# microsoft/ConfigNet

Measured on AMD Instinct MI355X. Metric: train-step images/sec at 256x256 (G+D fwd+bwd), higher is better.
Workload: dtype f32; 1 GPU; ConfigNet second-stage iteration (D + synth-D + latent-D + G + EMA), 256x256, batch 16 per GPU, fp32, Keras-Adam; global_batch=16, resolution=256, latent_dim=145, parallelism=dp1, losses_finite=True

## Files before the change

### confignet_amd/_lib.py

```python
import ctypes
import os

_HERE = os.path.dirname(os.path.abspath(__file__))
LIB_PATH = os.environ.get("CN_LIB") or os.path.join(_HERE, "libconfignet_hip.so")


class CnSumJob(ctypes.Structure):
    _fields_ = [("src", ctypes.c_void_p), ("dst", ctypes.c_void_p), ("count", ctypes.c_longlong), ("parts", ctypes.c_int),
                ("accumulate", ctypes.c_int)]


class CnDepthJob(ctypes.Structure):
    _fields_ = [("a", ctypes.c_void_p), ("b", ctypes.c_void_p), ("c", ctypes.c_void_p), ("m", ctypes.c_int), ("n", ctypes.c_int),
                ("k", ctypes.c_int), ("lda", ctypes.c_int), ("ldb", ctypes.c_int), ("ldc", ctypes.c_int)]


class CnRowsJob(ctypes.Structure):
    _fields_ = [("a", ctypes.c_void_p), ("b", ctypes.c_void_p), ("c", ctypes.c_void_p), ("bias", ctypes.c_void_p), ("mask", ctypes.c_void_p)] + \
               [(n_, ctypes.c_int) for n_ in ("m", "n", "k", "lda", "ldb", "ldc", "tb", "act", "accumulate")] + [("slope", ctypes.c_float)]


class CnGanJob(ctypes.Structure):
    _fields_ = [("s", ctypes.c_void_p), ("out", ctypes.c_void_p), ("gout", ctypes.c_void_p), ("n", ctypes.c_int), ("label", ctypes.c_float)]


class CnConvGeom(ctypes.Structure):
    _fields_ = [(n, ctypes.c_int) for n in (
        "nd", "n", "in_d", "in_h", "in_w", "cin", "out_d", "out_h", "out_w", "cout",
        "k_d", "k_h", "k_w", "s_d", "s_h", "s_w", "dl_d", "dl_h", "dl_w", "p_d", "p_h", "p_w", "up")]


CN_F32, CN_BF16 = 0, 1
CN_U8 = 2
CN_EUNSUPPORTED = -3


class ConfigNetHipError(RuntimeError):
    pass


if not os.path.exists(LIB_PATH):
    raise ImportError(
        "confignet_amd: %s is missing -- build it with `python confignet_amd/build.py` "
        "(or __graft_entry__.build()).  There is no CPU/PyTorch fallback." % LIB_PATH)

lib = ctypes.CDLL(LIB_PATH)

_p = ctypes.c_void_p
_i = ctypes.c_int
_f = ctypes.c_float
_z = ctypes.c_size_t
_G = ctypes.POINTER(CnConvGeom)

SIGNATURES = {
    "cn_version": [],
    "cn_conv_fwd": [_G, _p, _p, _p, _p, _i, _f, _p],
    "cn_conv_fwd_res": [_G, _p, _p, _p, _p, _p, _i, _f, _p],
    "cn_conv_fwd_stats": [_G, _p, _p, _p, _p, _i, _f, _p, _i, _f, _p],
    "cn_scale_columns_segments": [_p, _p, _p, _p, _i, _z, _p],
    "cn_conv_weight_tflip": [_p, _p, _i, _i, _i, _p],
    "cn_conv_dgrad": [_G, _p, _p, _p, _p],
    "cn_conv_dgrad_w": [_G, _p, _p, _p, _p],
    "cn_conv_dgrad_w_res": [_G, _p, _p, _p, _p, _p],
    "cn_bn_fold_bwd": [_p, _i, _i, _p, _p, _p, _p, _p, _p, _p, _p],
    "cn_conv_wgrad_thin_partials": [],
    "cn_conv_wgrad_thin": [_G, _p, _p, _p, _p, _i, _p],
    "cn_conv_wgrad": [_G, _p, _p, _p, _i, _p],
    "cn_conv_wgrad_workspace_bytes": [_G],
    "cn_conv_wgrad_ws": [_G, _p, _p, _p, _i, _p, _z, _p],
    "cn_conv_wgrad_ws_slabs": [_G, _p, _p, _p, _i, _p, _z, ctypes.POINTER(_i), _p],
    "cn_conv_wgrad_dt_workspace_bytes": [_G, _i, _i, ctypes.POINTER(_z)],
    "cn_conv_wgrad_dt": [_G, _p, _i, _p, _i, _p, _i, _p, _z, ctypes.POINTER(_i), _p],
    "cn_conv_wgrad_plan": [_G, _i, _i, _i, ctypes.c_uint, _i, ctypes.POINTER(ctypes.c_longlong)],
    "cn_sum_parts_grouped": [_p, _i, _p],
    "cn_gemm_depth_grouped": [_p, _i, _p],
    "cn_gan_loss_grouped": [_p, _i, _i, _p],
    "cn_gemm_rows_grouped": [_p, _i, _p],
    "cn_gemm_rows_grouped_k": [_p, _i, _p],
    "cn_gemm_rows_grouped_plan": [_p, _i, ctypes.POINTER(_i), _i, ctypes.POINTER(_i)],
    "cn_conv_tune": [_i, _i, ctypes.c_long],
    "cn_conv_fwd_plan": [_G, _i, _i, _i, _i, _i, _i, _i, ctypes.POINTER(ctypes.c_int * 8)],
    "cn_conv_loop_select": [_i, _i, _i, _i],
    "cn_fwd2_col_block": [_i, _i, _i, _i, _i, _i],
    "cn_conv_fwd_dt": [_p, _p, _i, _p, _p, _p, _i, _i, _f, _p],
    "cn_conv_dgrad_dt": [_p, _p, _i, _p, _p, _i, _p],
    "cn_conv_wgrad_c3_partials": [],
    "cn_conv_wgrad_c3": [_p, _p, _p, _i, _p, _p, _i, _p],
    "cn_conv_wino_filter": [_p, _p, _i, _i, _i, _p],
    "cn_conv_fwd_wino": [_i, _i, _i, _i, _i, _p, _p, _p, _p, _i, _f, _p],
    "cn_conv_fwd_wino4": [_i, _i, _i, _i, _i, _p, _p, _p, _p, _i, _f, _p],
    "cn_conv_fwd_wino4_ep": [_i, _i, _i, _i, _i, _p, _p, _p, _p, _i, _f, _i, _p, _p, _p, _p, _i, _f, _p],
    "cn_conv_wino4_filter": [_p, _p, _i, _i, _i, _p],
    "cn_sumpool2": [_p, _p, _i, _i, _i, _i, _i, _i, _i, _p],
    "cn_gemm": [_i, _i, _i, _i, _i, _p, _i, _p, _i, _p, _i, _p, _i, _f, _p],
    "cn_gemm_plan": [_i] * 10 + [ctypes.POINTER(ctypes.c_int * 9)],
    "cn_nc_reduce4": [_p, _p, _i, _i, _i, _f, _i, _i, _p],
    "cn_nc_reduce": [_p, _p, _p, _p, _i, _i, _i, _i, _f, _i, _p],
    "cn_nc_reduce_plan": [_i, _i, _i, _i, _i, _i, ctypes.POINTER(ctypes.c_int * 8)],
    "cn_nc_lin2": [_p, _p, _p, _p, _p, _p, _p, _p, _i, _i, _i, _i, _i, _f, _i, _p],
    "cn_nc_rows_plan": [ctypes.c_longlong, _i, _i, ctypes.POINTER(ctypes.c_int * 2)],
    "cn_norm_coef_fwd": [_i, _p, _p, _p, _p, _p, _p, _p, _p, _i, _i, _i, _f, _p, _i, _p],
    "cn_norm_coef_bwd": [_i, _p, _p, _p, _p, _p, _p, _p, _p, _p, _p, _i, _i, _i, _f, _p],
    "cn_dual_tail_coef_fwd": [_p] * 13 + [_i, _i, _i, _f, _i, _i, _p],
    "cn_dual_tail_coef_bwd": [_p] * 13 + [ctypes.POINTER(ctypes.c_void_p), _i, _i, _i, _f, _i, _i, _p],
    "cn_dual_tail_gx": [_p] * 12 + [_i, _i, _i, _f, _i, _i, _p],
    "cn_dual_tail_gx_tx": [_p] * 18 + [_i, _i, _i, _f, _i, _i, _i, _p],
    "cn_norm_apply": [_i, _i] + [_p] * 13 + [_i, _i, _i, _f, _i, _f, _i, _p],
    "cn_nc_reduce_hxt": [_p, _p, _p, _p, _i, _i, _i, _f, _i, _i, _i, _p],
    "cn_zero": [_p, ctypes.c_size_t, _p],
    "cn_set_deterministic": [_i],
    "cn_get_deterministic": [],
    "cn_det_release_stream": [_p],
    "cn_gemm_acc": [_i, _i, _i, _i, _i, _p, _i, _p, _i, _p, _i, _p],
    "cn_sum_rows_into": [_p, _p, _i, _i, _i, _p],
    "cn_bn_act_bwd": [_p, _p, _p, _p, _p, _p, _p, _p, _i, _i, _i, _i, _i, _i, _p],
    "cn_nc_reduce_dact": [_p, _p, _p, _p, _p, _i, _i, _i, _i, _f, _i, _i, _p],
    "cn_act_fwd": [_p, _p, _z, _i, _f, _i, _p],
    "cn_act_bwd": [_p, _p, _p, _z, _i, _f, _i, _p],
    "cn_act_bwd_bias": [_p, _p, _p, _p, _i, _i, _i, _i, _f, _i, _i, _p],
    "cn_axpby": [_p, _p, _p, _z, _f, _f, _i, _p],
    "cn_mul": [_p, _p, _p, _z, _i, _p],
    "cn_sqdiff_sum": [_p, _p, _p, _z, _f, _i, _p],
    "cn_row_sumsq": [_p, _p, _i, _z, _p],
    "cn_row_scale": [_p, _p, _p, _i, _z, _f, _i, _p],
    "cn_row_scale_diff": [_p, _p, _p, _p, _i, ctypes.c_size_t, _f, _i, _p],
    "cn_tap_bwd": [_p, _p, _p, _p, _p, _i, ctypes.c_size_t, _f, _i, _f, _i, _p],
    "cn_maxpool2_bwd_act": [_p, _p, _p, _p, _f, _p, _i, _i, _i, _i, _i, _i, _p],
    "cn_stream_plan": [_i, _i, ctypes.c_longlong, _z, _i, _i, _i, _i, _i, _i, ctypes.c_uint, _i, ctypes.POINTER(ctypes.c_longlong * 4)],
    "cn_stream_plan_ptrs": [_i, _i, _i, ctypes.c_longlong, _z, _i, _i, _i, _i, _i, _i, ctypes.POINTER(ctypes.c_void_p * 4), _i, ctypes.POINTER(ctypes.c_longlong * 4)],
    "cn_stream_last_plan": [ctypes.POINTER(ctypes.c_longlong * 5)],
    "cn_masked_diff": [_p, _p, _p, _p, _z, _i, _p],
    "cn_maxpool_fwd": [_p, _p, _i, _i, _i, _i, _i, _i, _i, _i, _p],
    "cn_maxpool_bwd": [_p, _p, _p, _i, _i, _i, _i, _i, _i, _i, _i, _p],
    "cn_avgpool3_same": [_p, _p, _i, _i, _i, _i, _i, _p],
    "cn_dwconv3x3_fwd": [_p, _p, _p, _p, _i, _i, _i, _i, _i, _i, _f, _p],
    "cn_image_preprocess": [_p, _i, _p, _i, _i, _i, _i, _i, _i, _f, _f, _p],
    "cn_dwconv3x3_dgrad": [_p, _p, _p, _i, _i, _i, _i, _i, _p],
    "cn_dwconv3x3_wgrad_slices": [_i, _i, _i, _i, _i],
    "cn_dwconv3x3_wgrad": [_p, _p, _p, _i, _i, _i, _i, _i, _i, _p],
    "cn_bn_train_coef": [_p] * 12 + [ctypes.c_longlong, _i, _f, ctypes.c_double, _i, _p],
    "cn_bn_train_apply": [_p, _p, _p, _p, ctypes.c_longlong, _i, _i, _p],
    "cn_bn_train_bwd_slices": [ctypes.c_longlong, _i],
    "cn_chan_slices_plan": [ctypes.c_longlong, _i, _i, ctypes.POINTER(ctypes.c_int * 5)],
    "cn_bn_train_bwd_reduce": [_p] * 6 + [_i, ctypes.c_longlong, _i, _i, _p],
    "cn_bn_train_bwd_apply": [_p] * 8 + [ctypes.c_longlong, _i, _i, _p],
    "cn_chan_affine3_fwd": [_p, _p, _z, ctypes.POINTER(_i), _f, ctypes.POINTER(_f), _p],
    "cn_chan_affine3_bwd": [_p, _p, _z, ctypes.POINTER(_i), _f, _p],
    "cn_gan_loss_fwd": [_p, _p, _i, _f, _p],
    "cn_gan_loss_bwd": [_p, _p, _p, _i, _f, _p],
    "cn_euler_matrix": [_p, _p, _i, _p],
    "cn_euler_matrix_bwd": [_p, _p, _p, _i, _p],
    "cn_rotate3d_fwd": [_p, _p, _p, _i, _i, _i, _p],
    "cn_rotate3d_bwd": [_p, _p, _p, _p, _p, _i, _i, _i, _p],
    "cn_rotate3d_bwd_plan": [_i, _i, _i, _i, ctypes.POINTER(ctypes.c_int * 4)],
    "cn_adam_step": [_p, _p, _p, _p, _p, _z, _p, _f, _f, _f, _f, _p],
    "cn_ema_step": [_p, _p, _z, _f, _p],
    "cn_gather_images_u8": [_p, _p, _p, _p, _i, _i, _i, _i, _p],
    "cn_to_uint8": [_p, _p, _z, _p],
    "cn_hdri_rows_v": [_p, _p, _p, _p, _i, _i, _i, _i, _i, _p],
    "cn_hdri_rows_h": [_p, _p, _p, _p, _p, _p, _p, _i, _i, _i, _i, _i, _i, _p],
    "cn_exp2m1": [_p, _p, _z, _p],
    "cn_warp_affine_u8": [_p] * 6 + [_i] * 6 + [_p],
    "cn_warp_nearest_f32": [_p] * 6 + [_i] * 6 + [_p],
    "cn_eye_mask": [_p, _p, _z, _i] + [_f] * 6 + [_p],
    "cn_spin": [ctypes.c_ulonglong, _p],
    "cn_conv_weight_prep_bf16": [_p, _p, _p, _i, _i, _i, _p],
    "cn_conv_fwd_bf16": [_G, _p, _p, _p, _p, _i, _f, _p],
    "cn_conv_dgrad_bf16": [_G, _p, _p, _p, _p],
    "cn_conv_wgrad_bf16": [_G, _p, _p, _p, _i, _p],
    "cn_cast": [_p, _i, _p, _i, _z, _p],
    "cn_upfold_weights": [_p, _p, _p, _i, ctypes.POINTER(_i), ctypes.POINTER(_i), _i, _i, ctypes.POINTER(_i), ctypes.POINTER(_i), _p],
    "cn_upfold_wgrad": [_p, _p, _i, ctypes.POINTER(_i), ctypes.POINTER(_i), _i, _i, _i, _p],
    "cn_prof_enable": [_i],
    "cn_prof_reset": [],
    "cn_prof_collect": [ctypes.POINTER(_i), ctypes.POINTER(ctypes.c_double), ctypes.POINTER(ctypes.c_double)],
    "cn_prof_collect_by_family": [ctypes.POINTER(_i), ctypes.POINTER(ctypes.c_double), ctypes.POINTER(ctypes.c_double), ctypes.POINTER(ctypes.c_double)],
}

for _name, _args in SIGNATURES.items():
    _fn = getattr(lib, _name)
    _fn.argtypes = _args
    _fn.restype = ctypes.c_int
lib.cn_conv_wgrad_workspace_bytes.restype = ctypes.c_size_t
lib.cn_last_error_string.argtypes = []
lib.cn_last_error_string.restype = ctypes.c_char_p


def check(code, what):
    if code != 0:
        raise ConfigNetHipError("%s failed (%d): %s" % (what, code, lib.cn_last_error_string().decode()))
```

### confignet_amd/csrc/common.h

```cpp
#pragma once
#include <hip/hip_runtime.h>
#include <stdint.h>
#include <stdio.h>
#include "../../include/confignet_hip.h"

void cn_set_error(const char* fmt, ...);

#define CN_CHECK_ARG(cond, ...)            \
    do {                                   \
        if (!(cond)) {                     \
            cn_set_error(__VA_ARGS__);     \
            return CN_EINVAL;              \
        }                                  \
    } while (0)

#define CN_HIP(expr)                                                              \
    do {                                                                          \
        hipError_t e__ = (expr);                                                  \
        if (e__ != hipSuccess) {                                                  \
            cn_set_error("%s failed: %s (%s:%d)", #expr, hipGetErrorString(e__), __FILE__, __LINE__); \
            return CN_EHIP;                                                       \
        }                                                                         \
    } while (0)

#define CN_LAUNCH_CHECK()                                                         \
    do {                                                                          \
        hipError_t e__ = hipGetLastError();                                       \
        if (e__ != hipSuccess) {                                                  \
            cn_set_error("kernel launch failed: %s (%s:%d)", hipGetErrorString(e__), __FILE__, __LINE__); \
            return CN_EHIP;                                                       \
        }                                                                         \
    } while (0)

int cn_zero_async(void* p, size_t bytes, hipStream_t s);

int cn_det();
float* cn_det_ws(hipStream_t s, size_t need_floats);
constexpr size_t CN_DET_WS_FLOATS = (size_t)16 << 20;
int cn_sum_parts(const float* src, float* dst, int parts, long count, int accumulate, float scale, hipStream_t s);

int cn_fwd2(const CnConvGeom* gp, int cfg, int bt, const float* A, const float* B, const float* bias, float* C, long M, int N, int K,
            int act, float slope, int splits, long part_stride, int par, hipStream_t s, const float* res, double x_elems, double w_elems,
            float* stats = nullptr, int stats_mode = 0, float stats_slope = 0.f, int srows = 1, int sper = 1);
void cn_fwd2_tune(int kb, int ns, int np);
void cn_fwd2_grid(int cfg, long M, int N, int par, int splits, int grid[3]);
int cn_igemm_fwd(int cfg, const CnConvGeom& g, bool vec, int par, int splits, const float* x, const float* w, const float* bias, float* y,
                 int act, float slope, hipStream_t s, int bt, long part_stride, const float* res);
void cn_igemm_fwd_grid(int cfg, const CnConvGeom& g, bool vec, int par, int splits, int grid[3]);
int cn_igemm_fwd_thin(const CnConvGeom& g, const float* x, const float* w, const float* bias, float* y, int act, float slope, hipStream_t s);
enum ConvRoute { CN_ROUTE_UP2K4_RGB = 0, CN_ROUTE_S2_IMAGE_DGRAD, CN_ROUTE_S1_IMAGE_DGRAD, CN_ROUTE_THIN_PAR_IGEMM, CN_ROUTE_THIN_COOP,
                 CN_ROUTE_THIN, CN_ROUTE_C3, CN_ROUTE_C7S2, CN_ROUTE_FWD2, CN_ROUTE_IGEMM, CN_ROUTE_UNSUPPORTED };
constexpr int CN_THIN_COOP_PX = 4;
void cn_small_conv(int route, unsigned grid_x, const CnConvGeom& g, bool vec, int par, const void* x, int x_dt, const float* w,
                   const float* bias, void* y, int y_dt, int act, float slope, hipStream_t s);
int cn_fwd2_bf16(const CnConvGeom& g, int cfg, int flip, const void* x, const void* wb, const float* bias, void* y, int act, float slope,
                 int par, hipStream_t s);

enum WgradRoute { CN_WG_C3 = 0, CN_WG_THIN, CN_WG_TINY, CN_WG_WGRAD2, CN_WG_IGEMM, CN_WG_BF16, CN_WG_NONE };
constexpr int CN_C3_WGRAD_TILE = 64, CN_C3_WGRAD_PARTS = 512;
constexpr int CN_THIN_WGRAD_TH = 8, CN_THIN_WGRAD_TW = 32, CN_THIN_WGRAD_PARTS = 512;
struct Wg2Plan {
    int cfg;
    long tiles_x, tiles_y, splits, rows;
};
bool cn_wgrad2_ok(const CnConvGeom& g);
Wg2Plan cn_wgrad2_plan(const CnConvGeom& g, int forced_cfg, long wg_target);
void cn_wgrad2(int cfg, int ns, const CnConvGeom& g, const float* x, const float* gy, float* out, long slab_stride, int rows, int tiles_x,
               int tiles_y, int splits, int accumulate, unsigned grid, hipStream_t s);
void cn_igemm_wgrad(int cfg, const CnConvGeom& g, const float* x, const float* gy, float* gw, int rows, float* parts, int tx, int ty,
                    int splits, dim3 grid, hipStream_t s);
int cn_tiny_wgrad(const CnConvGeom& g, const float* x, const float* gy, float* gw, int blocks, float* parts, hipStream_t s);
void cn_bf16_wgrad(int cfg, const CnConvGeom& g, const void* x, const void* gy, float* gw, int rows, int tx, int ty, int splits, dim3 grid,
                   hipStream_t s);
int cn_c3_wgrad(const CnConvGeom& g, const float* x, const void* gy, int gy_dt, float* scratch, int tiles_x, int ntiles, int nparts,
                size_t lds, hipStream_t s);
void cn_c3_wgrad_reduce(const float* scratch, float* gw, int nparts, int count, int accumulate, hipStream_t s);
void cn_thin_wgrad(const CnConvGeom& g, const float* x, const float* gy, float* scratch, int nwg, size_t lds, int tiles_y, int tiles_x,
                   int ntiles, hipStream_t s);

enum { CN_FAM_FWD_128x128 = 0, CN_FAM_FWD_128x64, CN_FAM_FWD_64x64, CN_FAM_FWD_128x32, CN_FAM_FWD_128x96, CN_FAM_WGRAD_128x128,
       CN_FAM_WGRAD_128x96, CN_FAM_WGRAD_64x64, CN_FAM_WGRAD_128x32, CN_FAM_WINO, CN_FAM_C3_FWD, CN_FAM_S2_IMAGE_DGRAD,
       CN_FAM_THIN, CN_FAM_C3_WGRAD, CN_FAM_BF16_FWD, CN_FAM_BF16_WGRAD, CN_FAM_WGRAD_256x64, CN_FAM_WGRAD_SLAB_SUM };
void cn_prof_begin(hipStream_t s, double flops, double bytes = 0.0, int family = 31);
void cn_prof_end(hipStream_t s);

__device__ __forceinline__ void divmod_pos(int m, int d, int& q, int& r) {
    if ((d & (d - 1)) == 0) {
        q = m >> (__builtin_ctz(d));
        r = m & (d - 1);
    } else {
        q = m / d;
        r = m - q * d;
    }
}

__device__ __forceinline__ float cn_apply_act(float v, int act, float slope) {
    switch (act) {
        case CN_ACT_LRELU: return v > 0.f ? v : v * slope;
        case CN_ACT_RELU: return v > 0.f ? v : 0.f;
        case CN_ACT_TANH: return tanhf(v);
        default: break;
    }
    if (act == CN_ACT_RELU6) return fminf(fmaxf(v, 0.f), 6.f);
    if (act == CN_ACT_SIGMOID) return __fdividef(1.f, 1.f + __expf(-v));
    return v;
}

__device__ __forceinline__ float act_deriv(float o, int act, float slope) {
    if (act == CN_ACT_LRELU) return o > 0.f ? 1.f : slope;
    if (act == CN_ACT_RELU) return o > 0.f ? 1.f : 0.f;
    if (act == CN_ACT_TANH) return 1.f - o * o;
    return 1.f;
}

static inline int cn_cdiv(long a, long b) { return (int)((a + b - 1) / b); }

int cn_cu_count();
```

### confignet_amd/csrc/conv_dispatch.hip

```cpp
#include "common.h"

#include <algorithm>

#include "mma_tile.h"
#include "conv_geom.h"

namespace {

int g_tune_cfg = -1;
int g_tune_splits = 0;
long g_tune_wg_blocks = 0;
int g_tune_wg2_ns = 0;
int g_fwd2_sel = -1;
constexpr int g_fwd2_min_nks = 1;
constexpr int g_fwd2_min_c = 48;

struct ConvReq {
    int bt, has_bias, act, has_res, stats_mode, x_dt, y_dt;
};

struct ConvPlan {
    int route = CN_ROUTE_UNSUPPORTED;
    int ret = CN_EUNSUPPORTED;
    int cfg = -1;
    int splits = 1, par = 0;
    bool vec = false;
    bool plain = false;
    int family = -1;
    int srows = 1, sper = 1;
    int grid[3] = {0, 0, 0};
};

int image_route(const CnConvGeom& g, const ConvReq& q) {
    const bool x32 = q.x_dt == CN_F32, y32 = q.y_dt == CN_F32, x16 = q.x_dt == CN_BF16, y16 = q.y_dt == CN_BF16;
    if (x32 && (y32 || y16) && !q.bt && g.nd == 2 && g.cin == 3 && g.dl_h == 1 && g.dl_w == 1 && !g.up && g.cout > 4 && g.cout <= 64) {
        if (g.k_h == 3 && g.k_w == 3 && g.s_h == g.s_w && (g.s_h == 1 || g.s_h == 2)) return CN_ROUTE_C3;
        if (g.k_h == 7 && g.k_w == 7 && g.s_h == 2 && g.s_w == 2 && !q.has_res) return CN_ROUTE_C7S2;
    }
    if (y32 && g.nd == 2 && g.k_h == 3 && g.k_w == 3 && g.s_h == 1 && g.s_w == 1 && !g.up && g.cout == 3 && !q.has_bias &&
        q.act == CN_ACT_NONE && g.p_h >= 0 && g.p_h <= 2 && g.p_w >= 0 && g.p_w <= 2) {
        if ((x32 || x16) && g.dl_h == 2 && g.dl_w == 2 && g.cin == 48 && g.out_h <= 2 * g.in_h && g.out_w <= 2 * g.in_w) return CN_ROUTE_S2_IMAGE_DGRAD;
        if (x32 && g.dl_h == 1 && g.dl_w == 1 && g.cin == 64) return CN_ROUTE_S1_IMAGE_DGRAD;
    }
    return CN_ROUTE_UNSUPPORTED;
}

ConvPlan plan_conv_fwd(const CnConvGeom& g, const ConvReq& q) {
    ConvPlan p;
    const long M = (long)g.n * g.out_d * g.out_h * g.out_w;
    const bool res = q.has_res != 0, stats = q.stats_mode != 0;
    const int bt = q.bt;
    auto small = [&p](int route, int family, long grid_x) {
        p.route = route;
        p.ret = CN_OK;
        p.family = family;
        p.grid[0] = (int)grid_x; p.grid[1] = p.grid[2] = 1;
        return p;
    };
    auto refuse = [&p](int code) {
        p.ret = code;
        return p;
    };
    const int img = image_route(g, q);
    const long img_grid = img == CN_ROUTE_S2_IMAGE_DGRAD ? (long)g.n * cn_cdiv(g.in_h, 8) * cn_cdiv(g.in_w, 32)
                                                         : (long)g.n * cn_cdiv(g.out_h, 8) * cn_cdiv(g.out_w, 32);
    const int img_family = img == CN_ROUTE_C3 || img == CN_ROUTE_C7S2 ? CN_FAM_C3_FWD : CN_FAM_S2_IMAGE_DGRAD;
    if (q.x_dt != CN_F32 || q.y_dt != CN_F32)
        return img != CN_ROUTE_UNSUPPORTED ? small(img, img_family, img_grid) : p;
    if ((res || stats) && (g.cout <= 4 || g.cin == 3 || g.cout % 4 != 0)) return p;
    if (stats && (bt || cn_det() || g.cin % BK != 0)) return p;
    if (bt && (g.cout <= 4 || g.cin % BK != 0 || g.cout % 4 != 0)) return p;
    if (g.cout <= 4) {
        p.vec = g.cin % 4 == 0;
        p.par = parity_ordered(g);
        const size_t lds = sizeof(float) * 4 * (size_t)g.k_d * g.k_h * g.k_w * g.cin;
        if (lds > 64 * 1024) {
            cn_set_error("thin conv: filter of %zu bytes does not fit the LDS stage", lds);
            return refuse(CN_EINVAL);
        }
        const int T = g.k_d * g.k_h * g.k_w, CL = g.cin / 4;
        const bool dl1 = g.dl_d * g.dl_h * g.dl_w == 1;
        if (g.nd == 2 && g.up == 1 && g.k_h == 4 && g.k_w == 4 && g.s_h == 1 && g.s_w == 1 && g.dl_h == 1 && g.dl_w == 1 &&
            g.cout == 3 && g.cin == 32 && g.p_h == 1 && g.p_w == 1 && g.out_h <= 2 * g.in_h && g.out_w <= 2 * g.in_w)
            return small(CN_ROUTE_UP2K4_RGB, CN_FAM_THIN, (long)g.n * cn_cdiv(g.in_h, 8) * cn_cdiv(g.in_w, 16));
        if (img != CN_ROUTE_UNSUPPORTED) return small(img, img_family, img_grid);
        if (p.par && g.cin % BK == 0 && q.act == CN_ACT_NONE) return small(CN_ROUTE_THIN_PAR_IGEMM, CN_FAM_FWD_128x32, cn_cdiv(M, 128));
        if (p.vec && g.cout == 3 && CL >= 5 && CL <= 16 && T <= 32 && (p.par || dl1) && g.dl_d * g.dl_h * g.dl_w <= 8)
            return small(CN_ROUTE_THIN_COOP, -1, cn_cdiv(M, (256 / (CL <= 8 ? 8 : 16)) * CN_THIN_COOP_PX));
        return small(CN_ROUTE_THIN, -1, cn_cdiv(M, 256));
    }
    if (img != CN_ROUTE_UNSUPPORTED) return small(img, img_family, img_grid);
    if (g.cout % 4 != 0) {
        cn_set_error("cout=%d: implicit-GEMM path needs cout %% 4 == 0", g.cout);
        return refuse(CN_EINVAL);
    }
    const bool vec = g.cin % BK == 0;
    const int par = parity_ordered(g) && vec;
    const long t128 = (long)cn_cdiv(M, 128) * cn_cdiv(g.cout, 128);
    const long t128x64 = (long)cn_cdiv(M, 128) * cn_cdiv(g.cout, 64);
    int cfg;
    long tiles;
    if (g.cout <= 32) { cfg = 3; tiles = (long)cn_cdiv(M, 128) * cn_cdiv(g.cout, 32); }
    else if (g.cout > 64 && t128 >= 512) { cfg = 0; tiles = t128; }
    else if (t128x64 >= 512) { cfg = 1; tiles = t128x64; }
    else { cfg = 2; tiles = (long)cn_cdiv(M, 64) * cn_cdiv(g.cout, 64); }
    if (g.cout % 96 == 0 && g.cout % 128 != 0 &&
        (long)cn_cdiv(M, 128) * (g.cout / 96) >= (g.cout == 96 ? 256 : 384)) {
        cfg = 4;
        tiles = (long)cn_cdiv(M, 128) * (g.cout / 96);
    }
    int splits = 1;
    const bool par_small = par && cfg == 2;
    const long nks_total = vec ? (long)g.k_d * g.k_h * g.k_w * (g.cin / BK) : 0;
    if (cfg == 0 && vec && !par && nks_total <= 8) { cfg = 1; tiles = t128x64; }
    const bool short_full = !par && tiles >= 256 && nks_total < 64;
    if (vec && tiles < (par_small ? 1024 : 512) && !short_full) {
        long nks = nks_total;
        if (par) nks /= (long)g.dl_d * g.dl_h * g.dl_w;
        long want = ((par_small ? 3072 : 1024) + tiles - 1) / tiles;
        if (want > 16) want = 16;
        const long min_steps = par_small ? 8 : 16;
        if (want > nks / min_steps) want = nks / min_steps;
        if (want > 1) splits = (int)want;
    }
    const bool n32 = g.cout == 32 && g.cin >= 32;
    const bool fwd2_takes = g_fwd2_sel != 0 && vec && nks_total > g_fwd2_min_nks && ((g.cin >= g_fwd2_min_c && g.cout >= g_fwd2_min_c) || n32) &&
                            g.dl_d <= 2 && g.dl_h <= 2 && g.dl_w <= 2 && (double)g.n * g.in_d * g.in_h * g.in_w * g.cin < 5.3e8 &&
                            (double)g.k_d * g.k_h * g.k_w * g.cin * g.cout < 5.3e8;
    if (fwd2_takes) {
        const int T = g.k_d * g.k_h * g.k_w;
        const long Me = (par && T == 1) ? M / ((long)g.dl_d * g.dl_h * g.dl_w) : M;
        long nks = nks_total;
        if (par) nks /= (long)g.dl_d * g.dl_h * g.dl_w;
        splits = 1;
        const bool par_balanced = par && g.k_d % g.dl_d == 0 && g.k_h % g.dl_h == 0 && g.k_w % g.dl_w == 0;
        if (n32) {
            cfg = 3;
            tiles = cn_cdiv(M, 128);
        } else if (par && T > 1 && !par_balanced) {
            cfg = 2;
            tiles = (long)cn_cdiv(M, 64) * cn_cdiv(g.cout, 64);
            if (g.cout % 96 == 0 && g.cout % 64 != 0 && (long)cn_cdiv(M, 128) * (g.cout / 96) >= 512) {
                cfg = 4;
                tiles = (long)cn_cdiv(M, 128) * (g.cout / 96);
            }
            if (cfg == 2 && tiles < 1024) {
                long want = (1536 + tiles / 2) / tiles;
                if (want > 16) want = 16;
                if (want > nks / 8) want = nks / 8;
                if (want > 1) splits = (int)want;
            }
        } else {
            struct Cand { int cfg, bm, bn; double step_us; };
            const Cand cands[2] = {{2, 64, 64, 0.265}, {4, 128, 96, 0.68}};
            double best = 0.0;
            bool have = false;
            for (const Cand& c : cands) {
                if (c.cfg == 4 && (g.cout % 96 != 0 || g.cout % 64 == 0 || (long)cn_cdiv(Me, 128) * (g.cout / 96) < 256)) continue;
                const long tl = (long)cn_cdiv(Me, c.bm) * cn_cdiv(g.cout, c.bn);
                const long smax = nks / 8 > 1 ? (nks / 8 > 16 ? 16 : nks / 8) : 1;
                for (long s_ = 1; s_ <= smax; ++s_) {
                    const double waves = (double)cn_cdiv(tl * s_, cn_cu_count());
                    double t = 10.0 + waves * (double)cn_cdiv(nks, s_) * c.step_us * (waves == 1.0 ? 1.06 : 1.0);
                    if (s_ > 1) t += 9.0 + (double)s_ * (double)M * g.cout * 4.0 / 6.0e6;
                    if (s_ > 1 && (res || stats)) t += 5.0 + 2.0 * (double)M * g.cout * 4.0 / 3.0e6;
                    if (!have || t < best) { have = true; best = t; cfg = c.cfg; tiles = tl; splits = (int)s_; }
                }
            }
        }
    }
    if (g_tune_cfg >= 0) cfg = g_tune_cfg;
    if (g_tune_splits > 0) splits = g_tune_splits;
    if (res && splits > 1) return p;
    if (stats) {
        const int qd = par ? g.out_d / g.dl_d : g.out_d, qh = par ? g.out_h / g.dl_h : g.out_h, qw = par ? g.out_w / g.dl_w : g.out_w;
        p.srows = qd * qh * qw;
        p.sper = par ? g.n * p.srows : (int)M;
        if (!fwd2_takes || splits > 1 || cfg == 3 || p.srows % (cfg == 2 ? 64 : 128) != 0) return p;
    }
    if (cn_det() && splits > 1) {
        const long cap = (long)(CN_DET_WS_FLOATS / ((size_t)M * g.cout));
        if (splits > cap) splits = (int)cap;
        if (splits <= 1 || !vec) splits = 1;
    }
    p.route = fwd2_takes && (cfg != 3 || n32) && cfg >= 0 && cfg <= 4 ? CN_ROUTE_FWD2 : CN_ROUTE_IGEMM;
    if (stats && p.route != CN_ROUTE_FWD2) return refuse(CN_EINVAL);
    p.ret = CN_OK;
    p.cfg = cfg;
    p.splits = splits;
    p.par = par;
    p.vec = vec;
    p.family = cfg == 0 ? CN_FAM_FWD_128x128 : cfg == 1 ? CN_FAM_FWD_128x64 : cfg == 3 ? CN_FAM_FWD_128x32 : cfg == 4 ? CN_FAM_FWD_128x96 : CN_FAM_FWD_64x64;
    if (p.route == CN_ROUTE_FWD2) {
        p.plain = !par && g.k_d * g.k_h * g.k_w == 1 && g.s_d == 1 && g.s_h == 1 && g.s_w == 1 && g.dl_d == 1 && g.dl_h == 1 &&
                  g.dl_w == 1 && !g.up && g.p_d == 0 && g.p_h == 0 && g.p_w == 0 && g.out_d == g.in_d && g.out_h == g.in_h &&
                  g.out_w == g.in_w;
        cn_fwd2_grid(cfg, M, g.cout, par, splits, p.grid);
    } else {
        cn_igemm_fwd_grid(cfg, g, vec, par, splits, p.grid);
    }
    return p;
}

int run_conv_fwd(const ConvPlan& p, const CnConvGeom& g, const ConvReq& q, const void* x, const float* w, const float* bias,
                 const float* res, void* y, float slope, float* stats, float stats_slope, hipStream_t s) {
    if (p.route == CN_ROUTE_UNSUPPORTED) return p.ret;
    const long M = (long)g.n * g.out_d * g.out_h * g.out_w;
    const int splits = p.splits;
    float* parts = nullptr;
    if (cn_det() && splits > 1) {
        parts = cn_det_ws(s, (size_t)splits * M * g.cout);
        if (!parts) return CN_EINVAL;
    }
    const int kact = splits > 1 ? CN_ACT_NONE : q.act;
    if (splits > 1 && !parts) {
        if (int ez__ = cn_zero_async(y, sizeof(float) * M * g.cout, s)) return ez__;
    }
    const long part_stride = parts ? (long)M * g.cout : 0;
    float* const out = parts ? parts : (float*)y;
    if (p.family >= 0) cn_prof_begin(s, conv_flops(g), conv_bytes(g, q.x_dt == CN_BF16 ? 2.0 : 4.0, q.y_dt == CN_BF16 ? 2.0 : 4.0), p.family);
    int e = CN_OK;
    switch (p.route) {
        case CN_ROUTE_FWD2: {
            const double xe = (double)g.n * g.in_d * g.in_h * g.in_w * g.cin, we = (double)g.k_d * g.k_h * g.k_w * g.cin * g.cout;
            e = cn_fwd2(p.plain ? nullptr : &g, p.cfg, q.bt, (const float*)x, w, bias, out, M, g.cout, g.cin, kact, slope, splits, part_stride,
                        p.plain ? 0 : p.par, s, res, xe, we, stats, q.stats_mode, stats_slope, p.srows, p.sper);
            break;
        }
        case CN_ROUTE_IGEMM:
            e = cn_igemm_fwd(p.cfg, g, p.vec, p.par, splits, (const float*)x, w, bias, out, kact, slope, s, q.bt, part_stride, res);
            break;
        case CN_ROUTE_THIN_PAR_IGEMM:
            e = cn_igemm_fwd_thin(g, (const float*)x, w, bias, out, kact, slope, s);
            break;
        default:
            cn_small_conv(p.route, (unsigned)p.grid[0], g, p.vec, p.par, x, q.x_dt, w, bias, y, q.y_dt, kact, slope, s);
            break;
    }
    if (p.family >= 0) cn_prof_end(s);
    CN_CHECK_ARG(e != CN_EUNSUPPORTED, "convolution plan (route %d, tile %d) refused by its kernel", p.route, p.cfg);
    if (e != CN_OK) return e;
    CN_LAUNCH_CHECK();
    if (parts) e = cn_sum_parts(parts, (float*)y, splits, (long)M * g.cout, 0, 1.f, s);
    if (e == CN_OK && splits > 1 && q.act != CN_ACT_NONE) e = cn_act_fwd(y, y, (size_t)M * g.cout, q.act, slope, CN_F32, s);
    return e;
}

int conv_fwd(const CnConvGeom* gp, const ConvReq& q, const void* x, const float* w, const float* bias, const float* res, void* y,
             float slope, float* stats, float stats_slope, void* stream) {
    if (int e = check_geom(gp)) return e;
    CN_CHECK_ARG(x && w && y, "NULL tensor");
    return run_conv_fwd(plan_conv_fwd(*gp, q), *gp, q, x, w, bias, res, y, slope, stats, stats_slope, (hipStream_t)stream);
}

}

extern "C" int cn_conv_fwd(const CnConvGeom* gp, const float* x, const float* w, const float* bias, float* y, int act,
                           float slope, void* stream) {
    return conv_fwd(gp, ConvReq{0, bias != nullptr, act, 0, 0, CN_F32, CN_F32}, x, w, bias, nullptr, y, slope, nullptr, 0.f, stream);
}

extern "C" int cn_conv_fwd_stats(const CnConvGeom* gp, const float* x, const float* w, const float* bias, float* y, int act,
                                 float slope, float* stats, int stats_mode, float stats_slope, void* stream) {
    CN_CHECK_ARG(stats && (stats_mode == 1 || stats_mode == 2), "cn_conv_fwd_stats: stats buffer and mode 1 / 2");
    CN_CHECK_ARG(stats_mode == 1 || act == CN_ACT_NONE, "cn_conv_fwd_stats: mode 2 takes the statistics of the pre-activation output");
    return conv_fwd(gp, ConvReq{0, bias != nullptr, act, 0, stats_mode, CN_F32, CN_F32}, x, w, bias, nullptr, y, slope, stats, stats_slope, stream);
}

extern "C" int cn_conv_fwd_res(const CnConvGeom* gp, const float* x, const float* w, const float* bias, const float* res, float* y,
                               int act, float slope, void* stream) {
    CN_CHECK_ARG(res, "cn_conv_fwd_res: res is NULL");
    return conv_fwd(gp, ConvReq{0, bias != nullptr, act, 1, 0, CN_F32, CN_F32}, x, w, bias, res, y, slope, nullptr, 0.f, stream);
}

extern "C" int cn_conv_fwd_dt(const CnConvGeom* gp, const void* x, int x_dt, const float* w, const float* bias, void* y, int y_dt,
                              int act, float slope, void* stream) {
    if (int e = check_geom(gp)) return e;
    CN_CHECK_ARG(x && w && y, "NULL tensor");
    if (x_dt == CN_F32 && y_dt == CN_F32) return CN_EUNSUPPORTED;
    const ConvReq q{0, bias != nullptr, act, 0, 0, x_dt, y_dt};
    return run_conv_fwd(plan_conv_fwd(*gp, q), *gp, q, x, w, bias, nullptr, y, slope, nullptr, 0.f, (hipStream_t)stream);
}

extern "C" int cn_conv_dgrad(const CnConvGeom* gp, const float* gy, const float* w_tflip, float* gu, void* stream) {
    if (int e = check_geom(gp)) return e;
    CN_CHECK_ARG(gp->dl_d == 1 && gp->dl_h == 1 && gp->dl_w == 1, "dgrad of a dilated-input geometry is not defined here");
    const CnConvGeom d = dgrad_geom(*gp);
    return cn_conv_fwd(&d, gy, w_tflip, nullptr, gu, CN_ACT_NONE, 0.f, stream);
}

extern "C" int cn_conv_dgrad_dt(const CnConvGeom* gp, const void* gy, int gy_dt, const float* w_tflip, void* gu, int gu_dt,
                                void* stream) {
    if (int e = check_geom(gp)) return e;
    if (gp->dl_d != 1 || gp->dl_h != 1 || gp->dl_w != 1) return CN_EUNSUPPORTED;
    const CnConvGeom d = dgrad_geom(*gp);
    return cn_conv_fwd_dt(&d, gy, gy_dt, w_tflip, nullptr, gu, gu_dt, CN_ACT_NONE, 0.f, stream);
}

extern "C" int cn_conv_dgrad_w(const CnConvGeom* gp, const float* gy, const float* w, float* gu, void* stream) {
    if (int e = check_geom(gp)) return e;
    if (gp->dl_d != 1 || gp->dl_h != 1 || gp->dl_w != 1) return CN_EUNSUPPORTED;
    const CnConvGeom d = dgrad_geom(*gp);
    return conv_fwd(&d, ConvReq{1, 0, CN_ACT_NONE, 0, 0, CN_F32, CN_F32}, gy, w, nullptr, nullptr, gu, 0.f, nullptr, 0.f, stream);
}

// ... 40 lines not shown
    int grid[3] = {0, 0, 0};
    size_t lds = 0;
    size_t ws_floats = 0;
    size_t det_floats = 0;
    bool zero = false;
    int sum = WG_SUM_NONE;
};

struct WgTile { int bm, bn; };
WgTile wgrad_tile(int cfg) { return cfg == 3 ? WgTile{128, 32} : cfg == 4 ? WgTile{128, 96} : cfg == 0 ? WgTile{128, 128} : cfg == 5 ? WgTile{256, 64} : WgTile{64, 64}; }
int wgrad_family(int cfg) {
    return cfg == 3 ? CN_FAM_WGRAD_128x32 : cfg == 4 ? CN_FAM_WGRAD_128x96 : cfg == 0 ? CN_FAM_WGRAD_128x128 : cfg == 5 ? CN_FAM_WGRAD_256x64 : CN_FAM_WGRAD_64x64;
}

void sliced_grid(const CnConvGeom& g, WgTile t, WgradPlan& p) {
    const long Ktot = (long)g.k_d * g.k_h * g.k_w * g.cin;
    const int gx = cn_cdiv(Ktot, t.bm), gy = cn_cdiv(g.cout, t.bn);
    p.grid[0] = gx; p.grid[1] = gy; p.grid[2] = (int)p.splits;
    if ((long)gx * gy > 1 && p.splits >= 16) {
        p.tx = gx; p.ty = gy;
        p.grid[0] = cn_cdiv(p.splits, 8) * 8 * gx * gy; p.grid[1] = p.grid[2] = 1;
    }
}

bool igemm_wgrad_slices(const CnConvGeom& g, WgTile t, long wg_target, bool det, WgradPlan& p) {
    const long M = (long)g.n * g.out_d * g.out_h * g.out_w;
    const long Ktot = (long)g.k_d * g.k_h * g.k_w * g.cin;
    const long tiles = (long)cn_cdiv(Ktot, t.bm) * cn_cdiv(g.cout, t.bn);
    const long wg_blocks = wg_target > 0 ? wg_target : 2048;
    long splits = (wg_blocks + tiles - 1) / tiles;
    if (det) {
        const long cap = (long)(CN_DET_WS_FLOATS / ((size_t)Ktot * g.cout));
        if (cap < 1) {
            cn_set_error("deterministic filter gradient: %ld x %d filter does not fit the workspace", Ktot, g.cout);
            return false;
        }
        if (splits > cap) splits = cap;
    }
    long rows = (M + splits - 1) / splits;
    if (rows < 256) rows = 256;
    rows = (rows + BK - 1) / BK * BK;
    p.rows = rows;
    p.splits = (M + rows - 1) / rows;
    return true;
}

void bf16_wgrad_slices(const CnConvGeom& g, WgTile t, WgradPlan& p) {
    constexpr long KS = 32, min_rows = 512;
    const long M = (long)g.n * g.out_d * g.out_h * g.out_w;
    const long Ktot = (long)g.k_d * g.k_h * g.k_w * g.cin;
    const long tiles = (long)cn_cdiv(Ktot, t.bm) * cn_cdiv(g.cout, t.bn);
    const long per_cu = t.bm * t.bn >= 128 * 128 ? 3 : t.bm * t.bn >= 128 * 96 ? 4 : 5;
    const long target = 256 * per_cu * (t.bn >= 96 ? 1 : 2);
    long splits = target / tiles;
    if (splits > M / min_rows) splits = M / min_rows;
    const long fill = std::min<long>(M / 256, (256 + tiles - 1) / tiles);
    if (splits < fill) splits = fill;
    if (splits >= 16) splits &= ~7L;
    if (splits < 1) splits = 1;
    long rows = (M + splits - 1) / splits;
    if (rows < 256) rows = std::min<long>(256, (M + KS - 1) / KS * KS);
    rows = (rows + KS - 1) / KS * KS;
    p.rows = rows;
    p.splits = (M + rows - 1) / rows;
}

WgradPlan plan_conv_wgrad(const CnConvGeom& g, const WgradReq& q) {
    WgradPlan p;
    const long M = (long)g.n * g.out_d * g.out_h * g.out_w;
    const long Ktot = (long)g.k_d * g.k_h * g.k_w * g.cin;
    const size_t count = (size_t)Ktot * g.cout;
    const bool x32 = q.x_dt == CN_F32, y32 = q.gy_dt == CN_F32, x16 = q.x_dt == CN_BF16, y16 = q.gy_dt == CN_BF16;
    auto may = [&q](int route) { return (q.routes & wg_bit(route)) != 0; };
    auto take = [&p](int route, int family) {
        p.route = route;
        p.ret = CN_OK;
        p.family = family;
    };
    if (may(CN_WG_C3) && x32 && (y32 || y16) && g.nd == 2 && g.cin == 3 && g.k_h == 3 && g.k_w == 3 && g.k_d == 1 && g.s_h == g.s_w &&
        (g.s_h == 1 || g.s_h == 2) && g.dl_h == 1 && g.dl_w == 1 && g.up == 0 && g.cout <= 64 && g.cout >= 4 && g.cout % 4 == 0) {
        take(CN_WG_C3, CN_FAM_C3_WGRAD);
        p.tx = cn_cdiv(g.out_w, CN_C3_WGRAD_TILE);
        p.grid[0] = CN_C3_WGRAD_PARTS; p.grid[1] = p.grid[2] = 1;
        const int pw = CN_C3_WGRAD_TILE * g.s_h + 2, gpitch = (g.cout + 3) & ~3;
        p.lds = sizeof(float) * 4 * (size_t)(3 * pw * 3 + CN_C3_WGRAD_TILE * gpitch);
        if (p.lds < sizeof(float) * 4 * 2 * 16 * 64) p.lds = sizeof(float) * 4 * 2 * 16 * 64;
        p.ws_floats = CN_C3_WGRAD_PARTS * count;
        p.sum = WG_SUM_C3;
        return p;
    }
    const int T = g.k_h * g.k_w;
    if (may(CN_WG_THIN) && x32 && y32 && g.nd == 2 && g.cout <= 4 && g.cin % 4 == 0 && g.cin >= 8 && g.cin <= 64 && g.s_h == 1 && g.s_w == 1 &&
        g.dl_h == 1 && g.dl_w == 1 && T <= 16 && T * (g.cin / 4) <= 256) {
        const int PH0 = ((CN_THIN_WGRAD_TH + g.k_h - 1) >> g.up) + 2, PW0 = ((CN_THIN_WGRAD_TW + g.k_w - 1) >> g.up) + 2;
        size_t lds = sizeof(float) * ((size_t)PH0 * PW0 * g.cin + CN_THIN_WGRAD_TH * CN_THIN_WGRAD_TW * 4);
        const size_t red = sizeof(float) * 256 * 4 * g.cout;
        if (lds < red) lds = red;
        if (lds <= 64 * 1024) {
            take(CN_WG_THIN, -1);
            p.ty = cn_cdiv(g.out_h, CN_THIN_WGRAD_TH); p.tx = cn_cdiv(g.out_w, CN_THIN_WGRAD_TW);
            const int ntiles = g.n * p.ty * p.tx;
            p.grid[0] = ntiles < CN_THIN_WGRAD_PARTS ? ntiles : CN_THIN_WGRAD_PARTS; p.grid[1] = p.grid[2] = 1;
            p.lds = lds;
            p.ws_floats = CN_THIN_WGRAD_PARTS * count;
            p.sum = WG_SUM_PARTS;
            return p;
        }
    }
    if (x16 && y16) {
        if (!may(CN_WG_BF16) || g.cin % 8 || g.cout % 8) return p;
        take(CN_WG_BF16, CN_FAM_BF16_WGRAD);
        p.cfg = wgrad_tile_cfg(g);
        bf16_wgrad_slices(g, wgrad_tile(p.cfg), p);
        sliced_grid(g, wgrad_tile(p.cfg), p);
        p.zero = true;
        return p;
    }
    if (!x32 || !y32) return p;
    if (may(CN_WG_WGRAD2) && cn_wgrad2_ok(g) && Ktot >= 64) {
        const int t = g_tune_cfg;
        const Wg2Plan w = cn_wgrad2_plan(g, t == 0 || t == 2 || t == 3 || t == 4 || t == 5 ? t : -1, g_tune_wg_blocks);
        take(CN_WG_WGRAD2, wgrad_family(w.cfg));
        p.cfg = w.cfg;
        p.stages = w.cfg == 3 || g_tune_wg2_ns == 3 ? 3 : 4;
        p.splits = w.splits; p.rows = w.rows;
        p.tx = (int)w.tiles_x; p.ty = (int)w.tiles_y;
        p.grid[0] = (int)((w.splits >= 8 ? cn_cdiv(w.splits, 8) * 8 : w.splits) * w.tiles_x * w.tiles_y); p.grid[1] = p.grid[2] = 1;
        if (w.splits > 1) {
            p.ws_floats = (size_t)w.splits * count;
            p.sum = q.caller_slabs ? WG_SUM_CALLER : WG_SUM_PARTS;
        }
        return p;
    }
    if (may(CN_WG_TINY) && Ktot <= 4 && g.cout <= 4 && g.k_d * g.k_h * g.k_w == 1 && g.s_h == 1 && g.s_w == 1 && g.s_d == 1 && !g.up &&
        g.p_h == 0 && g.p_w == 0 && g.p_d == 0) {
        take(CN_WG_TINY, -1);
        p.grid[0] = cn_cdiv(M, 256) > 1024 ? 1024 : cn_cdiv(M, 256); p.grid[1] = p.grid[2] = 1;
        p.zero = true;
        if (q.det) {
            p.det_floats = (size_t)p.grid[0] * 16;
            p.sum = WG_SUM_PARTS;
        }
        return p;
    }
    if (!may(CN_WG_IGEMM)) return p;
    const int cfg = wgrad_tile_cfg(g);
    if (!igemm_wgrad_slices(g, wgrad_tile(cfg), g_tune_wg_blocks, q.det, p)) {
        p.ret = CN_EINVAL;
        return p;
    }
    take(CN_WG_IGEMM, wgrad_family(cfg));
    p.cfg = cfg;
    sliced_grid(g, wgrad_tile(cfg), p);
    p.zero = true;
    if (q.det) {
        p.det_floats = (size_t)p.splits * count;
        p.sum = WG_SUM_PARTS;
    }
    return p;
}

int sum_conv_wgrad(const WgradPlan& p, int nparts, long count, int mode, float* gw, const float* ws, const float* det, int* parts_out,
                   hipStream_t s) {
    CN_LAUNCH_CHECK();
    const int add = mode != CN_WGRAD_WRITE;
    if (p.sum == WG_SUM_PARTS) return cn_sum_parts(det ? det : ws, gw, nparts, count, det ? 1 : add, 1.f, s);
    if (p.sum == WG_SUM_C3) {
        cn_c3_wgrad_reduce(ws, gw, nparts, (int)count, mode == CN_WGRAD_ADD, s);
        CN_LAUNCH_CHECK();
    }
    if (p.sum == WG_SUM_CALLER) *parts_out = nparts;
    return CN_OK;
}

int run_conv_wgrad(const WgradPlan& p, const CnConvGeom& g, const WgradReq& q, const void* x, const void* gy, float* gw, int mode,
                   float* ws, size_t ws_bytes, int* parts_out, hipStream_t s) {
    if (parts_out) *parts_out = 0;
    if (p.route == CN_WG_NONE) return p.ret;
    CN_CHECK_ARG(mode == CN_WGRAD_WRITE || mode == CN_WGRAD_ADD || mode == CN_WGRAD_ZEROED, "filter gradient: mode %d", mode);
    CN_CHECK_ARG(p.ws_floats == 0 || (ws && ws_bytes >= sizeof(float) * p.ws_floats), "filter gradient: workspace of %zu bytes, %zu needed",
                 ws ? ws_bytes : (size_t)0, sizeof(float) * p.ws_floats);
    CN_CHECK_ARG(p.sum != WG_SUM_CALLER || parts_out, "filter gradient: slabs left to a caller that takes none");
    CN_CHECK_ARG(p.route != CN_WG_BF16 || (((uintptr_t)x | (uintptr_t)gy) & 15) == 0, "bf16 convolution needs 16-byte aligned tensors");
    const long count = (long)g.k_d * g.k_h * g.k_w * g.cin * g.cout;
    const int add = mode != CN_WGRAD_WRITE;
    float* det = nullptr;
    if (p.det_floats) {
        det = cn_det_ws(s, p.det_floats);
        if (!det) return CN_EINVAL;
    }
    if (p.zero && !add) {
        if (int ez__ = cn_zero_async(gw, sizeof(float) * count, s)) return ez__;
    }
    if (p.family >= 0)
        cn_prof_begin(s, p.route == CN_WG_C3 ? 2.0 * 27.0 * g.cout * (double)g.n * g.out_h * g.out_w : conv_flops(g),
                      conv_bytes(g, q.x_dt == CN_BF16 ? 2.0 : 4.0, q.gy_dt == CN_BF16 ? 2.0 : 4.0, 4.0), p.family);
    const dim3 grid(p.grid[0], p.grid[1], p.grid[2]);
    int nparts = (int)p.splits, e = CN_OK;
    switch (p.route) {
        case CN_WG_C3:
            e = cn_c3_wgrad(g, (const float*)x, gy, q.gy_dt, ws, p.tx, g.n * g.out_h * p.tx, nparts = p.grid[0], p.lds, s);
            break;
        case CN_WG_THIN:
            cn_thin_wgrad(g, (const float*)x, (const float*)gy, ws, nparts = p.grid[0], p.lds, p.ty, p.tx, g.n * p.ty * p.tx, s);
            break;
        case CN_WG_TINY:
            nparts = cn_tiny_wgrad(g, (const float*)x, (const float*)gy, gw, p.grid[0], det, s);
            break;
        case CN_WG_WGRAD2:
            cn_wgrad2(p.cfg, p.stages, g, (const float*)x, (const float*)gy, p.splits > 1 ? ws : gw, p.splits > 1 ? count : 0, (int)p.rows,
                      p.tx, p.ty, (int)p.splits, add, grid.x, s);
            break;
        case CN_WG_IGEMM:
            cn_igemm_wgrad(p.cfg, g, (const float*)x, (const float*)gy, gw, (int)p.rows, det, p.tx, p.ty, (int)p.splits, grid, s);
            break;
        default:
            cn_bf16_wgrad(p.cfg, g, x, gy, gw, (int)p.rows, p.tx, p.ty, (int)p.splits, grid, s);
            break;
    }
    const bool sum_in_bracket = p.route != CN_WG_C3;
    if (p.family >= 0 && !sum_in_bracket) cn_prof_end(s);
    if (e == CN_OK) e = sum_conv_wgrad(p, nparts, count, mode, gw, ws, det, parts_out, s);
    if (p.family >= 0 && sum_in_bracket) cn_prof_end(s);
    return e;
}

int conv_wgrad(const CnConvGeom* gp, const WgradReq& q, const void* x, const void* gy, float* gw, int mode, void* ws, size_t ws_bytes,
               int* parts, void* stream) {
    if (int e = check_geom(gp)) return e;
    CN_CHECK_ARG(x && gy && gw, "NULL tensor");
    return run_conv_wgrad(plan_conv_wgrad(*gp, q), *gp, q, x, gy, gw, mode, (float*)ws, ws_bytes, parts, (hipStream_t)stream);
}

}

extern "C" int cn_conv_wgrad(const CnConvGeom* gp, const float* x, const float* gy, float* gw, int accumulate, void* stream) {
    return conv_wgrad(gp, WgradReq{CN_F32, CN_F32, false, WG_ATOMIC}, x, gy, gw, accumulate ? CN_WGRAD_ADD : CN_WGRAD_WRITE, nullptr, 0, nullptr, stream);
}

extern "C" size_t cn_conv_wgrad_workspace_bytes(const CnConvGeom* gp) {
    if (!gp || check_geom(gp) != CN_OK) return 0;
    return sizeof(float) * plan_conv_wgrad(*gp, WgradReq{CN_F32, CN_F32, false, WG_FP32_GEMM}).ws_floats;
}

extern "C" int cn_conv_wgrad_ws(const CnConvGeom* gp, const float* x, const float* gy, float* gw, int accumulate, void* workspace,
                                size_t workspace_bytes, void* stream) {
    return conv_wgrad(gp, WgradReq{CN_F32, CN_F32, false, WG_FP32_GEMM}, x, gy, gw, accumulate ? CN_WGRAD_ADD : CN_WGRAD_WRITE, workspace,
                      workspace_bytes, nullptr, stream);
}

extern "C" int cn_conv_wgrad_ws_slabs(const CnConvGeom* gp, const float* x, const float* gy, float* gw, int accumulate, void* workspace,
                                      size_t workspace_bytes, int* parts, void* stream) {
    CN_CHECK_ARG(parts, "cn_conv_wgrad_ws_slabs: parts is NULL");
    return conv_wgrad(gp, WgradReq{CN_F32, CN_F32, true, WG_FP32_GEMM}, x, gy, gw, accumulate ? CN_WGRAD_ADD : CN_WGRAD_WRITE, workspace,
                      workspace_bytes, parts, stream);
}

extern "C" int cn_conv_wgrad_bf16(const CnConvGeom* gp, const uint16_t* x, const uint16_t* gy, float* gw, int accumulate,
                                  void* stream) {
    return conv_wgrad(gp, WgradReq{CN_BF16, CN_BF16, false, wg_bit(CN_WG_BF16)}, x, gy, gw, accumulate ? CN_WGRAD_ADD : CN_WGRAD_WRITE, nullptr, 0,
                      nullptr, stream);
}

extern "C" int cn_conv_wgrad_c3_partials(void) { return CN_C3_WGRAD_PARTS; }

extern "C" int cn_conv_wgrad_c3(const CnConvGeom* gp, const float* x, const void* gy, int gy_dt, float* scratch, float* gw,
                                int accumulate, void* stream) {
    CN_CHECK_ARG(gp && x && gy && scratch && gw && (gy_dt == CN_F32 || gy_dt == CN_BF16), "conv_wgrad_c3: bad args");
    return conv_wgrad(gp, WgradReq{CN_F32, gy_dt, false, wg_bit(CN_WG_C3)}, x, gy, gw, accumulate ? CN_WGRAD_ADD : CN_WGRAD_WRITE, scratch, SIZE_MAX,
                      nullptr, stream);
}

extern "C" int cn_conv_wgrad_thin_partials(void) { return CN_THIN_WGRAD_PARTS; }

extern "C" int cn_conv_wgrad_thin(const CnConvGeom* gp, const float* x, const float* gy, float* scratch, float* gw, int accumulate,
                                  void* stream) {
    CN_CHECK_ARG(scratch, "conv_wgrad_thin: NULL");
    return conv_wgrad(gp, WgradReq{CN_F32, CN_F32, false, wg_bit(CN_WG_THIN)}, x, gy, gw, accumulate ? CN_WGRAD_ADD : CN_WGRAD_WRITE, scratch, SIZE_MAX,
                      nullptr, stream);
}

extern "C" int cn_conv_wgrad_dt_workspace_bytes(const CnConvGeom* gp, int x_dt, int gy_dt, size_t* bytes) {
    if (int e = check_geom(gp)) return e;
    CN_CHECK_ARG(bytes, "cn_conv_wgrad_dt_workspace_bytes: bytes is NULL");
    const WgradPlan p = plan_conv_wgrad(*gp, WgradReq{x_dt, gy_dt, false, WG_ALL});
    *bytes = sizeof(float) * p.ws_floats;
    return p.ret;
}

extern "C" int cn_conv_wgrad_dt(const CnConvGeom* gp, const void* x, int x_dt, const void* gy, int gy_dt, float* gw, int mode, void* workspace,
                                size_t workspace_bytes, int* parts, void* stream) {
    return conv_wgrad(gp, WgradReq{x_dt, gy_dt, parts != nullptr, WG_ALL}, x, gy, gw, mode, workspace, workspace_bytes, parts, stream);
}

extern "C" int cn_conv_wgrad_plan(const CnConvGeom* gp, int x_dt, int gy_dt, int caller_slabs, unsigned routes, int det, long long out[12]) {
    if (int e = check_geom(gp)) return e;
    CN_CHECK_ARG(out, "cn_conv_wgrad_plan: out is NULL");
    const WgradPlan p = plan_conv_wgrad(*gp, WgradReq{x_dt, gy_dt, caller_slabs != 0, routes, det < 0 ? cn_det() != 0 : det != 0});
    const long long v[12] = {p.route, p.cfg, p.splits, p.rows, p.family, p.grid[0], p.grid[1], p.grid[2], (long long)p.ws_floats, p.zero, p.sum, p.stages};
    for (int i = 0; i < 12; ++i) out[i] = v[i];
    return p.ret;
}

extern "C" int cn_conv_loop_select(int loop, int kb, int ns, int np) {
    CN_CHECK_ARG(loop >= -1 && loop <= 1 && (kb == 0 || kb == 16 || kb == 32) && (ns == 0 || ns == 3 || ns == 4) && np >= -1 && np <= 2,
                 "cn_conv_loop_select: bad argument");
    g_fwd2_sel = loop;
    cn_fwd2_tune(kb, ns, np);
    g_tune_wg2_ns = ns;
    return CN_OK;
}

extern "C" int cn_conv_tune(int cfg, int splits, long wg_blocks) {
    g_tune_cfg = cfg;
    g_tune_splits = splits;
    g_tune_wg_blocks = wg_blocks;
    return CN_OK;
}
```

### confignet_amd/csrc/elementwise.hip

```cpp
#include "common.h"
#include "typed.h"
#include <stdlib.h>

namespace {

__device__ __forceinline__ float lrelu(float v, float s) { return v > 0.f ? v : v * s; }


template <int V> struct RowV { float v[V]; };

template <int V, typename T>
__device__ __forceinline__ RowV<V> ld_row(const T* p) {
    RowV<V> r;
    if constexpr (V == 4) {
        const float4 t = ld4<T>(p);
        r.v[0] = t.x; r.v[1] = t.y; r.v[2] = t.z; r.v[3] = t.w;
    } else {
        r.v[0] = ldf<T>(p);
    }
    return r;
}
template <int V, typename T>
__device__ __forceinline__ void st_row(T* p, const RowV<V>& r) {
    if constexpr (V == 4) st4<T>(p, make_float4(r.v[0], r.v[1], r.v[2], r.v[3]));
// ... 1312 lines not shown
    CN_CHECK_ARG(a && b && out && (dt == CN_F32 || dt == CN_BF16), "sqdiff_sum: bad args");
    if (!numel) return CN_OK;
    StreamPlan sp;
    if (int e = stream_entry_plan(stream_req(SP_SQDIFF_SUM, dt, 1, numel), dt, StreamPtrs{{a, b}}, &sp)) return e;
    const int vec = sp.path == SP_VEC, blocks = sp.gx;
    float* parts = nullptr;
    if (sp.parts) {
        parts = cn_det_ws((hipStream_t)stream, (size_t)sp.parts);
        if (!parts) return CN_EINVAL;
    }
    CN_DISPATCH_DT(dt, hipLaunchKernelGGL((sqdiff_sum_kernel<T>), dim3(blocks), dim3(256), 0, (hipStream_t)stream, (const T*)a, (const T*)b, out, numel, scale, vec, parts));
    CN_LAUNCH_CHECK();
    if (parts) return cn_sum_parts(parts, out, blocks, 1, 1, scale, (hipStream_t)stream);
    return CN_OK;
}
extern "C" int cn_row_sumsq(const float* x, float* out, int n, size_t row, void* stream) {
    CN_CHECK_ARG(x && out && n > 0 && row > 0, "row_sumsq: bad args");
    StreamPlan sp;
    if (int e = stream_entry_plan(stream_req(SP_ROW_SUMSQ, CN_F32, n, row), CN_F32, StreamPtrs{{x}}, &sp)) return e;
    const int vec = sp.path == SP_VEC, bpr = sp.gx;
    if (sp.parts) {
        float* parts = cn_det_ws((hipStream_t)stream, (size_t)sp.parts);
        if (!parts) return CN_EINVAL;
        hipLaunchKernelGGL(row_sumsq_kernel, dim3(bpr, n), dim3(256), 0, (hipStream_t)stream, x, out, row, vec, parts);
        CN_LAUNCH_CHECK();
        return cn_sum_parts(parts, out, bpr, n, 0, 1.f, (hipStream_t)stream);
    }
    if (int ez__ = cn_zero_async(out, sizeof(float) * n, (hipStream_t)stream)) return ez__;
    hipLaunchKernelGGL(row_sumsq_kernel, dim3(bpr, n), dim3(256), 0, (hipStream_t)stream, x, out, row, vec, (float*)nullptr);
    CN_LAUNCH_CHECK();
    return CN_OK;
}
extern "C" int cn_row_scale(const void* x, const float* s, void* out, int n, size_t row, float k, int dt, void* stream) {
    CN_CHECK_ARG(x && s && out && n > 0 && row > 0 && (dt == CN_F32 || dt == CN_BF16), "row_scale: bad args");
    StreamPlan sp;
    if (int e = stream_entry_plan(stream_req(SP_ROW_SCALE, dt, n, row), dt, StreamPtrs{{x, out}}, &sp)) return e;
    const int vec = sp.path == SP_VEC;
    CN_DISPATCH_DT(dt, hipLaunchKernelGGL((row_scale_kernel<T>), dim3(sp.gx, sp.gy), dim3(256), 0, (hipStream_t)stream, (const T*)x, s, (T*)out, row, k, vec));
    CN_LAUNCH_CHECK();
    return CN_OK;
}
extern "C" int cn_row_scale_diff(const void* x, const void* x2, const float* s, void* out, int n, size_t row, float k, int dt, void* stream) {
    CN_CHECK_ARG(x && x2 && s && out && n > 0 && row > 0 && (dt == CN_F32 || dt == CN_BF16), "row_scale_diff: bad args");
    StreamPlan sp;
    if (int e = stream_entry_plan(stream_req(SP_ROW_SCALE_DIFF, dt, n, row), dt, StreamPtrs{{x, x2, out}}, &sp)) return e;
    const int vec = sp.path == SP_VEC;
    CN_DISPATCH_DT(dt, hipLaunchKernelGGL((row_scale_kernel<T>), dim3(sp.gx, sp.gy), dim3(256), 0, (hipStream_t)stream, (const T*)x, s, (T*)out, row, k, vec, (const T*)x2));
    CN_LAUNCH_CHECK();
    return CN_OK;
}
extern "C" int cn_tap_bwd(const void* y, const void* target, const void* g, const float* s, void* out, int n, size_t row, float k,
                          int act, float slope, int dt, void* stream) {
    CN_CHECK_ARG(y && target && s && out && n > 0 && row > 0 && (dt == CN_F32 || dt == CN_BF16), "tap_bwd: bad args");
    StreamPlan sp;
    if (int e = stream_entry_plan(stream_req(SP_TAP_BWD, dt, n, row), dt, StreamPtrs{{y, target, g, out}}, &sp)) return e;
    const int vec = sp.path == SP_VEC;
    CN_DISPATCH_DT(dt, hipLaunchKernelGGL((tap_bwd_kernel<T>), dim3(sp.gx, sp.gy), dim3(256), 0, (hipStream_t)stream, (const T*)y, (const T*)target,
                                          (const T*)g, s, (T*)out, row, k, vec, act, slope));
    CN_LAUNCH_CHECK();
    return CN_OK;
}
extern "C" int cn_masked_diff(const float* a, const float* b, const uint8_t* mask, float* out, size_t pixels, int c, void* stream) {
    CN_CHECK_ARG(a && mask && out && c > 0, "masked_diff: bad args");
    if (!pixels) return CN_OK;
    EW_LAUNCH(masked_diff_kernel, pixels, a, b, mask, out, pixels, c)
}
extern "C" int cn_maxpool_fwd(const void* x, void* y, int n, int h, int w, int c, int k, int s, int pad, int dt, void* stream) {
    CN_CHECK_ARG(x && y && n > 0 && h > 0 && w > 0 && c > 0 && k > 0 && s > 0 && pad >= 0 && (dt == CN_F32 || dt == CN_BF16), "maxpool: bad args");
    StreamPlan sp;
    if (int e = stream_entry_plan(pool_req(SP_MAXPOOL_FWD, dt, n, h, w, c, k, s, pad), dt, StreamPtrs{{x, y}}, &sp)) return e;
    const int oh = sp.oh, ow = sp.ow;
    if (sp.path == SP_VEC) {
        CN_DISPATCH_DT(dt, hipLaunchKernelGGL((maxpool_fwd4_kernel<T>), dim3(sp.gx), dim3(256), 0, (hipStream_t)stream,
                                              (const T*)x, (T*)y, n, h, w, c / 4, oh, ow, k, s, pad));
        CN_LAUNCH_CHECK();
        return CN_OK;
    }
    CN_DISPATCH_DT(dt, hipLaunchKernelGGL((maxpool_fwd_kernel<T>), dim3(sp.gx), dim3(256), 0, (hipStream_t)stream, (const T*)x, (T*)y, n, h, w, c, oh, ow, k, s, pad));
    CN_LAUNCH_CHECK();
    return CN_OK;
}
extern "C" int cn_avgpool3_same(const void* x, void* y, int n, int h, int w, int c, int dt, void* stream) {
    CN_CHECK_ARG(x && y && n > 0 && h > 0 && w > 0 && c > 0 && (dt == CN_F32 || dt == CN_BF16), "avgpool3_same: bad args");
    StreamPlan sp;
    if (int e = stream_entry_plan(pool_req(SP_AVGPOOL3_SAME, dt, n, h, w, c, 3, 1, 1), dt, StreamPtrs{{x, y}}, &sp)) return e;
    CN_DISPATCH_DT(dt, {
        if (sp.path == SP_VEC) hipLaunchKernelGGL((avgpool3_same_kernel<4, T>), dim3(sp.gx), dim3(256), 0, (hipStream_t)stream, (const T*)x, (T*)y, n, h, w, c);
        else hipLaunchKernelGGL((avgpool3_same_kernel<1, T>), dim3(sp.gx), dim3(256), 0, (hipStream_t)stream, (const T*)x, (T*)y, n, h, w, c);
    });
    CN_LAUNCH_CHECK();
    return CN_OK;
}
extern "C" int cn_maxpool_bwd(const void* x, const void* gy, void* gx, int n, int h, int w, int c, int k, int s, int pad, int dt, void* stream) {
    CN_CHECK_ARG(x && gy && gx && n > 0 && h > 0 && w > 0 && c > 0 && k > 0 && s > 0 && pad >= 0 && (dt == CN_F32 || dt == CN_BF16), "maxpool_bwd: bad args");
    StreamPlan sp;
    if (int e = stream_entry_plan(pool_req(SP_MAXPOOL_BWD, dt, n, h, w, c, k, s, pad), dt, StreamPtrs{{x, gy, gx}}, &sp)) return e;
    const int oh = sp.oh, ow = sp.ow;
    if (sp.path == SP_POOL2) {
        const long windows4 = (long)n * oh * ow * (c / 4);
        CN_DISPATCH_DT(dt, hipLaunchKernelGGL((maxpool2_bwd_kernel<T>), dim3(sp.gx), dim3(256), 0, (hipStream_t)stream,
                                              (const T*)x, (const T*)gy, (T*)gx, windows4, oh, ow, c / 4));
        CN_LAUNCH_CHECK();
        return CN_OK;
    }
    if (sp.path == SP_VEC) {
        CN_DISPATCH_DT(dt, hipLaunchKernelGGL((maxpool_bwd4_kernel<T>), dim3(sp.gx), dim3(256), 0, (hipStream_t)stream,
                                              (const T*)x, (const T*)gy, (T*)gx, n, h, w, c / 4, oh, ow, k, s, pad));
        CN_LAUNCH_CHECK();
        return CN_OK;
    }
    CN_DISPATCH_DT(dt, hipLaunchKernelGGL((maxpool_bwd_kernel<T>), dim3(sp.gx), dim3(256), 0, (hipStream_t)stream, (const T*)x, (const T*)gy, (T*)gx, n, h, w, c, oh, ow, k, s, pad));
    CN_LAUNCH_CHECK();
    return CN_OK;
}
extern "C" int cn_maxpool2_bwd_act(const void* x, const void* gy, const void* target, const float* s, float k, void* gx, int n, int h,
                                   int w, int c, int s_rows, int dt, void* stream) {
    CN_CHECK_ARG(x && gy && gx && n > 0 && h > 0 && w > 0 && c > 0 && (dt == CN_F32 || dt == CN_BF16) && (!target || (s && (s_rows == 1 || s_rows == n))),
                 "maxpool2_bwd_act: bad args");
    StreamPlan sp;
    if (int e = stream_entry_plan(pool_req(SP_MAXPOOL2_BWD_ACT, dt, n, h, w, c, 2, 2, 0), dt, StreamPtrs{{x, gy, target, gx}}, &sp)) return e;
    const int oh = sp.oh, ow = sp.ow;
    const long windows4 = (long)n * oh * ow * (c / 4);
    CN_DISPATCH_DT(dt, hipLaunchKernelGGL((maxpool2_bwd_kernel<T>), dim3(sp.gx), dim3(256), 0, (hipStream_t)stream,
                                          (const T*)x, (const T*)gy, (T*)gx, windows4, oh, ow, c / 4, 1, (const T*)target, s, s_rows, k));
    CN_LAUNCH_CHECK();
    return CN_OK;
}
extern "C" int cn_stream_plan(int op, int dt, long long rows, size_t row, int c, int h, int w, int k, int s, int pad, unsigned aligned, int det,
                              long long out[4]) {
    CN_CHECK_ARG(out && op >= 0 && op < SP_OPS && (dt == CN_F32 || dt == CN_BF16) && rows > 0 && rows <= 2147483647LL, "stream_plan: bad args");
    const bool pool = op >= SP_MAXPOOL_FWD;
    CN_CHECK_ARG(pool || row > 0, "stream_plan: no elements");
    CN_CHECK_ARG(!pool || (c > 0 && h > 0 && w > 0 && k > 0 && s > 0 && pad >= 0), "stream_plan: bad pool geometry");
    CN_CHECK_ARG(op != SP_ROW_SUMSQ || dt == CN_F32, "stream_plan: row_sumsq is fp32");
    StreamPlan sp;
    const StreamReq r{op, dt, (long)rows, row, c, h, w, k, s, pad, aligned, det ? 1 : 0};
    if (int e = plan_stream(r, &sp)) return e;
    out[0] = sp.path; out[1] = sp.gx; out[2] = sp.gy; out[3] = sp.parts;
    return CN_OK;
}
extern "C" int cn_stream_plan_ptrs(int op, int dt, int dst_dt, long long rows, size_t row, int c, int h, int w, int k, int s, int pad,
                                   const void* const ptrs[4], int det, long long out[4]) {
    CN_CHECK_ARG(ptrs && op >= 0 && op < SP_OPS && (dst_dt == CN_F32 || dst_dt == CN_BF16) && (dt == CN_F32 || dt == CN_BF16), "stream_plan_ptrs: bad args");
    return cn_stream_plan(op, dt, rows, row, c, h, w, k, s, pad, stream_mask(op, dt, dst_dt, StreamPtrs{{ptrs[0], ptrs[1], ptrs[2], ptrs[3]}}), det, out);
}
extern "C" int cn_stream_last_plan(long long out[5]) {
    CN_CHECK_ARG(out, "stream_last_plan: NULL");
    for (int i = 0; i < 5; ++i) out[i] = g_stream_last[i];
    return CN_OK;
}
extern "C" int cn_chan_affine3_fwd(const float* x, float* y, size_t pixels, const int* perm, float scale, const float* off, void* stream) {
    CN_CHECK_ARG(x && y && perm && off, "chan_affine3: NULL");
    for (int i = 0; i < 3; ++i) CN_CHECK_ARG(perm[i] >= 0 && perm[i] < 3, "chan_affine3: bad perm");
    EW_LAUNCH(chan_affine3_fwd_kernel, pixels, x, y, pixels, perm[0], perm[1], perm[2], scale, off[0], off[1], off[2])
}
extern "C" int cn_chan_affine3_bwd(const float* gy, float* gx, size_t pixels, const int* perm, float scale, void* stream) {
    CN_CHECK_ARG(gy && gx && perm, "chan_affine3_bwd: NULL");
    for (int i = 0; i < 3; ++i) CN_CHECK_ARG(perm[i] >= 0 && perm[i] < 3, "chan_affine3: bad perm");
    EW_LAUNCH(chan_affine3_bwd_kernel, pixels, gy, gx, pixels, perm[0], perm[1], perm[2], scale)
}
extern "C" int cn_gan_loss_fwd(const float* s, float* out, int n, float label, void* stream) {
    CN_CHECK_ARG(s && out && n > 0, "gan_loss: bad args");
    hipLaunchKernelGGL(gan_loss_fwd_kernel, dim3(1), dim3(256), 0, (hipStream_t)stream, s, out, n, label);
    CN_LAUNCH_CHECK();
    return CN_OK;
}
extern "C" int cn_gan_loss_bwd(const float* s, const float* gout, float* gs, int n, float label, void* stream) {
    CN_CHECK_ARG(s && gout && gs && n > 0, "gan_loss_bwd: bad args");
    hipLaunchKernelGGL(gan_loss_bwd_kernel, dim3(cn_cdiv(n, 256)), dim3(256), 0, (hipStream_t)stream, s, gout, gs, n, label);
    CN_LAUNCH_CHECK();
    return CN_OK;
}
namespace {
constexpr int CN_GAN_GROUP = 16;
struct GanJobs {
    const float* s[CN_GAN_GROUP];
    float* out[CN_GAN_GROUP];
    const float* gout[CN_GAN_GROUP];
    int n[CN_GAN_GROUP];
    float label[CN_GAN_GROUP];
};
__global__ __launch_bounds__(256) void gan_loss_grouped_fwd_kernel(GanJobs J) {
    const int j = blockIdx.x;
    const float* __restrict__ s = J.s[j];
    const int n = J.n[j];
    const float label = J.label[j];
    float acc = 0.f;
    for (int i = threadIdx.x; i < n; i += 256) acc += label * softplus_f(-s[i]) + (1.f - label) * softplus_f(s[i]);
    const float t = block_sum(acc);
    if (threadIdx.x == 0) J.out[j][0] = t / (float)n;
}
__global__ __launch_bounds__(256) void gan_loss_grouped_bwd_kernel(GanJobs J) {
    const int j = blockIdx.x;
    const float* __restrict__ s = J.s[j];
    float* __restrict__ gs = J.out[j];
    const int n = J.n[j];
    const float label = J.label[j];
    const float g = J.gout[j] ? J.gout[j][0] : 0.f;
    for (int i = threadIdx.x; i < n; i += 256) gs[i] = g * (-label * sigmoid_f(-s[i]) + (1.f - label) * sigmoid_f(s[i])) / (float)n;
}
}
extern "C" int cn_gan_loss_grouped(const CnGanJob* jobs, int njobs, int backward, void* stream) {
    CN_CHECK_ARG(njobs >= 0 && (njobs == 0 || jobs), "cn_gan_loss_grouped: bad arguments");
    for (int first = 0; first < njobs; first += CN_GAN_GROUP) {
        GanJobs J{};
        const int cnt = njobs - first < CN_GAN_GROUP ? njobs - first : CN_GAN_GROUP;
        for (int q = 0; q < cnt; ++q) {
            const CnGanJob& d = jobs[first + q];
            CN_CHECK_ARG(d.s && d.out && d.n > 0, "cn_gan_loss_grouped: job %d: NULL tensor or n = %d", first + q, d.n);
            J.s[q] = d.s; J.out[q] = d.out; J.gout[q] = d.gout; J.n[q] = d.n; J.label[q] = d.label;
        }
        if (backward) hipLaunchKernelGGL(gan_loss_grouped_bwd_kernel, dim3(cnt), dim3(256), 0, (hipStream_t)stream, J);
        else hipLaunchKernelGGL(gan_loss_grouped_fwd_kernel, dim3(cnt), dim3(256), 0, (hipStream_t)stream, J);
        CN_LAUNCH_CHECK();
    }
    return CN_OK;
}
extern "C" int cn_adam_step(float* theta, const float* grad, float* m, float* v, float* ema, size_t numel,
                            const float* lr_t, float beta1, float beta2, float eps, float ema_alpha, void* stream) {
    CN_CHECK_ARG(theta && grad && m && v && lr_t, "adam: NULL");
    if (!numel) return CN_OK;
    EW_LAUNCH(adam_kernel, numel, theta, grad, m, v, ema, numel, lr_t, beta1, beta2, eps, ema_alpha)
}
extern "C" int cn_ema_step(float* ema, const float* theta, size_t numel, float alpha, void* stream) {
    CN_CHECK_ARG(ema && theta, "ema: NULL");
    if (!numel) return CN_OK;
    EW_LAUNCH(ema_kernel, numel, ema, theta, numel, alpha)
}
extern "C" int cn_gather_images_u8(const uint8_t* pool, const int64_t* idx, const uint8_t* flip, float* out, int n, int h,
                                   int w, int c, void* stream) {
    CN_CHECK_ARG(pool && idx && out && n > 0, "gather_images: bad args");
    const size_t total = (size_t)n * h * w * c;
    EW_LAUNCH(gather_u8_kernel, total, pool, idx, flip, out, n, h, w, c)
}
namespace {
__global__ void scale_columns_segments_kernel(const float* __restrict__ src, float* __restrict__ dst, const int* __restrict__ seg,
                                              const float* __restrict__ a, int nseg, long total4) {
    for (long e4 = (long)blockIdx.x * blockDim.x + threadIdx.x; e4 < total4; e4 += (long)gridDim.x * blockDim.x) {
        const int e = (int)(e4 * 4);
        int lo = 0, hi = nseg - 1;
        while (lo < hi) {
            const int mid = (lo + hi + 1) >> 1;
            if (seg[5 * mid + 1] <= e) lo = mid; else hi = mid - 1;
        }
        const int* sg = seg + 5 * lo;
        const int local = e - sg[1];
        if (local >= sg[2]) continue;
        const int col = local % sg[3];
        const float4 v = *reinterpret_cast<const float4*>(src + sg[0] + local);
        const float4 c = *reinterpret_cast<const float4*>(a + sg[4] + col);
        *reinterpret_cast<float4*>(dst + e) = make_float4(v.x * c.x, v.y * c.y, v.z * c.z, v.w * c.w);
    }
}

__global__ __launch_bounds__(256) void bn_fold_bwd_kernel(const int* __restrict__ seg, int nseg, const float* __restrict__ gwf,
                                                          const float* __restrict__ gshift, const float* __restrict__ arena,
                                                          const float* __restrict__ a, const float* __restrict__ rs,
                                                          const float* __restrict__ bm, float* __restrict__ gout) {
    const int b = blockIdx.x;
    int lo = 0, hi = nseg - 1;
    while (lo < hi) {
        const int mid = (lo + hi + 1) >> 1;
        if (seg[9 * mid + 8] <= b) lo = mid; else hi = mid - 1;
    }
    const int* sg = seg + 9 * lo;
    const int cout = sg[3], K = sg[2] / cout;
    const int c4 = threadIdx.x & 15, rl = threadIdx.x >> 4;
    const int col = (b - sg[8]) * 64 + c4 * 4;
    const float4 av = *reinterpret_cast<const float4*>(a + sg[4] + col);
    float4 dot = make_float4(0.f, 0.f, 0.f, 0.f);
    for (int r = rl; r < K; r += 16) {
        const long off = (long)r * cout + col;
        const float4 g = *reinterpret_cast<const float4*>(gwf + sg[1] + off);
        const float4 w = *reinterpret_cast<const float4*>(arena + sg[0] + off);
        float4* d = reinterpret_cast<float4*>(gout + sg[0] + off);
        float4 o = *d;
        o.x += g.x * av.x; o.y += g.y * av.y; o.z += g.z * av.z; o.w += g.w * av.w;
        *d = o;
        dot.x += g.x * w.x; dot.y += g.y * w.y; dot.z += g.z * w.z; dot.w += g.w * w.w;
    }
    __shared__ float4 red[16][16];
    red[rl][c4] = dot;
    __syncthreads();
    if (rl == 0) {
        float4 t = red[0][c4];
        for (int q = 1; q < 16; ++q) { const float4 u = red[q][c4]; t.x += u.x; t.y += u.y; t.z += u.z; t.w += u.w; }
        const float4 gs = *reinterpret_cast<const float4*>(gshift + sg[4] + col);
        const float4 m = *reinterpret_cast<const float4*>(bm + sg[4] + col);
        const float4 rv = *reinterpret_cast<const float4*>(rs + sg[4] + col);
        float4* gg = reinterpret_cast<float4*>(gout + sg[6] + col);
        float4* gbeta = reinterpret_cast<float4*>(gout + sg[7] + col);
        float4* gbias = reinterpret_cast<float4*>(gout + sg[5] + col);
        float4 o = *gg;
        o.x += rv.x * (t.x + gs.x * m.x); o.y += rv.y * (t.y + gs.y * m.y); o.z += rv.z * (t.z + gs.z * m.z); o.w += rv.w * (t.w + gs.w * m.w);
        *gg = o;
        o = *gbeta;
        o.x += gs.x; o.y += gs.y; o.z += gs.z; o.w += gs.w;
        *gbeta = o;
        o = *gbias;
        o.x += av.x * gs.x; o.y += av.y * gs.y; o.z += av.z * gs.z; o.w += av.w * gs.w;
        *gbias = o;
    }
}
}

extern "C" int cn_bn_fold_bwd(const int* seg, int nseg, int blocks, const float* gwf, const float* gshift, const float* arena,
                              const float* a, const float* rs, const float* bm, float* gout, void* stream) {
    CN_CHECK_ARG(seg && gwf && gshift && arena && a && rs && bm && gout && nseg > 0 && blocks > 0, "bn_fold_bwd: bad args");
    hipLaunchKernelGGL(bn_fold_bwd_kernel, dim3((unsigned)blocks), dim3(256), 0, (hipStream_t)stream, seg, nseg, gwf, gshift, arena, a, rs,
                       bm, gout);
    CN_LAUNCH_CHECK();
    return CN_OK;
}

extern "C" int cn_scale_columns_segments(const float* src, float* dst, const int* seg, const float* a, int nseg, size_t total,
                                         void* stream) {
    CN_CHECK_ARG(src && dst && seg && a && nseg > 0 && total % 4 == 0, "scale_columns_segments: bad args");
    if (!total) return CN_OK;
    const long total4 = (long)(total / 4);
    hipLaunchKernelGGL(scale_columns_segments_kernel, dim3(ew_blocks((size_t)total4)), dim3(256), 0, (hipStream_t)stream, src, dst, seg, a,
                       nseg, total4);
    CN_LAUNCH_CHECK();
    return CN_OK;
}

extern "C" int cn_to_uint8(const float* x, uint8_t* out, size_t numel, void* stream) {
    CN_CHECK_ARG(x && out, "to_uint8: NULL");
    if (!numel) return CN_OK;
    EW_LAUNCH(to_uint8_kernel, numel, x, out, numel)
}
```

### confignet_amd/csrc/wgrad2.hip

```cpp
#include "common.h"

#include "mma_tile.h"
#include "conv_geom.h"
#include "slots.h"

namespace {

typedef __attribute__((address_space(3))) float lds_float;
typedef float v2f __attribute__((ext_vector_type(2)));

constexpr int w2_task_slot(int q, int nslot, int ntask) { return q * nslot / ntask; }
constexpr int w2_dma_before(int ja, int jb, int nslot, int ntask, int limit) {
    int n = 0;
    for (int j = 0; j < ja; ++j) n += w2_task_slot(4 * j + 3, nslot, ntask) < limit ? 1 : 0;
    for (int j = 0; j < jb; ++j) n += w2_task_slot(4 * ja + 2 * j + 1, nslot, ntask) < limit ? 1 : 0;
    return n;
}

template <int WM, int WN, int TM, int TN, int KB, int NS>
__device__ __forceinline__ void wgrad2_body(const CnConvGeom& g, const float* __restrict__ X, const float* __restrict__ GY,
                                            float* __restrict__ out, long slab_stride, int rows_per_split, int tiles_x, int tiles_y,
                                            int nsplits, int accumulate) {
    static_assert(WM * WN == 4, "4 waves per workgroup");
    constexpr int BI = 32 * WM * TM, BN = 32 * WN * TN;
    constexpr int QA = KB * BI / 256, QB = KB * BN / 256;
    static_assert(QA % 4 == 0, "A pieces divide over the 4 waves");
    constexpr int JA = QA / 4, JB = (QB + 3) / 4, LPW = JA + JB;
    constexpr int SA = KB * BI, SB = JB * 4 * 256;
    constexpr int NMT = TM * TN;
    constexpr int GK = NMT >= 3 ? 1 : 4 / NMT;
    constexpr int NM = GK * NMT, G = KB / (2 * GK);
    constexpr int RDA = TM == 2 ? 1 : TM, RDB = TN == 2 ? 1 : TN, RD1 = RDA + RDB, RD = GK * RD1;
    constexpr int NSL = NM > 1 ? NM / 2 : 1;
    constexpr int AHEAD = 2, NSET = 4;
    constexpr int NTASK = 4 * JA + 2 * JB, NSLOT = G * NM;
    static_assert(G >= 4 && G % NSET == 0, "operand sets rotate per group and return to set 0 at the step boundary");
    static_assert((NS - 1) * LPW < 64, "vmcnt range");
    constexpr int VMW = (NS - 3) * LPW + w2_dma_before(JA, JB, NSLOT, NTASK, (G - AHEAD) * NM);
    static_assert(NS >= 3, "stages");
    __shared__ __attribute__((aligned(1024))) float SM[NS * (SA + SB)];

    const int ntile = tiles_x * tiles_y, id = blockIdx.x;
    int bz, tt;
    if (nsplits >= 8) {
        const int grp = id / (8 * ntile), rr = id - grp * 8 * ntile;
        bz = grp * 8 + (rr & 7);
        if (bz >= nsplits) return;
        tt = rr >> 3;
    } else {
        tt = id / nsplits;
        bz = id - tt * nsplits;
    }
    const int by = tt / tiles_x, bx = tt - by * tiles_x;

    const int tid = threadIdx.x, lane = tid & 63;
    const int wave = __builtin_amdgcn_readfirstlane(tid >> 6);
    const int wm = wave / WN, wn = wave % WN, half = lane >> 5, l31 = lane & 31;
    const int M = g.n * g.out_d * g.out_h * g.out_w;
    const int Ktot = g.k_d * g.k_h * g.k_w * g.cin;
    const int i0 = bx * BI, n0 = by * BN;
    const int mbeg = bz * rows_per_split;
    const int mend = min(M, mbeg + rows_per_split);
    const int nks = (mend - mbeg + KB - 1) / KB;

    const __amdgpu_buffer_rsrc_t xres = __builtin_amdgcn_make_buffer_rsrc(
        const_cast<float*>(X), 0, (int)((long)g.n * g.in_d * g.in_h * g.in_w * g.cin * 4), 0x00020000);
    const __amdgpu_buffer_rsrc_t yres = __builtin_amdgcn_make_buffer_rsrc(const_cast<float*>(GY), 0, (int)((long)M * g.cout * 4), 0x00020000);
    constexpr unsigned OOB = 0x80000000u;

    constexpr int PA = BI / 4;
    const int a_pc = lane % PA;
    const int a_i = i0 + 4 * a_pc;
    const bool a_ok = a_i < Ktot;
    int a_kd, a_kh, a_kw;
    const int a_tap = a_ok ? a_i / g.cin : 0;
    const int a_ci = a_ok ? a_i - a_tap * g.cin : 0;
    tap_decode(g, a_tap, a_kd, a_kh, a_kw);
    const int up = g.up;
    const int bw = a_kw - g.p_w, bh = a_kh - g.p_h, bd = a_kd - g.p_d;
    const unsigned ext_w = (unsigned)(g.in_w << up), ext_h = (unsigned)(g.in_h << up), ext_d = (unsigned)(g.in_d << up);
    const int Sw = g.cin, Sh = g.in_w * g.cin, Sd = g.in_h * Sh, Sn = g.in_d * Sd;
    int dg_w, dg_t, dg_h, dg_u, dg_d, dg_n;
    divmod_pos(KB, g.out_w, dg_t, dg_w);
    divmod_pos(dg_t, g.out_h, dg_u, dg_h);
    divmod_pos(dg_u, g.out_d, dg_n, dg_d);
    const int st_w = dg_w * g.s_w, st_h = dg_h * g.s_h, st_d = dg_d * g.s_d, st_n = dg_n * Sn;
    const int wr_w = g.out_w * g.s_w, wr_h = g.out_h * g.s_h, wr_d = g.out_d * g.s_d;
    const int lim_w = bw + wr_w, lim_h = bh + wr_h, lim_d = bd + wr_d;
    int p_m[JA], v_w[JA], v_h[JA], v_d[JA], n_off[JA];
#pragma unroll
    for (int j = 0; j < JA; ++j) {
        int m = mbeg + ((wave + 4 * j) * 64 + lane) / PA, pw, ph, pd, pn;
        p_m[j] = m;
        divmod_pos(m, g.out_w, m, pw);
        divmod_pos(m, g.out_h, m, ph);
        divmod_pos(m, g.out_d, pn, pd);
        v_w[j] = pw * g.s_w + bw;
        v_h[j] = ph * g.s_h + bh;
        v_d[j] = pd * g.s_d + bd;
        n_off[j] = pn * Sn + a_ci;
    }
    constexpr int PB = BN / 4;
    int b_m[JB], b_col[JB];
    unsigned b_dead[JB];
#pragma unroll
    for (int j = 0; j < JB; ++j) {
        const int idx = (wave + 4 * j) * 64 + lane;
        const int col = n0 + 4 * (idx % PB);
        const bool live = wave + 4 * j < QB && col < g.cout;
        b_m[j] = mbeg + idx / PB;
        b_col[j] = live ? col : 0;
        b_dead[j] = live ? 0u : OOB;
    }

    unsigned vo[LPW];
    auto task = [&](auto qc, int rs) __attribute__((always_inline)) {
        constexpr int q = decltype(qc)::value;
        (void)vo; (void)p_m; (void)v_w; (void)v_h; (void)v_d; (void)n_off; (void)b_m; (void)b_col; (void)b_dead;
        if constexpr (q < 4 * JA) {
            constexpr int j = q / 4, part = q % 4;
            if constexpr (part == 0) {
                const bool ok = a_ok & (p_m[j] < mend) & ((unsigned)v_w[j] < ext_w) & ((unsigned)v_h[j] < ext_h) & ((unsigned)v_d[j] < ext_d);
                const int off = n_off[j] + __mul24(v_d[j] >> up, Sd) + __mul24(v_h[j] >> up, Sh) + __mul24(v_w[j] >> up, Sw);
                vo[j] = ok ? (unsigned)off * 4u : OOB;
            } else if constexpr (part == 1) {
                p_m[j] += KB;
                v_w[j] += st_w;
                const bool cw = v_w[j] >= lim_w;
                v_w[j] -= cw ? wr_w : 0;
                v_h[j] += st_h + (cw ? g.s_h : 0);
            } else if constexpr (part == 2) {
                const bool ch = v_h[j] >= lim_h;
                v_h[j] -= ch ? wr_h : 0;
                v_d[j] += st_d + (ch ? g.s_d : 0);
                const bool cd = v_d[j] >= lim_d;
                v_d[j] -= cd ? wr_d : 0;
                n_off[j] += st_n + (cd ? Sn : 0);
            } else {
                __builtin_amdgcn_raw_ptr_buffer_load_lds(xres, (lds_float*)(SM + rs * SA + (wave + 4 * j) * 256), 16, vo[j], 0, 0, 0);
            }
        } else {
            constexpr int j = (q - 4 * JA) / 2, part = (q - 4 * JA) % 2;
            if constexpr (part == 0) {
                const int m = min(b_m[j], M - 1);
                b_m[j] += KB;
                vo[JA + j] = ((unsigned)(__mul24(m, g.cout) + b_col[j]) * 4u) | b_dead[j];
            } else {
                __builtin_amdgcn_raw_ptr_buffer_load_lds(yres, (lds_float*)(SM + NS * SA + rs * SB + (wave + 4 * j) * 256), 16, vo[JA + j], 0, 0, 0);
            }
        }
    };

    f32x16 acc[TM][TN];
#pragma unroll
    for (int i = 0; i < TM; ++i)
#pragma unroll
        for (int j = 0; j < TN; ++j)
#pragma unroll
            for (int r = 0; r < 16; ++r) acc[i][j][r] = 0.f;

    const int ac = wm * 32 * TM + (TM == 2 ? 2 * l31 : l31), bc = wn * 32 * TN + (TN == 2 ? 2 * l31 : l31);
    const unsigned lds0 = (unsigned)(unsigned long long)(lds_float*)SM;
    const unsigned a_lane = lds0 + 4u * (unsigned)(half * BI + ac), b_lane = lds0 + 4u * (unsigned)(NS * SA + half * BN + bc);
    v2f a2[NSET][GK], b2[NSET][GK];
    float a1[NSET][GK][TM], b1[NSET][GK][TN];
    auto read_op = [&](auto rc, auto gc, unsigned ab, unsigned bb) __attribute__((always_inline)) {
        constexpr int r = decltype(rc)::value, gq = decltype(gc)::value, set = gq % NSET;
        constexpr int k = r / RD1, q = r % RD1, kk = 2 * (GK * gq + k);
        (void)a2; (void)b2; (void)a1; (void)b1;
        if constexpr (q < RDA) {
            if constexpr (TM == 2) asm volatile("ds_read_b64 %0, %1 offset:%2" : "=v"(a2[set][k]) : "v"(ab), "n"(4 * kk * BI));
            else asm volatile("ds_read_b32 %0, %1 offset:%2" : "=v"(a1[set][k][TM == 2 ? 0 : q]) : "v"(ab), "n"(4 * kk * BI + 128 * q));
        } else {
            constexpr int qb = q - RDA;
            if constexpr (TN == 2) asm volatile("ds_read_b64 %0, %1 offset:%2" : "=v"(b2[set][k]) : "v"(bb), "n"(4 * kk * BN));
            else asm volatile("ds_read_b32 %0, %1 offset:%2" : "=v"(b1[set][k][TN == 2 ? 0 : qb]) : "v"(bb), "n"(4 * kk * BN + 128 * qb));
        }
    };
    auto read_slot = [&](auto mc, auto gc, unsigned ab, unsigned bb) __attribute__((always_inline)) {
        constexpr int m = decltype(mc)::value;
        sl_static_for<RD>([&](auto rc) __attribute__((always_inline)) {
            constexpr int r = decltype(rc)::value;
            if constexpr (m < NSL && r >= (m * RD + NSL - 1) / NSL && r < ((m + 1) * RD + NSL - 1) / NSL) read_op(rc, gc, ab, bb);
        });
    };
    auto mfma_one = [&](auto mc, auto gc) __attribute__((always_inline)) {
        constexpr int m = decltype(mc)::value, set = decltype(gc)::value % NSET;
        constexpr int k = m / NMT, i = (m % NMT) / TN, j = m % TN;
        float av, bv;
        if constexpr (TM == 2) av = a2[set][k][i]; else av = a1[set][k][i];
        if constexpr (TN == 2) bv = b2[set][k][j]; else bv = b1[set][k][j];
        acc[i][j] = __builtin_amdgcn_mfma_f32_32x32x2f32(av, bv, acc[i][j], 0, 0, 0);
    };

    if (nks > 0) {
#pragma unroll 1
        for (int s = 0; s < NS - 1; ++s)
            sl_static_for<NTASK>([&](auto qc) __attribute__((always_inline)) { task(qc, s); });
        sl_wait_vmcnt<(NS - 2) * LPW>();
        __builtin_amdgcn_s_barrier();
        __builtin_amdgcn_sched_barrier(0);
        sl_static_for<RD>([&](auto rc) __attribute__((always_inline)) { read_op(rc, SlInt<0>{}, a_lane, b_lane); });
        sl_static_for<RD>([&](auto rc) __attribute__((always_inline)) { read_op(rc, SlInt<1>{}, a_lane, b_lane); });
        int st = 0;
        for (int t = 0; t < nks; ++t) {
            const int st_next = st + 1 == NS ? 0 : st + 1, rs = st == 0 ? NS - 1 : st - 1;
            const unsigned a_st = a_lane + 4u * (unsigned)(st * SA), b_st = b_lane + 4u * (unsigned)(st * SB);
            const unsigned a_nx = a_lane + 4u * (unsigned)(st_next * SA), b_nx = b_lane + 4u * (unsigned)(st_next * SB);
            sl_static_for<G>([&](auto gc) __attribute__((always_inline)) {
                constexpr int gq = decltype(gc)::value;
                if constexpr (gq == G - AHEAD) {
                    sl_wait_lgkm<0>();
                    sl_wait_vmcnt<VMW>();
                    __builtin_amdgcn_s_barrier();
                    __builtin_amdgcn_sched_barrier(0);
                } else if constexpr (gq < G - AHEAD) {
                    sl_wait_lgkm<(AHEAD - 1) * RD>();
                }
                sl_static_for<NM>([&](auto mc) __attribute__((always_inline)) {
                    constexpr int m = decltype(mc)::value;
                    mfma_one(mc, gc);
                    __builtin_amdgcn_sched_barrier(0);
                    if constexpr (gq + AHEAD < G) read_slot(mc, SlInt<gq + AHEAD>{}, a_st, b_st);
                    else read_slot(mc, SlInt<gq + AHEAD - G>{}, a_nx, b_nx);
                    sl_static_for<NTASK>([&](auto qc) __attribute__((always_inline)) {
                        constexpr int q = decltype(qc)::value;
                        if constexpr (w2_task_slot(q, NSLOT, NTASK) == gq * NM + m) task(qc, rs);
                    });
                    __builtin_amdgcn_sched_barrier(0);
                });
            });
            st = st_next;
        }
        sl_wait_lgkm<0>();
        sl_wait_vmcnt<0>();
    }

    float* dst = out + (slab_stride ? (long)bz * slab_stride : 0);
    const bool direct_add = !slab_stride && accumulate;
#pragma unroll
    for (int i = 0; i < TM; ++i)
#pragma unroll
        for (int r = 0; r < 16; ++r) {
            const int rho = 4 * half + (r & 3) + 8 * (r >> 2);
            const int row = i0 + wm * 32 * TM + (TM == 2 ? 2 * rho + i : 32 * i + rho);
            if (row >= Ktot) continue;
            float* drow = dst + (long)row * g.cout;
            if (TN == 2 && !direct_add) {
                const int col = n0 + wn * 64 + 2 * l31;
                if (col + 1 < g.cout && (g.cout & 1) == 0) {
                    *reinterpret_cast<float2*>(drow + col) = make_float2(acc[i][0][r], acc[i][TN - 1][r]);
                    continue;
                }
            }
#pragma unroll
            for (int j = 0; j < TN; ++j) {
                const int col = n0 + wn * 32 * TN + (TN == 2 ? 2 * l31 + j : 32 * j + l31);
                if (col >= g.cout) continue;
                if (direct_add) unsafeAtomicAdd(drow + col, acc[i][j][r]);
                else drow[col] = acc[i][j][r];
            }
        }
}

template <int WM, int WN, int TM, int TN, int KB, int NS>
__global__ __launch_bounds__(256) void wgrad2_kernel(CnConvGeom g, const float* __restrict__ X, const float* __restrict__ GY,
                                                     float* __restrict__ out, long slab_stride, int rows_per_split, int tiles_x,
                                                     int tiles_y, int nsplits, int accumulate) {
    wgrad2_body<WM, WN, TM, TN, KB, NS>(g, X, GY, out, slab_stride, rows_per_split, tiles_x, tiles_y, nsplits, accumulate);
}

struct Wg2Tile {
    int cfg, bi, bn, kb;
    double e1, e2;
};
const Wg2Tile WG2_TILES[5] = {{0, 128, 128, 16, 0.72, 0.84}, {4, 128, 96, 16, 0.62, 0.72}, {2, 64, 64, 32, 0.50, 0.56},
                              {3, 128, 32, 32, 0.38, 0.42}, {5, 256, 64, 16, 0.55, 0.63}};

double wg2_cost(const Wg2Tile& t, long M, long Ktot, int cout, long s, long& rows_out, long& splits_out) {
    long rows = (M + s - 1) / s;
    rows = (rows + t.kb - 1) / t.kb * t.kb;
    const long splits = (M + rows - 1) / rows;
    rows_out = rows;
    splits_out = splits;
    const long tiles = (long)cn_cdiv(Ktot, t.bi) * cn_cdiv(cout, t.bn);
    const long per_xcd = splits >= 8 ? (long)cn_cdiv(splits, 8) * tiles : (long)cn_cdiv(tiles * splits, 8);
    const double cyc_row = 32.0 * (t.bi / 32) * (t.bn / 32) / 4.0;
    const double life = ((double)rows * cyc_row + 9000.0) / 2400.0;
    const long xcd_cus = cn_cu_count() >= 8 ? cn_cu_count() / 8 : 1;
    const long rounds = cn_cdiv(per_xcd, 2 * xcd_cus), rem = per_xcd - 2 * xcd_cus * (rounds - 1);
    double us = (double)(rounds - 1) * 2.0 * life / t.e2 + (rem <= xcd_cus ? life / t.e1 : 2.0 * life / t.e2);
    if (splits > 1) us += 2.0 * (double)splits * (double)Ktot * cout * 4.0 / 2.5e6 + 5.0;
    return us;
}

}

Wg2Plan cn_wgrad2_plan(const CnConvGeom& g, int forced, long target) {
    const long M = (long)g.n * g.out_d * g.out_h * g.out_w;
    const long Ktot = (long)g.k_d * g.k_h * g.k_w * g.cin;
    Wg2Plan p{};
    double best = -1.0;
    for (const Wg2Tile& t : WG2_TILES) {
        if (forced >= 0 ? t.cfg != forced
                        : ((t.cfg == 3) != (g.cout <= 32) || (t.cfg == 4 && g.cout % 96 != 0) || (t.cfg == 0 && g.cout < 96) ||
                           (t.cfg == 5 && (g.cout % 64 != 0 || Ktot < 256)) || (t.cfg != 2 && t.cfg != 3 && Ktot < 128)))
            continue;
        const long tiles = (long)cn_cdiv(Ktot, t.bi) * cn_cdiv(g.cout, t.bn);
        const long max_splits = cn_cdiv(M, 4 * t.kb);
        auto consider = [&](long s_) {
            if (s_ < 1) s_ = 1;
            if (s_ > max_splits) s_ = max_splits;
            long rows, splits;
            const double us = wg2_cost(t, M, Ktot, g.cout, s_, rows, splits);
            if (best < 0.0 || us < best) {
                best = us;
                p.cfg = t.cfg;
                p.tiles_x = cn_cdiv(Ktot, t.bi); p.tiles_y = cn_cdiv(g.cout, t.bn);
                p.rows = rows; p.splits = splits;
            }
        };
        if (target > 0) {
            consider(tiles >= target ? 1 : (target + tiles / 2) / tiles);
        } else {
            for (long s_ = 1; s_ < 8 && s_ <= max_splits; ++s_) consider(s_);
            for (long s_ = 8; s_ <= max_splits && s_ <= 1024; s_ += 8) consider(s_);
        }
    }
    return p;
}

bool cn_wgrad2_ok(const CnConvGeom& g) {
    const double xb = (double)g.n * g.in_d * g.in_h * g.in_w * g.cin * 4.0;
    const double yb = (double)g.n * g.out_d * g.out_h * g.out_w * g.cout * 4.0;
    const double sd = (double)g.in_h * g.in_w * g.cin, rows = (double)g.n * g.out_d * g.out_h * g.out_w;
    return g.cin % 4 == 0 && g.cout % 4 == 0 && g.cout > 4 && xb < 2147483647.0 && yb < 2147483647.0 &&
           g.dl_d == 1 && g.dl_h == 1 && g.dl_w == 1 && sd < 8388608.0 && rows < 8388608.0 && g.cout < 8388608;
}

void cn_wgrad2(int cfg, int ns, const CnConvGeom& g, const float* x, const float* gy, float* out, long slab_stride, int rows, int tiles_x,
               int tiles_y, int splits, int accumulate, unsigned grid, hipStream_t s) {
#define WG2(WM, WN, TM, TN, KB_, NS_) hipLaunchKernelGGL((wgrad2_kernel<WM, WN, TM, TN, KB_, NS_>), dim3(grid), dim3(256), 0, s, g, x, gy, out, slab_stride, \
                                                          rows, tiles_x, tiles_y, splits, accumulate)
#define WG2N(WM, WN, TM, TN, KB_) do { if (ns == 3) WG2(WM, WN, TM, TN, KB_, 3); else WG2(WM, WN, TM, TN, KB_, 4); } while (0)
    switch (cfg) {
        case 0: WG2N(2, 2, 2, 2, 16); break;
        case 4: WG2N(4, 1, 1, 3, 16); break;
        case 2: WG2N(2, 2, 1, 1, 32); break;
        case 5: WG2N(4, 1, 2, 2, 16); break;
        default: WG2(4, 1, 1, 1, 32, 3); break;
    }
#undef WG2N
#undef WG2
}
```

### confignet_amd/dnn_models/real_encoder.py

```python
import numpy as np
import torch

from .. import functional as F
from ..nn import Net, glorot_uniform, he_normal
from ..ops import ACT_TANH, ConvSpec

RESNET50_STACKS = [(64, 3, 1), (128, 4, 2), (256, 6, 2), (512, 3, 2)]
BN_EPS = 1.001e-5
C7 = ConvSpec((7, 7), stride=2, explicit_pad=3)
C1 = {1: ConvSpec((1, 1)), 2: ConvSpec((1, 1), stride=2)}
C3 = ConvSpec((3, 3))


def resnet50_layers():
    yield "conv1_conv", "conv", 3, 64, 7
    yield "conv1_bn", "bn", 0, 64, 0
    cin = 64
    for si, (f, blocks, _) in enumerate(RESNET50_STACKS):
        for bi in range(blocks):
            n = "conv%d_block%d" % (si + 2, bi + 1)
            yield n + "_1_conv", "conv", cin, f, 1
            yield n + "_1_bn", "bn", 0, f, 0
            yield n + "_2_conv", "conv", f, f, 3
            yield n + "_2_bn", "bn", 0, f, 0
            if bi == 0:
                yield n + "_0_conv", "conv", cin, 4 * f, 1
                yield n + "_3_conv", "conv", f, 4 * f, 1
                yield n + "_0_bn", "bn", 0, 4 * f, 0
                yield n + "_3_bn", "bn", 0, 4 * f, 0
            else:
                yield n + "_3_conv", "conv", f, 4 * f, 1
                yield n + "_3_bn", "bn", 0, 4 * f, 0
            cin = 4 * f


class RealEncoder(Net):
    def __init__(self, latent_dim, input_shape, rotation_ranges, rng=None):
        super().__init__()
        rng = rng or np.random.default_rng()
        where = {}
        for name, kind, cin, cout, k in resnet50_layers():
            where[name] = len(self._entries)
            if kind == "conv":
                self.add_weight(name + "/kernel", he_normal(rng, (k, k, cin, cout)))
                self.add_weight(name + "/bias", np.zeros(cout, np.float32))
            else:
                self.add_weight(name + "/gamma", np.full(cout, 0.25 if name.endswith("_3_bn") else 1.0, np.float32))
                self.add_weight(name + "/beta", np.zeros(cout, np.float32))
                self.add_weight(name + "/moving_mean", np.zeros(cout, np.float32), trainable=False)
                self.add_weight(name + "/moving_variance", np.ones(cout, np.float32), trainable=False)
        self._convs = []

        def conv_bn(prefix, spec):
            self._convs.append((where[prefix + "_conv"], where[prefix + "_bn"], spec))

        conv_bn("conv1", C7)
        for si, (filters, blocks, stride1) in enumerate(RESNET50_STACKS):
            for bi in range(blocks):
                n = "conv%d_block%d" % (si + 2, bi + 1)
                s = stride1 if bi == 0 else 1
                if bi == 0:
                    conv_bn(n + "_0", C1[s])
                conv_bn(n + "_1", C1[s])
                conv_bn(n + "_2", C3)
                conv_bn(n + "_3", C1[1])
        self.resnet_feature_dim = 2048
        self.add_weight("rotation_regressor/kernel", glorot_uniform(rng, (2048, 3)))
        self.add_weight("rotation_regressor/bias", np.zeros(3, np.float32))
        self.add_weight("feature_to_latent_mlp/kernel", glorot_uniform(rng, (2048, latent_dim)))
        self.add_weight("feature_to_latent_mlp/bias", np.zeros(latent_dim, np.float32))
        self.finalize()
        mult = np.pi * np.array([rotation_ranges[0][1], rotation_ranges[1][1], rotation_ranges[2][1]]) / 180.0
        self.rotation_range_multiplier = torch.tensor(mult, dtype=torch.float32, device=self.device)

    def _bn_coefficients(self, cat=False):
        ws = self.weights
        ks = [k for k, _, _ in self._convs]
        bs = [b for _, b, _ in self._convs]
        sizes = [ws[k + 1].shape[0] for k in ks]
        bias = torch.cat([ws[k + 1] for k in ks])
        gamma = torch.cat([ws[b] for b in bs])
        beta = torch.cat([ws[b + 1] for b in bs])
        if getattr(self, "_stat_cache", None) is None:
            self._stat_cache = (torch.cat([ws[b + 2] for b in bs]), torch.cat([ws[b + 3] for b in bs]))
        mean, var = self._stat_cache
        a = gamma * torch.rsqrt(var + BN_EPS)
        shift = beta + a * (bias - mean)
        if cat:
            return a, torch.split(shift, sizes)
        return torch.split(a, sizes), torch.split(shift, sizes)

    def non_trainable_changed(self):
        cache = getattr(self, "_stat_cache", None)
        if cache is not None:
            bs = [b for _, b, _ in self._convs]
            with torch.no_grad():
                cache[0].copy_(torch.cat([self.weights[b + 2] for b in bs]))
                cache[1].copy_(torch.cat([self.weights[b + 3] for b in bs]))

    def _fold_table(self):
        if getattr(self, "_fold_tab", None) is None:
            rows, views, dst, aoff = [], [], 0, 0
            base = self.arena.data_ptr()
            for kidx, _, _ in self._convs:
                w = self.weights[kidx]
                src = (w.data_ptr() - base) // 4
                assert 0 <= src and src % 4 == 0 and w.numel() % 4 == 0 and w.shape[-1] % 4 == 0 and w.is_contiguous()
                rows.append((src, dst, w.numel(), w.shape[-1], aoff))
                views.append((dst, tuple(w.shape)))
                dst += w.numel()
                aoff += w.shape[-1]
            self._fold_tab = (torch.tensor(rows, dtype=torch.int32, device=self.device), dst, views)
        return self._fold_tab

    def _folded_filters(self, a_cat):
        from ..nn import WEIGHTS_EPOCH
        from .. import ops
        stream = torch.cuda.current_stream().cuda_stream
        key = (WEIGHTS_EPOCH[0], self.epoch)
        cache = self.__dict__.setdefault("_fold_cache", {})
        c = cache.get(stream)
        if c is None or c[0] != key:
            for k in [k for k, v in cache.items() if v[0] != key]:
                del cache[k]
            seg, total, views = self._fold_table()
            packed = ops.scale_columns_segments(self.arena, seg, a_cat, total)
            c = cache[stream] = (key, [packed[o:o + int(np.prod(shp))].view(shp) for o, shp in views], packed)
        if ops._keepalive is not None:
            ops._keepalive.append(c[2])
        return c[1]

    def _features_folded(self, img):
        from .. import ops
        from ..ops import ACT_NONE, ACT_RELU
        a, shift = self._bn_coefficients(cat=True)
        wf = self._folded_filters(a)

        def conv(ci, x, res=None, relu=True):
            spec = self._convs[ci][2]
            g = spec.geom(tuple(x.shape), wf[ci].shape[-1])
            if res is None:
                return ops.conv_fwd(x, wf[ci], shift[ci], g, ACT_RELU if relu else ACT_NONE)
            return ops.conv_fwd_res(x, wf[ci], shift[ci], res, g, ACT_RELU)

        x = F.caffe_preprocess(img)
        x = conv(0, x)
        x = F.maxpool(x, 3, 2, 1)
        ci = 1
        for filters, blocks, stride1 in RESNET50_STACKS:
            for bi in range(blocks):
                if bi == 0:
                    sc = conv(ci, x, relu=False)
                    ci += 1
                else:
                    sc = x
                y = conv(ci, x)
                y = conv(ci + 1, y)
                x = conv(ci + 2, y, res=sc)
                ci += 3
        return F.global_avg_pool(x)

    def _fold_table9(self):
        if getattr(self, "_fold_tab9", None) is None:
            seg = self._fold_table()[0].cpu().numpy()
            base = self.arena.data_ptr()
            rows, blk = [], 0
            for (kidx, bidx, _), r in zip(self._convs, seg):
                cout = int(r[3])
                assert cout % 64 == 0
                offs = [(self.weights[i].data_ptr() - base) // 4 for i in (kidx + 1, bidx, bidx + 1)]
                assert all(o >= 0 and o % 4 == 0 for o in offs)
                rows.append(list(map(int, r)) + offs + [blk])
                blk += cout // 64
            self._fold_tab9 = (torch.tensor(rows, dtype=torch.int32, device=self.device), blk)
        return self._fold_tab9

    def _fold_coefficients(self):
        ws = self.weights
        ks = [k for k, _, _ in self._convs]
        bs = [b for _, b, _ in self._convs]
        with torch.no_grad():
            if getattr(self, "_stat_cache", None) is None:
                self._stat_cache = (torch.cat([ws[b + 2] for b in bs]), torch.cat([ws[b + 3] for b in bs]))
            mean, var = self._stat_cache
            rs = torch.rsqrt(var + BN_EPS)
            a = torch.cat([ws[b] for b in bs]) * rs
            bm = torch.cat([ws[k + 1] for k in ks]) - mean
            shift = torch.addcmul(torch.cat([ws[b + 1] for b in bs]), a, bm)
        return a, shift, rs, bm

    def _trunk_params(self):
        return [w for w in self.weights[:-4] if w.requires_grad]

    folded_tape = True

    def _conv_bn(self, ci, x, coef, res=None, relu=True):
        kidx, _, spec = self._convs[ci]
        z = F.conv(x, self.weights[kidx], None, spec)
        return F.channel_affine_act(z, coef[0][ci], coef[1][ci], res, relu)

    fold_inference = True

    def features(self, img):
        if self.fold_inference and not torch.is_grad_enabled() and img.dtype == torch.float32:
            from .. import ops
            if ops.ACT_DTYPE == torch.float32:
                return self._features_folded(img)
        from .. import ops as _ops
        if self.folded_tape and torch.is_grad_enabled() and (_ops.ACT_DTYPE == torch.float32 or self.folded_tape == "always"):
            params = self._trunk_params()
            if len(params) == sum(1 for i in self._trainable_idx if i < len(self.weights) - 4) or (not params and img.requires_grad):
                x = F.caffe_preprocess(img)
                return F.global_avg_pool(ResNetTrunkFn.apply(self, x, *params))
        coef = self._bn_coefficients()
        x = F.caffe_preprocess(img)
        x = self._conv_bn(0, x, coef)
        x = F.maxpool(x, 3, 2, 1)
        ci = 1
        for filters, blocks, stride1 in RESNET50_STACKS:
            for bi in range(blocks):
                if bi == 0:
                    sc = self._conv_bn(ci, x, coef, relu=False)
                    ci += 1
                else:
                    sc = x
                y = self._conv_bn(ci, x, coef)
                y = self._conv_bn(ci + 1, y, coef)
                x = self._conv_bn(ci + 2, y, coef, res=sc, relu=True)
                ci += 3
        return F.global_avg_pool(x)

    def __call__(self, input_img):
        feat = self.features(self.to_device(input_img))
        w = self.weights
        rot = F.linear(feat, w[-4], w[-3], ACT_TANH) * self.rotation_range_multiplier
        return F.linear(feat, w[-2], w[-1]), rot

    def predict(self, imgs, batch_size=32):
        embs, rots = [], []
        with torch.no_grad():
            for s in range(0, len(imgs), batch_size):
                e, r = self(imgs[s:s + batch_size])
                embs.append(e.cpu().numpy())
                rots.append(r.cpu().numpy())
        return np.concatenate(embs), np.concatenate(rots)


class ResNetTrunkFn(torch.autograd.Function):

    @staticmethod
    def forward(ctx, enc, x, *params):
        from .. import ops
        from ..ops import ACT_NONE, ACT_RELU
        a, shift, rs, bm = enc._fold_coefficients()
        wf = enc._folded_filters(a)
        sizes = [wf[ci].shape[-1] for ci in range(len(enc._convs))]
        offs = [0]
        for c in sizes:
            offs.append(offs[-1] + c)
        sh = [shift[offs[i]:offs[i + 1]] for i in range(len(sizes))]
        x = x.contiguous()

        def conv(ci, t, res=None, relu=True):
            g = enc._convs[ci][2].geom(tuple(t.shape), sizes[ci])
            if res is None:
                return ops.conv_fwd(t, wf[ci], sh[ci], g, ACT_RELU if relu else ACT_NONE)
            return ops.conv_fwd_res(t, wf[ci], sh[ci], res, g, ACT_RELU)

        saved = [x]
        y0 = conv(0, x)
        t = ops.maxpool_fwd(y0, 3, 2, 1)
        saved += [y0, t]
        ci = 1
        for filters, blocks, stride1 in RESNET50_STACKS:
            for bi in range(blocks):
                sc = t
                if bi == 0:
                    sc = conv(ci, t, relu=False)
                    ci += 1
                y1 = conv(ci, t)
                y2 = conv(ci + 1, y1)
                t = conv(ci + 2, y2, res=sc)
                saved += [y1, y2, t]
                ci += 3
        ctx.enc, ctx.coef, ctx.wf, ctx.offs = enc, (a, rs, bm), wf, offs
        ctx.save_for_backward(*saved)
        return t

    @staticmethod
    def backward(ctx, gy):
        from .. import ops
        from ..ops import ACT_RELU
        if torch.is_grad_enabled():
            raise RuntimeError("ResNetTrunkFn is first-order only")
        enc, wf, offs = ctx.enc, ctx.wf, ctx.offs
        a, rs, bm = ctx.coef
        saved = list(ctx.saved_tensors)
        seg5, total, views = enc._fold_table()
        seg9, blocks = enc._fold_table9()
        dev = gy.device
        params = enc._trunk_params()
        want_w = any(ctx.needs_input_grad[2:]) and not F._INPUT_GRADS_ONLY
        sunk = want_w and ops.sink_for(params[0]) is not None
        gwf = gsh = None
        if want_w:
            gwf = torch.empty(total, device=dev, dtype=torch.float32)
            gsh = ops.zero_pool_alloc((offs[-1],), dev)
            if gsh is None:
                gsh = torch.zeros(offs[-1], device=dev, dtype=torch.float32)

        def geom(ci, t):
            return enc._convs[ci][2].geom(tuple(t.shape), wf[ci].shape[-1])

        def wgrad(ci, t_in, gu):
            o, shp = views[ci]
            if want_w:
                ops.sink_conv_wgrad_to(t_in, gu, geom(ci, t_in), shp, gwf[o:o + int(np.prod(shp))].view(shp), defer=sunk)

        def relu_bwd(ci, g, y, also=None):
            if not want_w:
                return ops.act_bwd(g, y, ACT_RELU)
            gu, part = ops.act_bwd_partials(g, y, ACT_RELU)
            ops.sum_rows_into(part, gsh[offs[ci]:offs[ci + 1]], defer=sunk)
            if also is not None:
                ops.sum_rows_into(part, gsh[offs[also]:offs[also + 1]], defer=sunk)
            return gu

        g = gy.contiguous()
        layout = []
        ci = 1
        for filters, blocks_, stride1 in RESNET50_STACKS:
            for bi in range(blocks_):
                layout.append((ci, bi == 0))
                ci += 4 if bi == 0 else 3
        pos = len(saved)
        for first, has_sc in reversed(layout):
            y1, y2, t_out = saved[pos - 3], saved[pos - 2], saved[pos - 1]
            pos -= 3
            t_in = saved[pos - 1]
            c1 = first + 1 if has_sc else first
            gu3 = relu_bwd(c1 + 2, g, t_out, also=first if has_sc else None)
            wgrad(c1 + 2, y2, gu3)
            gu2 = relu_bwd(c1 + 1, ops.conv_dgrad(gu3, wf[c1 + 2], geom(c1 + 2, y2)), y2)
            wgrad(c1 + 1, y1, gu2)
            gu1 = relu_bwd(c1, ops.conv_dgrad(gu2, wf[c1 + 1], geom(c1 + 1, y1)), y1)
            wgrad(c1, t_in, gu1)
            if has_sc:
                wgrad(first, t_in, gu3)
                skip = ops.conv_dgrad(gu3, wf[first], geom(first, t_in))
            else:
                skip = gu3
            g = ops.conv_dgrad_res(gu1, wf[c1], geom(c1, t_in), skip)
        x, y0, t = saved[0], saved[1], saved[2]
        g = ops.maxpool_bwd(y0, g, 3, 2, 1)
        gu0 = relu_bwd(0, g, y0)
        wgrad(0, x, gu0)
        gx = ops.conv_dgrad(gu0, wf[0], geom(0, x)) if ctx.needs_input_grad[1] else None
        if not want_w:
            return (None, gx) + (None,) * len(params)
        if sunk:
            gout = enc.grad_arena
            ops.sink_post(lambda: ops.bn_fold_bwd(seg9, blocks, gwf, gsh, enc.arena, a, rs, bm, gout), keep=(gwf, gsh, a, rs, bm))
            return (None, gx) + (None,) * len(params)
        gout = torch.zeros_like(enc.arena)
        ops.bn_fold_bwd(seg9, blocks, gwf, gsh, enc.arena, a, rs, bm, gout)
        base = enc.arena.data_ptr()
        grads = []
        for p_ in params:
            o = (p_.data_ptr() - base) // 4
            grads.append(gout[o:o + p_.numel()].view(p_.shape))
        return (None, gx) + tuple(grads)
```

### confignet_amd/ops.py

```python
import contextlib
import ctypes
import math
import os
import threading

import torch

from ._lib import CN_BF16, CN_EUNSUPPORTED, CN_F32, CN_U8, CnConvGeom, CnDepthJob, CnGanJob, CnRowsJob, CnSumJob, check, lib

ACT_NONE, ACT_LRELU, ACT_RELU, ACT_TANH, ACT_RELU6, ACT_SIGMOID = 0, 1, 2, 3, 4, 5

ACT_DTYPE = torch.float32


def set_activation_dtype(dtype):
    global ACT_DTYPE
    if isinstance(dtype, str):
        dtype = {"f32": torch.float32, "fp32": torch.float32, "float32": torch.float32, "bf16": torch.bfloat16,
                 "bfloat16": torch.bfloat16}[dtype]
    assert dtype in (torch.float32, torch.bfloat16)
    ACT_DTYPE = dtype


def _stream():
# ... 199 lines not shown
        p3 = (ctypes.c_int * 3)(g.p_d, g.p_h, g.p_w)
        k2, p2 = (ctypes.c_int * 3)(), (ctypes.c_int * 3)()
        wd_ = _c(wd_)
        ks = [g.k_d, g.k_h, g.k_w]
        sizes = [1 if (g.nd == 2 and i == 0) else (ks[i] + 1 if ks[i] >= 3 else 3) for i in range(3)]
        t2 = sizes[0] * sizes[1] * sizes[2]
        both = torch.empty((2, t2 * g.cin * g.cout), device=wd_.device, dtype=torch.float32)
        check(lib.cn_upfold_weights(_fptr(wd_), _ptr(both[0]), _ptr(both[1]), g.nd, k3, p3, g.cin, g.cout, k2, p2, _stream()),
              "cn_upfold_weights")
        assert list(k2) == sizes, (list(k2), sizes)
        return both[0], both[1], tuple(k2), tuple(p2)
    wf, wd, (kd, kh, kw), (pd, ph, pw) = _weight_cache(w, "_cn_upfold_%d_%d%d%d_%d%d%d" % (g.nd, g.k_d, g.k_h, g.k_w, g.p_d, g.p_h, g.p_w), make)
    gd = _copy_geom(g, k_d=kd, k_h=kh, k_w=kw, dl_d=(2 if g.nd == 3 else 1), dl_h=2, dl_w=2,
                    p_d=kd - 1 - pd, p_h=kh - 1 - ph, p_w=kw - 1 - pw, up=0)
    g2 = _copy_geom(g, in_d=g.out_d, in_h=g.out_h, in_w=g.out_w, cin=g.cout, out_d=g.in_d, out_h=g.in_h, out_w=g.in_w,
                    cout=g.cin, k_d=kd, k_h=kh, k_w=kw, s_d=(2 if g.nd == 3 else 1), s_h=2, s_w=2, p_d=pd, p_h=ph, p_w=pw, up=0)
    taps = (kd, kh, kw) if g.nd == 3 else (kh, kw)
    return wf.view(taps + (g.cin, g.cout)), wd.view(taps + (g.cout, g.cin)), gd, g2


def upfold_wgrad(gw2, g, w_shape, out=None, single_writer=False):
    gw = out if out is not None else torch.empty(w_shape, device=gw2.device, dtype=torch.float32)
    k3 = (ctypes.c_int * 3)(g.k_d, g.k_h, g.k_w)
    p3 = (ctypes.c_int * 3)(g.p_d, g.p_h, g.p_w)
    mode = 0 if out is None else (2 if single_writer else 1)
    check(lib.cn_upfold_wgrad(_fptr(_c(gw2)), _ptr(gw), g.nd, k3, p3, g.cin, g.cout, mode, _stream()), "cn_upfold_wgrad")
    return gw


WINOGRAD = True
WINO_MIN_WGS = 32
WINO_MIN_FILL = 0.7


def _wino_ok(g, cin, cout):
    if not (WINOGRAD and g.nd == 2 and g.k_h == 3 and g.k_w == 3 and g.s_h == 1 and g.s_w == 1 and g.dl_h == 1 and g.dl_w == 1
            and g.up == 0 and g.p_h == 1 and g.p_w == 1 and g.out_h == g.in_h and g.out_w == g.in_w):
        return False
    if cin % 16 or cout % 64:
        return False
    th, tw = (g.in_h + 1) // 2, (g.in_w + 1) // 2
    bh, bw = (th + 7) // 8, (tw + 7) // 8
    if th * tw < WINO_MIN_FILL * (bh * bw * 64):
        return False
    return g.n * bh * bw * (cout // 64) >= WINO_MIN_WGS


WINO4 = True
WINO4_MIN_WGS = 128


def _wino4_ok(g, cin, cout):
    if not (WINO4 and WINOGRAD and g.nd == 2 and g.k_h == 3 and g.k_w == 3 and g.s_h == 1 and g.s_w == 1 and g.dl_h == 1 and g.dl_w == 1
            and g.up == 0 and g.p_h == 1 and g.p_w == 1 and g.out_h == g.in_h and g.out_w == g.in_w):
        return False
    if g.in_h % 16 or g.in_w % 32 or cin % 16 or cout % 64:
        return False
    return g.n * (g.in_h // 16) * (g.in_w // 32) * (cout // 64) >= WINO4_MIN_WGS


def _wino4_filter(w, dgrad):
    def make(wd_):
        wd_ = _c(wd_)
        cin, cout = wd_.shape[-2], wd_.shape[-1]
        u = torch.empty((36, cout, cin) if dgrad else (36, cin, cout), device=wd_.device, dtype=torch.float32)
        check(lib.cn_conv_wino4_filter(_fptr(wd_), _ptr(u), cin, cout, int(dgrad), _stream()), "cn_conv_wino4_filter")
        return u
    return _weight_cache(w, "_cn_wino4_d" if dgrad else "_cn_wino4_f", make)


def wino4_saved_flops(g):
    tiles = g.n * (g.in_h // 4) * (g.in_w // 4)
    return 2.0 * g.cin * g.cout * (9.0 * g.n * g.in_h * g.in_w - 36.0 * tiles)


def _wino_filter(w, dgrad):
    def make(wd_):
        wd_ = _c(wd_)
        cin, cout = wd_.shape[-2], wd_.shape[-1]
        u = torch.empty((16, cout, cin) if dgrad else (16, cin, cout), device=wd_.device, dtype=torch.float32)
        check(lib.cn_conv_wino_filter(_fptr(wd_), _ptr(u), cin, cout, int(dgrad), _stream()), "cn_conv_wino_filter")
        return u
    return _weight_cache(w, "_cn_wino_d" if dgrad else "_cn_wino_f", make)


class _StatsSlot(threading.local):
    request = None
    ready = None


_stats = _StatsSlot()
STATS_FUSION = True


class request_stats:
    def __init__(self, kind, slope=0.0):
        self.req = (kind, float(slope))

    def __enter__(self):
        self.prev, _stats.request = _stats.request, (self.req if STATS_FUSION and not DETERMINISTIC else None)

    def __exit__(self, *exc):
        _stats.request = self.prev


def take_stats(y, kind):
    ent, _stats.ready = _stats.ready, None
    if ent is not None and ent[0] == y.data_ptr() and ent[1] == tuple(y.shape) and ent[2] == kind:
        return ent[3]
    return None


def conv_fwd(x, w, bias, g, act=ACT_NONE, slope=0.0):
    req, _stats.request = _stats.request, None
    _stats.ready = None
    out_dtype = _act_out_dtype(g.cout)
    if ACT_DTYPE == torch.float32 and x.dtype == torch.float32 and _wino4_ok(g, g.cin, g.cout):
        y = torch.empty(geom_out_shape(g), device=x.device, dtype=torch.float32)
        check(lib.cn_conv_fwd_wino4(g.n, g.in_h, g.in_w, g.cin, g.cout, _ptr(_c(x)), _ptr(_wino4_filter(w, False)), _fptr(bias), _ptr(y),
                                    act, slope, _stream()), "cn_conv_fwd_wino4")
        prof_note_saved(wino4_saved_flops(g))
        return y
    if ACT_DTYPE == torch.float32 and x.dtype == torch.float32 and _wino_ok(g, g.cin, g.cout):
        y = torch.empty(geom_out_shape(g), device=x.device, dtype=torch.float32)
        check(lib.cn_conv_fwd_wino(g.n, g.in_h, g.in_w, g.cin, g.cout, _ptr(x), _ptr(_wino_filter(w, False)), _fptr(bias), _ptr(y),
                                   act, slope, _stream()), "cn_conv_fwd_wino")
        prof_note_saved(wino_saved_flops(g))
        return y
    if _bf16_conv_ok(g):
        x = cast(x, torch.bfloat16)
        y = torch.empty(geom_out_shape(g), device=x.device, dtype=torch.bfloat16)
        wf, _ = weight_prep_bf16(w)
        check(lib.cn_conv_fwd_bf16(ctypes.byref(g), _ptr(x), _ptr(wf), _fptr(bias), _ptr(y), act, slope, _stream()), "cn_conv_fwd_bf16")
        return y
    x = f32(x)
    if out_dtype == torch.bfloat16 and MIXED_FIRST_LAYERS and g.cin == 3:
        y = torch.empty(geom_out_shape(g), device=x.device, dtype=torch.bfloat16)
        rc = lib.cn_conv_fwd_dt(ctypes.byref(g), _ptr(x), CN_F32, _fptr(w), _fptr(bias), _ptr(y), CN_BF16, act, slope, _stream())
        if rc == 0:
            return y
        if rc != CN_EUNSUPPORTED:
            check(rc, "cn_conv_fwd_dt")
    y = torch.empty(geom_out_shape(g), device=x.device, dtype=torch.float32)
    if req is not None and out_dtype == torch.float32 and g.cout % 4 == 0 and (req[0] == "act" or act == ACT_NONE):
        nk = 2 if req[0] == "act" else 4
        mark = _active_pool.cur if _active_pool is not None else None
        st = zero_pool_alloc((nk, g.n, g.cout), x.device)
        if st is not None:
            rc = lib.cn_conv_fwd_stats(ctypes.byref(g), _ptr(_c(x)), _fptr(w), _fptr(bias), _ptr(y), act, slope, _ptr(st), 1 if nk == 2 else 2,
                                       req[1], _stream())
            if rc == 0:
                _stats.ready = (y.data_ptr(), tuple(y.shape), req[0], tuple(st[k] for k in range(nk)))
                return y
            if rc != CN_EUNSUPPORTED:
                check(rc, "cn_conv_fwd_stats")
            _active_pool.cur = mark
    check(lib.cn_conv_fwd(ctypes.byref(g), _ptr(x), _fptr(w), _fptr(bias), _ptr(y), act, slope, _stream()), "cn_conv_fwd")
    return cast(y, out_dtype)


W4_EP_POOL, W4_EP_POOL_ONLY, W4_EP_MASK = 1, 2, 3


def conv_fwd_pool(x, w, bias, g, act=ACT_NONE, slope=0.0, keep_full=True):
    if not (ACT_DTYPE == torch.float32 and x.dtype == torch.float32 and _wino4_ok(g, g.cin, g.cout)):
        return None
    _stats.request = _stats.ready = None
    y = torch.empty(geom_out_shape(g), device=x.device, dtype=torch.float32) if keep_full else None
    pooled = torch.empty((g.n, g.in_h // 2, g.in_w // 2, g.cout), device=x.device, dtype=torch.float32)
    check(lib.cn_conv_fwd_wino4_ep(g.n, g.in_h, g.in_w, g.cin, g.cout, _ptr(_c(x)), _ptr(_wino4_filter(w, False)), _fptr(bias), _ptr(y),
                                   act, slope, W4_EP_POOL if keep_full else W4_EP_POOL_ONLY, _ptr(pooled), None, None, None, 1, 0.0,
                                   _stream()), "cn_conv_fwd_wino4_ep")
    prof_note_saved(wino4_saved_flops(g))
    return y, pooled


def conv_dgrad_masked(gy, w, g, y, target=None, s=None, k=0.0):
    if not (ACT_DTYPE == torch.float32 and gy.dtype == torch.float32 and y.dtype == torch.float32 and _wino4_ok(g, g.cout, g.cin)):
        return None
    if target is not None and (target.dtype != torch.float32 or s is None or s.numel() not in (1, g.n)):
        return None
    _log_mask(y, ACT_RELU)
    gu = torch.empty(geom_in_shape(g, upsampled=True), device=gy.device, dtype=torch.float32)
    check(lib.cn_conv_fwd_wino4_ep(g.n, g.in_h, g.in_w, g.cout, g.cin, _ptr(_c(gy)), _ptr(_wino4_filter(w, True)), None, _ptr(gu),
                                   ACT_NONE, 0.0, W4_EP_MASK, None, _ptr(_c(y)), None if target is None else _ptr(_c(target)),
                                   None if target is None else _fptr(s), 1 if target is None else s.numel(), k, _stream()),
          "cn_conv_fwd_wino4_ep")
    prof_note_saved(wino4_saved_flops(g))
    return gu


def conv_fwd_res(x, w, bias, res, g, act=ACT_NONE, slope=0.0):
    assert act in (ACT_NONE, ACT_RELU)
    if ACT_DTYPE == torch.float32 and x.dtype == torch.float32 and res.dtype == torch.float32 and not _wino_ok(g, g.cin, g.cout):
        x, res = _c(x), _c(res)
        y = torch.empty(geom_out_shape(g), device=x.device, dtype=torch.float32)
        rc = lib.cn_conv_fwd_res(ctypes.byref(g), _ptr(x), _fptr(w), _fptr(bias), _ptr(res), _ptr(y), act, slope, _stream())
        if rc == 0:
            return y
        if rc != CN_EUNSUPPORTED:
            check(rc, "cn_conv_fwd_res")
    y = conv_fwd(x, w, bias, g)
    return nc_lin2(tuple(y.shape), y, None, res, None, None, flags=8 if act == ACT_RELU else 0)


def scale_columns_segments(src, seg, a, total):
    dst = torch.empty(total, device=src.device, dtype=torch.float32)
    check(lib.cn_scale_columns_segments(_fptr(src), _ptr(dst), _ptr(seg), _fptr(_c(a)), seg.shape[0], total, _stream()),
          "cn_scale_columns_segments")
    return dst


def weight_tflip(w):
    w = _c(w)
    taps = int(math.prod(w.shape[:-2]))
    wt = torch.empty(w.shape[:-2] + (w.shape[-1], w.shape[-2]), device=w.device, dtype=torch.float32)
    check(lib.cn_conv_weight_tflip(_fptr(w), _ptr(wt), taps, w.shape[-2], w.shape[-1], _stream()), "cn_conv_weight_tflip")
    return wt


def conv_dgrad(gy, w, g):
    shape = geom_in_shape(g, upsampled=True)
    if _bf16_conv_ok(g):
        gy = cast(gy, torch.bfloat16)
        gu = torch.empty(shape, device=gy.device, dtype=torch.bfloat16)
        _, wd = weight_prep_bf16(w)
        check(lib.cn_conv_dgrad_bf16(ctypes.byref(g), _ptr(gy), _ptr(wd), _ptr(gu), _stream()), "cn_conv_dgrad_bf16")
        return gu
    if gy.dtype == torch.bfloat16 and MIXED_FIRST_LAYERS and g.cin == 3:
        gu = torch.empty(shape, device=gy.device, dtype=torch.float32)
        wt = _weight_cache(w, "_cn_tflip", weight_tflip)
        rc = lib.cn_conv_dgrad_dt(ctypes.byref(g), _ptr(_c(gy)), CN_BF16, _fptr(wt), _ptr(gu), CN_F32, _stream())
        if rc == 0:
            return cast(gu, _act_out_dtype(g.cin))
        if rc != CN_EUNSUPPORTED:
            check(rc, "cn_conv_dgrad_dt")
    gy = f32(gy)
    gu = torch.empty(shape, device=gy.device, dtype=torch.float32)
    if ACT_DTYPE == torch.float32 and _wino4_ok(g, g.cout, g.cin):
        check(lib.cn_conv_fwd_wino4(g.n, g.in_h, g.in_w, g.cout, g.cin, _ptr(_c(gy)), _ptr(_wino4_filter(w, True)), None, _ptr(gu),
                                    ACT_NONE, 0.0, _stream()), "cn_conv_fwd_wino4")
        prof_note_saved(wino4_saved_flops(g))
        return gu
    if ACT_DTYPE == torch.float32 and _wino_ok(g, g.cout, g.cin):
        check(lib.cn_conv_fwd_wino(g.n, g.in_h, g.in_w, g.cout, g.cin, _ptr(gy), _ptr(_wino_filter(w, True)), None, _ptr(gu),
                                   ACT_NONE, 0.0, _stream()), "cn_conv_fwd_wino")
        prof_note_saved(wino_saved_flops(g))
        return gu
    if DGRAD_FROM_W:
        rc = lib.cn_conv_dgrad_w(ctypes.byref(g), _ptr(gy), _fptr(_c(w)), _ptr(gu), _stream())
        if rc == 0:
            return cast(gu, _act_out_dtype(g.cin))
        if rc != CN_EUNSUPPORTED:
            check(rc, "cn_conv_dgrad_w")
    wt = _weight_cache(w, "_cn_tflip", weight_tflip)
    check(lib.cn_conv_dgrad(ctypes.byref(g), _ptr(gy), _fptr(wt), _ptr(gu), _stream()), "cn_conv_dgrad")
    return cast(gu, _act_out_dtype(g.cin))


def conv_dgrad_res(gy, w, g, res):
    if (ACT_DTYPE == torch.float32 and gy.dtype == torch.float32 and res.dtype == torch.float32 and DGRAD_FROM_W and not g.up
            and not _wino4_ok(g, g.cout, g.cin) and not _wino_ok(g, g.cout, g.cin)):
        gu = torch.empty(geom_in_shape(g, upsampled=True), device=gy.device, dtype=torch.float32)
        rc = lib.cn_conv_dgrad_w_res(ctypes.byref(g), _ptr(_c(gy)), _fptr(_c(w)), _ptr(_c(res)), _ptr(gu), _stream())
        if rc == 0:
            return gu
        if rc != CN_EUNSUPPORTED:
            check(rc, "cn_conv_dgrad_w_res")
    gu = conv_dgrad(gy, w, g)
    return nc_lin2(tuple(gu.shape), gu, None, res, None, None)


DGRAD_FROM_W = True
MIXED_FIRST_LAYERS = True
WGRAD_WRITE, WGRAD_ADD, WGRAD_ZEROED = 0, 1, 2


def conv_wgrad(x, gy, g, w_shape, out=None, accumulate=True, defer=True, ws=None):
    gw, mode = out, WGRAD_ADD if accumulate else WGRAD_WRITE
    if out is None:
        gw, mode = zero_pool_alloc(w_shape, x.device), WGRAD_ZEROED
        if gw is None:
            gw, mode = torch.empty(w_shape, device=x.device, dtype=torch.float32), WGRAD_WRITE
    x = _c(cast(x, torch.bfloat16 if _bf16_conv_ok(g) else torch.float32))
    nbytes = ctypes.c_size_t(0)
    rc = lib.cn_conv_wgrad_dt_workspace_bytes(ctypes.byref(g), _dt(x), _dt(gy), ctypes.byref(nbytes))
    if rc == CN_EUNSUPPORTED and gy.dtype != x.dtype:
        gy = cast(gy, x.dtype)
        rc = lib.cn_conv_wgrad_dt_workspace_bytes(ctypes.byref(g), _dt(x), _dt(gy), ctypes.byref(nbytes))
    check(rc, "cn_conv_wgrad_dt_workspace_bytes")
    gy, nbytes = _c(gy), nbytes.value
    if ws is None:
        ws = torch.empty(nbytes // 4, device=x.device, dtype=torch.float32) if nbytes else None
    else:
        assert ws.dtype == torch.float32 and ws.numel() * 4 >= nbytes, "conv_wgrad: workspace of %d bytes, %d needed" % (ws.numel() * 4, nbytes)
    parts = ctypes.c_int(0) if nbytes and out is not None and _SINK is not None and defer else None
    check(lib.cn_conv_wgrad_dt(ctypes.byref(g), _ptr(x), _dt(x), _ptr(gy), _dt(gy), _fptr(gw), mode, _ptr(ws), nbytes,
                               None if parts is None else ctypes.byref(parts), _stream()), "cn_conv_wgrad_dt")
    if parts is not None and parts.value:
        _SINK.slabs.append((ws, gw, parts.value, gw.numel(), int(mode != WGRAD_WRITE)))
    return gw


GRAD_SINK = True
_SINK = None


def sink_rounds(jobs, key):
    rounds, seen = [], {}
    for job in jobs:
        k = key(job)
        r = seen.get(k, 0)
        seen[k] = r + 1
        if r == len(rounds):
            rounds.append([])
        rounds[r].append(job)
    return rounds


class _Sink:

    def __init__(self, params):
        self.slots = {p.data_ptr(): p.grad for p in params if p.grad is not None}
        self.touched = []
        self.slabs = []
        self.depth = []
        self.upfold = {}
        self.post = []
        self.post_keep = []

    def note_stream(self):
        cur = torch.cuda.current_stream()
        if all(cur != s_ for s_ in self.touched):
            self.touched.append(cur)


def _sum_slabs_grouped(slabs):
    for batch in sink_rounds(slabs, lambda job: job[1].data_ptr()):
        jobs = (CnSumJob * len(batch))()
        for q, (ws, dst, parts, count, acc) in zip(jobs, batch):
            q.src, q.dst, q.count, q.parts, q.accumulate = ws.data_ptr(), dst.data_ptr(), count, parts, acc
        check(lib.cn_sum_parts_grouped(jobs, len(batch), _stream()), "cn_sum_parts_grouped")


def _gemm_depth_grouped(depth):
    for batch in sink_rounds(depth, lambda job: job[2].data_ptr()):
        jobs = (CnDepthJob * len(batch))()
        for q, (a, b, slot) in zip(jobs, batch):
            q.a, q.b, q.c = a.data_ptr(), b.data_ptr(), slot.data_ptr()
            q.m, q.n, q.k, q.lda, q.ldb, q.ldc = a.shape[1], b.shape[1], a.shape[0], a.shape[1], b.shape[1], b.shape[1]
        check(lib.cn_gemm_depth_grouped(jobs, len(batch), _stream()), "cn_gemm_depth_grouped")


def _release_operands(cur, others, operands):
    if not torch.cuda.is_current_stream_capturing():
        for t in operands:
            t.record_stream(cur)
    for s_ in others:
        s_.wait_stream(cur)


class grad_sink:
    def __init__(self, params):
        self.params = params

    def __enter__(self):
        global _SINK
        assert _SINK is None, "nested gradient sinks"
        if GRAD_SINK and self.params:
            _SINK = _Sink(self.params)
        return self

    def join(self):
        st = _SINK
        if st is None:
            return
        cur = torch.cuda.current_stream()
        others = [s_ for s_ in st.touched if s_ != cur]
        for s_ in others:
            cur.wait_stream(s_)
        slabs, depth, upfold, post, post_keep = st.slabs, st.depth, st.upfold, st.post, st.post_keep
        st.touched, st.slabs, st.depth, st.upfold, st.post, st.post_keep = [], [], [], {}, [], []
        _sum_slabs_grouped(slabs)
        _gemm_depth_grouped(depth)
        if slabs or depth:
            _release_operands(cur, others, [j[0] for j in slabs] + [t for j in depth for t in j[:2]])
        for gw2, g, w_shape, slot in upfold.values():
            upfold_wgrad(gw2, g, w_shape, out=slot, single_writer=True)
        for fn in post:
            fn()
        if post:
            _release_operands(cur, others, post_keep)
        if st.slabs or st.depth or st.upfold or st.post:
            raise RuntimeError("a sink_post function queued work on the gradient sink after its join")

    def __exit__(self, exc_type, exc, tb):
        global _SINK
        try:
            if exc_type is None:
                self.join()
        finally:
            _SINK = None


def sink_for(w):
    if _SINK is None or w is None:
        return None
    return _SINK.slots.get(w.data_ptr())


def sink_conv_wgrad(x, gy, g, w_shape, slot):
    if _SINK is not None:
        _SINK.note_stream()
    conv_wgrad(x, gy, g, w_shape, out=slot)


def sink_conv_wgrad_to(x, gy, g, w_shape, dst, defer=True):
    if _SINK is not None:
        _SINK.note_stream()
    conv_wgrad(x, gy, g, w_shape, out=dst, accumulate=False, defer=defer)


def sink_post(fn, keep=()):
    st = _SINK
    if st is None:
        fn()
        return
    st.note_stream()
    st.post_keep.extend(t for t in keep if t is not None)
    st.post.append(fn)


def bn_fold_bwd(seg9, blocks, gwf, gshift, arena, a, rs, bm, gout):
    check(lib.cn_bn_fold_bwd(_ptr(seg9), seg9.shape[0], blocks, _fptr(gwf), _fptr(gshift), _fptr(arena), _fptr(a), _fptr(rs), _fptr(bm),
                             _fptr(gout), _stream()), "cn_bn_fold_bwd")


def sink_upfold_wgrad(gy, x, g2, wd_shape, g, w_shape, slot):
    st = _SINK
    ent = st.upfold.get(slot.data_ptr())
    if ent is None:
        gw2 = zero_pool_alloc(wd_shape, x.device)
        if gw2 is None:
            gw2 = torch.zeros(wd_shape, device=x.device, dtype=torch.float32)
        ent = st.upfold[slot.data_ptr()] = (gw2, g, w_shape, slot)
    st.note_stream()
    conv_wgrad(gy, x, g2, wd_shape, out=ent[0])


def sink_gemm(a, b, slot, trans_a=False, trans_b=False):
    st = _SINK
    if st is not None:
        st.note_stream()
        if (trans_a and not trans_b and a.shape[0] <= 32 and a.dtype == torch.float32 and b.dtype == torch.float32
                and a.is_contiguous() and b.is_contiguous() and slot.is_contiguous()):
            st.depth.append((a, b, slot))
            return
    gemm_acc(a, b, slot, trans_a, trans_b)


class _ZeroPool:
    def __init__(self, device, numel):
        self.buf = torch.zeros(numel, device=device, dtype=torch.float32)
        self.cur = 0
        self.dirty = 0


_pools = {}
_active_pool = None
ZERO_POOL_FLOATS = 96 * 1024 * 1024


def zero_pool_begin(name, device):
    global _active_pool
    p = _pools.get((name, device))
    if p is None:
        p = _pools[(name, device)] = _ZeroPool(device, ZERO_POOL_FLOATS)
    if p.dirty:
        p.buf[:p.dirty].zero_()
    p.cur = 0
    _active_pool = p


def zero_pool_end():
    global _active_pool
    if _active_pool is not None:
        _active_pool.dirty = max(_active_pool.dirty, _active_pool.cur)
    _active_pool = None


def zero_pool_alloc(shape, device):
    p = _active_pool
    if p is None or p.buf.device != device:
        return None
    n = int(math.prod(shape))
    n4 = (n + 3) // 4 * 4
    if p.cur + n4 > p.buf.numel():
        return None
    out = p.buf[p.cur:p.cur + n].view(shape)
    p.cur += n4
    return out


def _sums(shape, device):
    t = zero_pool_alloc(shape, device)
    if t is not None:
        return t, 16
    return torch.empty(shape, device=device, dtype=torch.float32), 0


def zero_(t):
    check(lib.cn_zero(_fptr(t), t.numel() * 4, _stream()), "cn_zero")
    return t


def sumpool2(gu):
    nd = gu.dim() - 2
    sp = [s // 2 for s in gu.shape[1:-1]]
    gx = torch.empty((gu.shape[0], *sp, gu.shape[-1]), device=gu.device, dtype=gu.dtype)
    d, h, w = ([1] + sp) if nd == 2 else sp
    check(lib.cn_sumpool2(_ptr(gu), _ptr(gx), nd, gu.shape[0], d, h, w, gu.shape[-1], _dt(gu), _stream()), "cn_sumpool2")
    return gx


def gemm(a, b, trans_a=False, trans_b=False, bias=None, act=ACT_NONE, slope=0.0):
    m = a.shape[1] if trans_a else a.shape[0]
    k = a.shape[0] if trans_a else a.shape[1]
    n = b.shape[0] if trans_b else b.shape[1]
    kb = b.shape[1] if trans_b else b.shape[0]
    assert k == kb, "gemm inner dims %d vs %d" % (k, kb)
    a, b = f32(a), f32(b)
    c = torch.empty((m, n), device=a.device, dtype=torch.float32)
    check(lib.cn_gemm(int(trans_a), int(trans_b), m, n, k, _ptr(a), a.shape[1], _ptr(b), b.shape[1], _ptr(c), n,
                      _ptr(bias), act, slope, _stream()), "cn_gemm")
    return c


def gemm_acc(a, b, out, trans_a=False, trans_b=False):
    m = a.shape[1] if trans_a else a.shape[0]
    k = a.shape[0] if trans_a else a.shape[1]
    n = b.shape[0] if trans_b else b.shape[1]
    a, b = f32(a), f32(b)
    assert tuple(out.shape) == (m, n) and out.is_contiguous()
    check(lib.cn_gemm_acc(int(trans_a), int(trans_b), m, n, k, _ptr(a), a.shape[1], _ptr(b), b.shape[1], _fptr(out), n, _stream()),
          "cn_gemm_acc")
    return out


def _nsc(x):
    n, c = x.shape[0], x.shape[-1]
    return n, x.numel() // (n * c), c


def nc_reduce(x1, x2=None, want_sum=True, want_dot=True, flags=0, slope=0.0, per_channel=False, x2_period=0):
    x1, x2 = _unify(x1, x2)
    n, s, c = _nsc(x1)
    assert not (x2_period and per_channel)
    flags |= x2_period << 8
    rep = 1
    if per_channel:
        rep, s, c = _spread(x1)
        n = rep
    sums, flag = _sums((int(want_sum) + int(want_dot), n, c), x1.device)
    s1, s2 = (sums[0] if want_sum else None), (sums[-1] if want_dot else None)
    check(lib.cn_nc_reduce(_ptr(x1), _ptr(x2), _ptr(s1), _ptr(s2), n, s, c, flags | flag, slope, _dt(x1), _stream()), "cn_nc_reduce")
    sums = _readd(sums, rep, 1)
    return (sums[0] if want_sum else None), (sums[-1] if want_dot else None)


def nc_reduce4(x, slope):
    n, s, c = _nsc(x)
    out, flags = _sums((4, n, c), x.device)
    check(lib.cn_nc_reduce4(_ptr(x), _ptr(out), n, s, c, slope, flags, _dt(x), _stream()), "cn_nc_reduce4")
    return out[0], out[1], out[2], out[3]


def nc_lin2(shape, x1=None, a1=None, x2=None, a2=None, b=None, flags=0, slope=0.0, per_channel=False, a3=None, b3=None,
            x2_period=0, out=None):
    n, c = shape[0], shape[-1]
    s = int(math.prod(shape)) // (n * c)
    x1, x2 = _unify(x1, x2)
    if flags & 4:
        _log_mask(x2)
    ref = x1 if x1 is not None else (x2 if x2 is not None else b)
    dtype = ref.dtype if (x1 is not None or x2 is not None) else _act_out_dtype(c)
    if out is not None:
        assert out.is_contiguous() and out.numel() == int(math.prod(shape))
        if out.dtype != dtype:
            x1, x2 = (None if x1 is None else cast(x1, out.dtype)), (None if x2 is None else cast(x2, out.dtype))
        y = out
    else:
        y = torch.empty(shape, device=ref.device, dtype=dtype)
    flags |= x2_period << 8
    check(lib.cn_nc_lin2(_ptr(x1), _fptr(a1), _ptr(x2), _fptr(a2), _fptr(b), _fptr(a3), _fptr(b3), _ptr(y), n, s, c,
                         0 if per_channel else c, flags, slope, _dt(y), _stream()), "cn_nc_lin2")
    return y


NORM_ADAIN, NORM_INSTANCE, NORM_STYLE = 0, 1, 2


def norm_coef_fwd(mode, s1, s2, p1, p2, spatial, eps, x=None):
    n, c = s1.shape
    A = torch.empty((n, 2 * c) if mode == NORM_STYLE else (n, c), device=s1.device, dtype=torch.float32)
    B = torch.empty((n, c), device=s1.device, dtype=torch.float32) if mode != NORM_STYLE else None
    mean = torch.empty((n, c), device=s1.device, dtype=torch.float32)
    r = torch.empty((n, c), device=s1.device, dtype=torch.float32)
    check(lib.cn_norm_coef_fwd(mode, _ptr(s1), _ptr(s2), _ptr(p1), _ptr(p2), _ptr(A), _ptr(B), _ptr(mean), _ptr(r),
                               n, c, spatial, eps, _ptr(x), CN_F32 if x is None else _dt(x), _stream()), "cn_norm_coef_fwd")
    return A, B, mean, r


def norm_coef_bwd(mode, t1, t2, mean, r, p1, spatial, eps):
    n, c = mean.shape
    dev = mean.device
    c1 = torch.empty((n, c), device=dev, dtype=torch.float32) if mode != NORM_STYLE else None
    c2 = torch.empty((n, c), device=dev, dtype=torch.float32)
    c0 = torch.empty((n, c), device=dev, dtype=torch.float32)
    gp1 = gp2 = None
    if mode == NORM_ADAIN:
        gp1 = torch.empty((n, 2 * c), device=dev, dtype=torch.float32)
    elif mode == NORM_INSTANCE:
        gp1 = torch.empty((c,), device=dev, dtype=torch.float32)
        gp2 = torch.empty((c,), device=dev, dtype=torch.float32)
    check(lib.cn_norm_coef_bwd(mode, _ptr(t1), _ptr(t2), _ptr(mean), _ptr(r), _ptr(p1), _ptr(c1), _ptr(c2), _ptr(c0),
                               _ptr(gp1), _ptr(gp2), n, c, spatial, eps, _stream()), "cn_norm_coef_bwd")
    return c1, c2, c0, gp1, gp2


NORM_APPLY = True


def norm_apply_fwd(mode, x, s1, s2, p1, p2, eps, flags=0, slope=0.0):
    if not NORM_APPLY or x.shape[-1] % 4 or x.dtype != torch.float32:
        return None
    n, s, c = _nsc(x)
    y = torch.empty_like(x)
    mean = torch.empty((n, c), device=x.device, dtype=torch.float32)
    r = torch.empty_like(mean)
    rc = lib.cn_norm_apply(mode, 0, _ptr(x), None, _fptr(s1), _fptr(s2), _fptr(_c(p1)), _fptr(None if p2 is None else _c(p2)), _ptr(mean), _ptr(r),
                           None, None, None, None, _ptr(y), n, s, c, eps, flags, slope, _dt(x), _stream())
    if rc == CN_EUNSUPPORTED:
        return None
    check(rc, "cn_norm_apply")
    return y, mean, r


def norm_apply_bwd(mode, gy, x, t1, t2, mean, r, p1, eps, flags=0, slope=0.0, a3=None, b3=None):
    if not NORM_APPLY or x.shape[-1] % 4 or x.dtype != torch.float32 or gy.dtype != torch.float32:
        return None
    gy, x = _unify(gy, x)
    n, s, c = _nsc(x)
    if flags & 4:
        _log_mask(x)
    gx = torch.empty_like(x)
    if mode == NORM_ADAIN:
        gp1, gp2 = torch.empty((n, 2 * c), device=x.device, dtype=torch.float32), None
    else:
        gp1 = torch.empty((c,), device=x.device, dtype=torch.float32)
        gp2 = torch.empty_like(gp1)
    rc = lib.cn_norm_apply(mode, 1, _ptr(gy), _ptr(x), _fptr(t1), _fptr(t2), _fptr(_c(p1)), None, _ptr(mean), _ptr(r), _ptr(gp1), _ptr(gp2),
                           _fptr(a3), _fptr(b3), _ptr(gx), n, s, c, eps, flags, slope, _dt(x), _stream())
    if rc == CN_EUNSUPPORTED:
        return None
    check(rc, "cn_norm_apply")
    return gx, gp1, gp2


def dual_tail_coef_fwd(T, U, mean, q, sm, ssd, gamma, spatial, eps=1e-3):
    ref = mean if mean is not None else sm
    period, c = ref.shape
    mk = lambda *sh: torch.empty(sh, device=ref.device, dtype=torch.float32)
    C1 = C2 = C0 = ts = None
    n_inst = n_style = 0
    if T is not None:
        n_inst = T[0].shape[0]
        C1, C2, C0 = mk(n_inst, c), mk(n_inst, c), mk(n_inst, c)
    if U is not None:
        n_style = U[0].shape[0]
        ts = mk(n_style, 2 * c)
    T1, T2 = T if T is not None else (None, None)
    U1, U2 = U if U is not None else (None, None)
    check(lib.cn_dual_tail_coef_fwd(_ptr(T1), _ptr(T2), _ptr(U1), _ptr(U2), _ptr(mean), _ptr(q), _ptr(sm), _ptr(ssd),
                                    _ptr(gamma), _ptr(C1), _ptr(C2), _ptr(C0), _ptr(ts), n_inst + n_style, c, spatial, eps,
                                    n_style, period, _stream()),
          "cn_dual_tail_coef_fwd")
    return C1, C2, C0, ts


def dual_tail_coef_bwd(H, E, u, T, U, mean, q, sm, ssd, gamma, spatial, eps=1e-3):
    ref = mean if mean is not None else sm
    period, c = ref.shape
    names = ["K1", "K2", "K0", "D2", "D0", "kh", "kt", "ka", "kc", "et", "ex", "e0", "ggamma", "ggamma_rows"]
    out = {k: None for k in names}
    mk = lambda *sh: torch.empty(sh, device=ref.device, dtype=torch.float32)
    n_inst = n_style = 0
    if H is not None:
        n_inst = H[0].shape[0]
        for k in ("K1", "K2", "K0", "kh", "kt", "ka", "kc", "ggamma_rows"):
            out[k] = mk(n_inst, c)
        out["ggamma"] = mk(c)
    if u is not None:
        n_style = u.shape[0]
        for k in ("D2", "D0", "et", "ex", "e0"):
            out[k] = mk(n_style, c)
    arr = (ctypes.c_void_p * 14)(*[(out[k].data_ptr() if out[k] is not None else None) for k in names])
    H1, H2p = H if H is not None else (None, None)
    T1, T2 = T if T is not None else (None, None)
    U1, U2 = U if U is not None else (None, None)
    check(lib.cn_dual_tail_coef_bwd(_ptr(H1), _ptr(H2p), _ptr(E), _ptr(u), _ptr(T1), _ptr(T2), _ptr(U1), _ptr(U2),
                                    _ptr(mean), _ptr(q), _ptr(sm), _ptr(ssd), _ptr(gamma), arr, n_inst + n_style, c, spatial, eps,
                                    n_style, period, _stream()),
          "cn_dual_tail_coef_bwd")
    return out


def dual_tail_gx(h, ta, tx, x, co, slope):
    h, ta, tx, x = _unify(h, ta, tx, x)
    _log_mask(x)
    n, s, c = _nsc(x)
    nrep = 1 if h is None else h.shape[0] // n
    assert h is None or (h.shape[0] == nrep * n and ta.shape[0] == nrep * n)
    out = torch.empty_like(x)
    check(lib.cn_dual_tail_gx(_ptr(h), _ptr(ta), _ptr(tx), _ptr(x), _ptr(co["kh"]), _ptr(co["kt"]), _ptr(co["ka"]),
                              _ptr(co["kc"]), _ptr(co["et"]), _ptr(co["ex"]), _ptr(co["e0"]), _ptr(out), n, s, c, slope,
                              nrep, _dt(x), _stream()), "cn_dual_tail_gx")
    return out


def dual_tail_gx_tx(h, ta, tx, x, co, slope, ta_is_tx=False):
    h, ta, tx, x = _unify(h, ta, tx, x)
    _log_mask(x)
    n, s, c = _nsc(x)
    nrep = h.shape[0] // n
    assert h.shape[0] == nrep * n and ta.shape[0] == nrep * n and tx.shape[0] == (nrep + 1) * n
    out = torch.empty_like(x)
    out_tx = torch.empty_like(tx)
    check(lib.cn_dual_tail_gx_tx(_ptr(h), _ptr(ta), _ptr(tx), _ptr(x), _ptr(co["kh"]), _ptr(co["kt"]), _ptr(co["ka"]), _ptr(co["kc"]),
# ... 567 lines not shown
```

### include/confignet_hip.h

```cpp
#ifndef CONFIGNET_HIP_H
#define CONFIGNET_HIP_H
#include <stddef.h>
#include <stdint.h>

#ifdef __cplusplus
extern "C" {
#endif

#define CN_OK 0
#define CN_EINVAL (-1)
#define CN_EHIP (-2)
#define CN_EUNSUPPORTED (-3)

#define CN_F32 0
#define CN_BF16 1
#define CN_U8 2

#define CN_ACT_NONE 0
#define CN_ACT_LRELU 1
#define CN_ACT_RELU 2
#define CN_ACT_TANH 3
#define CN_ACT_RELU6 4
#define CN_ACT_SIGMOID 5

typedef struct CnConvGeom {
    int nd, n;
    int in_d, in_h, in_w, cin;
    int out_d, out_h, out_w, cout;
    int k_d, k_h, k_w;
    int s_d, s_h, s_w;
    int dl_d, dl_h, dl_w;
    int p_d, p_h, p_w;
    int up;
} CnConvGeom;

const char* cn_last_error_string(void);
int cn_version(void);

int cn_conv_fwd(const CnConvGeom* g, const float* x, const float* w, const float* bias,
                float* y, int act, float slope, void* stream);
int cn_conv_fwd_stats(const CnConvGeom* g, const float* x, const float* w, const float* bias, float* y, int act, float slope,
                      float* stats, int stats_mode, float stats_slope, void* stream);
int cn_conv_fwd_res(const CnConvGeom* g, const float* x, const float* w, const float* bias, const float* res, float* y,
                    int act, float slope, void* stream);
int cn_conv_weight_tflip(const float* w, float* w_tflip, int taps, int cin, int cout, void* stream);
int cn_conv_dgrad(const CnConvGeom* g, const float* gy, const float* w_tflip, float* gu, void* stream);
int cn_conv_dgrad_w(const CnConvGeom* g, const float* gy, const float* w, float* gu, void* stream);
int cn_conv_dgrad_w_res(const CnConvGeom* g, const float* gy, const float* w, const float* res, float* gu, void* stream);
int cn_conv_wgrad(const CnConvGeom* g, const float* x, const float* gy, float* gw, int accumulate, void* stream);
size_t cn_conv_wgrad_workspace_bytes(const CnConvGeom* g);
int cn_conv_wgrad_ws(const CnConvGeom* g, const float* x, const float* gy, float* gw, int accumulate, void* workspace,
                     size_t workspace_bytes, void* stream);
int cn_conv_wgrad_ws_slabs(const CnConvGeom* g, const float* x, const float* gy, float* gw, int accumulate, void* workspace,
                           size_t workspace_bytes, int* parts, void* stream);
#define CN_WGRAD_WRITE 0
#define CN_WGRAD_ADD 1
#define CN_WGRAD_ZEROED 2
int cn_conv_wgrad_dt_workspace_bytes(const CnConvGeom* g, int x_dt, int gy_dt, size_t* bytes);
int cn_conv_wgrad_dt(const CnConvGeom* g, const void* x, int x_dt, const void* gy, int gy_dt, float* gw, int mode, void* workspace,
                     size_t workspace_bytes, int* parts, void* stream);
int cn_conv_wgrad_plan(const CnConvGeom* g, int x_dt, int gy_dt, int caller_slabs, unsigned routes, int det, long long out[12]);
typedef struct CnSumJob {
    const float* src;
    float* dst;
    long long count;
    int parts;
    int accumulate;
} CnSumJob;
int cn_sum_parts_grouped(const CnSumJob* jobs, int njobs, void* stream);
typedef struct CnDepthJob {
    const float* a;
    const float* b;
    float* c;
    int m, n, k, lda, ldb, ldc;
} CnDepthJob;
int cn_gemm_depth_grouped(const CnDepthJob* jobs, int njobs, void* stream);
typedef struct CnRowsJob {
    const float* a;
    const float* b;
    float* c;
    const float* bias;
    const float* mask;
    int m, n, k, lda, ldb, ldc, tb, act, accumulate;
    float slope;
} CnRowsJob;
int cn_gemm_rows_grouped(const CnRowsJob* jobs, int njobs, void* stream);
int cn_gemm_rows_grouped_k(const CnRowsJob* jobs, int njobs, void* stream);
int cn_gemm_rows_grouped_plan(const CnRowsJob* jobs, int njobs, int* out, int cap, int* nlaunches);
typedef struct CnGanJob {
    const float* s;
    float* out;
    const float* gout;
    int n;
    float label;
} CnGanJob;
int cn_gan_loss_grouped(const CnGanJob* jobs, int njobs, int backward, void* stream);
int cn_conv_fwd_dt(const CnConvGeom* g, const void* x, int x_dt, const float* w, const float* bias, void* y, int y_dt, int act,
                   float slope, void* stream);
int cn_conv_dgrad_dt(const CnConvGeom* g, const void* gy, int gy_dt, const float* w_tflip, void* gu, int gu_dt, void* stream);
int cn_conv_wgrad_c3_partials(void);
int cn_conv_wgrad_c3(const CnConvGeom* g, const float* x, const void* gy, int gy_dt, float* scratch, float* gw, int accumulate,
                     void* stream);
int cn_conv_wgrad_thin_partials(void);
int cn_conv_wgrad_thin(const CnConvGeom* g, const float* x, const float* gy, float* scratch, float* gw, int accumulate, void* stream);
int cn_conv_wino_filter(const float* w, float* u, int cin, int cout, int dgrad, void* stream);
int cn_conv_fwd_wino(int n, int h, int w, int cin, int cout, const float* x, const float* u, const float* bias, float* y,
                     int act, float slope, void* stream);
int cn_conv_wino4_filter(const float* w, float* u, int cin, int cout, int dgrad, void* stream);
int cn_conv_fwd_wino4(int n, int h, int w, int cin, int cout, const float* x, const float* u, const float* bias,
                      float* y, int act, float slope, void* stream);
#define CN_W4_EP_POOL 1
#define CN_W4_EP_POOL_ONLY 2
#define CN_W4_EP_MASK 3
int cn_conv_fwd_wino4_ep(int n, int h, int w, int cin, int cout, const float* x, const float* u, const float* bias, float* y,
                         int act, float slope, int mode, float* pooled, const float* ym, const float* target, const float* s,
                         int s_rows, float k, void* stream);
int cn_conv_tune(int cfg, int splits, long wg_blocks);
int cn_conv_fwd_plan(const CnConvGeom* g, int bt, int has_bias, int act, int has_res, int stats_mode, int x_dt, int y_dt, int out[8]);
int cn_conv_loop_select(int loop, int kb, int ns, int np);
int cn_fwd2_col_block(int cfg, int bt, int gathered, int n, int kb, int np);
int cn_sumpool2(const void* gu, void* gx, int nd, int n, int d, int h, int w, int c, int dt, void* stream);

int cn_conv_weight_prep_bf16(const float* w, uint16_t* wf, uint16_t* wd, int taps, int cin, int cout, void* stream);
int cn_conv_fwd_bf16(const CnConvGeom* g, const uint16_t* x, const uint16_t* wf, const float* bias, uint16_t* y,
                     int act, float slope, void* stream);
int cn_conv_dgrad_bf16(const CnConvGeom* g, const uint16_t* gy, const uint16_t* wd, uint16_t* gu, void* stream);
int cn_conv_wgrad_bf16(const CnConvGeom* g, const uint16_t* x, const uint16_t* gy, float* gw, int accumulate, void* stream);
int cn_upfold_weights(const float* w, float* wf, float* wd, int nd, const int* k3, const int* pad_lo3, int cin, int cout,
                      int* k2_out3, int* pad2_out3, void* stream);
int cn_upfold_wgrad(const float* gw2, float* gw, int nd, const int* k3, const int* pad_lo3, int cin, int cout,
                    int accumulate, void* stream);
int cn_cast(const void* src, int src_dt, void* dst, int dst_dt, size_t numel, void* stream);

int cn_gemm(int trans_a, int trans_b, int m, int n, int k, const float* a, int lda,
            const float* b, int ldb, float* c, int ldc, const float* bias, int act, float slope,
            void* stream);
int cn_gemm_plan(int trans_a, int trans_b, int m, int n, int k, int ldc, int has_bias, int act, int accumulate, int deterministic,
                 int out[9]);

int cn_set_deterministic(int on);
int cn_get_deterministic(void);
int cn_det_release_stream(void* stream);
int cn_zero(void* p, size_t bytes, void* stream);
int cn_gemm_acc(int trans_a, int trans_b, int m, int n, int k, const float* a, int lda, const float* b, int ldb,
                float* c, int ldc, void* stream);
int cn_sum_rows_into(const float* src, float* dst, int rows, int cols, int accumulate, void* stream);

int cn_nc_reduce_plan(int n, int s, int c, int nsums, int prezeroed, int det, int out[8]);
int cn_nc_reduce4(const void* x, float* out, int n, int s, int c, float slope, int flags, int dt, void* stream);
int cn_nc_reduce(const void* x1, const void* x2, float* sum1, float* sum2, int n, int s, int c,
                 int flags, float slope, int dt, void* stream);
int cn_nc_reduce_dact(const void* x1, const void* x2, float* sum1, float* sum2, void* dact_out, int n, int s, int c,
                      int flags, float slope, int act, int dt, void* stream);
int cn_bn_act_bwd(const void* gy, const void* y, const void* x, const float* a, void* g_out, void* gx, float* sum_g,
                  float* sum_gx, int n, int s, int c, int act, int flags, int dt, void* stream);
int cn_nc_lin2(const void* x1, const float* a1, const void* x2, const float* a2, const float* bb,
               const float* a3, const float* b3, void* y, int n, int s, int c, int cstride, int flags,
               float slope, int dt, void* stream);
int cn_nc_rows_plan(long long G, int CG, int ny, int out[2]);

int cn_norm_coef_fwd(int mode, const float* s1, const float* s2, const float* p1, const float* p2, float* A,
                     float* B, float* save_mean, float* save_r, int n, int c, int S, float eps, const void* x, int dt,
                     void* stream);
int cn_norm_coef_bwd(int mode, const float* t1, const float* t2, const float* save_mean, const float* save_r,
                     const float* p1, float* c1, float* c2, float* c0, float* gp1, float* gp2, int n, int c,
                     int S, float eps, void* stream);
int cn_norm_apply(int mode, int dir, const void* x1, const void* x2, const float* sa, const float* sb, const float* p1,
                  const float* p2, float* save_mean, float* save_r, float* gp1, float* gp2, const float* a3, const float* b3,
                  void* y, int n, int s, int c, float eps, int flags, float slope, int dt, void* stream);

int cn_dual_tail_coef_fwd(const float* T1, const float* T2, const float* U1, const float* U2, const float* mean,
                          const float* q, const float* sm, const float* ssd, const float* gamma, float* C1,
                          float* C2, float* C0, float* tstyle, int n, int c, int S, float eps, int n_style, int period,
                          void* stream);
int cn_dual_tail_coef_bwd(const float* H1, const float* H2p, const float* E, const float* u, const float* T1,
                          const float* T2, const float* U1, const float* U2, const float* mean, const float* q,
                          const float* sm, const float* ssd, const float* gamma, float* const* out13, int n, int c,
                          int S, float eps, int n_style, int period, void* stream);
int cn_dual_tail_gx(const void* h, const void* ta, const void* tx, const void* x, const float* kh,
                    const float* kt, const float* ka, const float* kc, const float* et, const float* ex,
                    const float* e0, void* out, int n, int s, int c, float slope, int nrep, int dt, void* stream);
int cn_dual_tail_gx_tx(const void* h, const void* ta, const void* tx, const void* x, const float* kh, const float* kt,
                       const float* ka, const float* kc, const float* et, const float* ex, const float* e0,
                       const float* K1, const float* K2, const float* K0, const float* D2, const float* D0, void* out,
                       void* out_tx, int n, int s, int c, float slope, int nrep, int ta_is_tx, int dt, void* stream);
int cn_nc_reduce_hxt(const void* h, const void* x, const void* ta, float* out, int n, int s, int c, float slope, int period,
                     int flags, int dt, void* stream);

int cn_act_fwd(const void* x, void* y, size_t numel, int act, float slope, int dt, void* stream);
int cn_act_bwd(const void* gy, const void* y, void* gx, size_t numel, int act, float slope, int dt, void* stream);
int cn_act_bwd_bias(const void* gy, const void* y, void* gx, float* gb, int n, int s, int c, int act, float slope, int flags,
                    int dt, void* stream);
int cn_axpby(const void* x, const void* y, void* out, size_t numel, float a, float b, int dt, void* stream);
int cn_mul(const void* x, const void* y, void* out, size_t numel, int dt, void* stream);
int cn_sqdiff_sum(const void* a, const void* b, float* out, size_t numel, float scale, int dt, void* stream);
int cn_row_sumsq(const float* x, float* out, int n, size_t row, void* stream);
int cn_row_scale(const void* x, const float* s, void* out, int n, size_t row, float k, int dt, void* stream);
int cn_row_scale_diff(const void* x, const void* x2, const float* s, void* out, int n, size_t row, float k, int dt, void* stream);
int cn_tap_bwd(const void* y, const void* target, const void* g, const float* s, void* out, int n, size_t row, float k,
               int act, float slope, int dt, void* stream);
int cn_maxpool2_bwd_act(const void* x, const void* gy, const void* target, const float* s, float k, void* gx, int n, int h,
                        int w, int c, int s_rows, int dt, void* stream);
int cn_stream_plan(int op, int dt, long long rows, size_t row, int c, int h, int w, int k, int s, int pad, unsigned aligned, int det,
                   long long out[4]);
int cn_stream_plan_ptrs(int op, int dt, int dst_dt, long long rows, size_t row, int c, int h, int w, int k, int s, int pad,
                        const void* const ptrs[4], int det, long long out[4]);
int cn_stream_last_plan(long long out[5]);
int cn_masked_diff(const float* a, const float* b, const uint8_t* mask, float* out, size_t pixels, int c, void* stream);
int cn_maxpool_fwd(const void* x, void* y, int n, int h, int w, int c, int k, int s, int pad, int dt, void* stream);
int cn_maxpool_bwd(const void* x, const void* gy, void* gx, int n, int h, int w, int c, int k, int s, int pad, int dt, void* stream);
int cn_avgpool3_same(const void* x, void* y, int n, int h, int w, int c, int dt, void* stream);
int cn_dwconv3x3_fwd(const float* x, const float* w, const float* bias, float* y, int n, int h, int wd, int c, int stride,
                     int act, float slope, void* stream);
int cn_image_preprocess(const void* x, int x_dt, float* y, int n, int h, int wd, int c, int oh, int ow, float in_mul, float in_add,
                        void* stream);
int cn_dwconv3x3_dgrad(const float* gy, const float* w, float* gx, int n, int h, int wd, int c, int stride, void* stream);
int cn_dwconv3x3_wgrad_slices(int n, int h, int wd, int c, int stride);
int cn_dwconv3x3_wgrad(const float* x, const float* gy, float* part, int slices, int n, int h, int wd, int c, int stride, void* stream);
int cn_bn_train_coef(const float* s1, const float* s2, const float* gamma, const float* beta, const float* x, float* mean, float* var,
                     float* r, float* a, float* b, float* moving_mean, float* moving_var, long long m, int c, float eps,
                     double momentum, int bessel, void* stream);
int cn_bn_train_apply(const float* x, const float* a, const float* b, float* y, long long m, int c, int act, void* stream);
int cn_bn_train_bwd_slices(long long m, int c);
int cn_chan_slices_plan(long long rows, int c, int min_rows, int out[5]);
int cn_bn_train_bwd_reduce(const float* gy, const float* y, const float* x, const float* mean, const float* r, float* part, int slices,
                           long long m, int c, int act, void* stream);
int cn_bn_train_bwd_apply(const float* gy, const float* y, const float* x, const float* mean, const float* r, const float* a,
                          const float* sums, float* gx, long long m, int c, int act, void* stream);
int cn_chan_affine3_fwd(const float* x, float* y, size_t pixels, const int* perm, float scale, const float* off, void* stream);
int cn_chan_affine3_bwd(const float* gy, float* gx, size_t pixels, const int* perm, float scale, void* stream);
int cn_gan_loss_fwd(const float* s, float* out, int n, float label, void* stream);
int cn_gan_loss_bwd(const float* s, const float* gout, float* gs, int n, float label, void* stream);

int cn_euler_matrix(const float* angles, float* rot, int n, void* stream);
int cn_euler_matrix_bwd(const float* angles, const float* grot, float* gangles, int n, void* stream);
int cn_rotate3d_fwd(const float* grid, const float* rot , float* out, int n, int g, int c, void* stream);
int cn_rotate3d_bwd(const float* grid, const float* rot, const float* gout, float* ggrid, float* grot,
                    int n, int g, int c, void* stream);
int cn_rotate3d_bwd_plan(int n, int g, int c, int det, int out[4]);

int cn_adam_step(float* theta, const float* grad, float* m, float* v, float* ema, size_t numel,
                 const float* lr_t, float beta1, float beta2, float eps, float ema_alpha, void* stream);
int cn_ema_step(float* ema, const float* theta, size_t numel, float alpha, void* stream);

int cn_gather_images_u8(const uint8_t* pool, const int64_t* idx, const uint8_t* flip, float* out,
                        int n, int h, int w, int c, void* stream);
int cn_to_uint8(const float* x, uint8_t* out, size_t numel, void* stream);
int cn_scale_columns_segments(const float* src, float* dst, const int* seg, const float* a, int nseg, size_t total, void* stream);
int cn_bn_fold_bwd(const int* seg, int nseg, int blocks, const float* gwf, const float* gshift, const float* arena,
                   const float* a, const float* rs, const float* bm, float* gout, void* stream);

int cn_hdri_rows_v(const float* x, float* v, const int* y0, const float* wy, int pool, int h, int w, int oh, int t_len,
                   void* stream);
int cn_hdri_rows_h(const float* v, float* out, const int* idx, const int* shift, const int* x0, const float* wx,
                   const float* mean, int n, int pool, int w, int oh, int ow, int t_len, void* stream);
int cn_exp2m1(const float* x, float* y, size_t numel, void* stream);

int cn_warp_affine_u8(const uint8_t* src, uint8_t* dst, const int* x0, const int* y0, const int* adelta, const int* bdelta,
                      int n, int sh, int sw, int c, int oh, int ow, void* stream);
int cn_warp_nearest_f32(const float* src, float* dst, const int* x0, const int* y0, const int* adelta, const int* bdelta,
                        int n, int sh, int sw, int c, int oh, int ow, void* stream);
int cn_eye_mask(const float* uv, uint8_t* mask, size_t pixels, int c, float l_min, float l_max, float r_min, float r_max,
                float y_min, float y_max, void* stream);

int cn_prof_enable(int on);
int cn_prof_reset(void);
int cn_prof_collect(int* launches, double* total_ms, double* total_flops);
int cn_prof_collect_by_family(int* launches, double* ms, double* flops, double* bytes);

int cn_spin(unsigned long long ticks, void* stream);

#ifdef __cplusplus
}
#endif
#endif
```

Before: 428.3 images/sec.

## Group encoder filter-gradient convs into multi-job launches and split BN-fold backward

Encoder conv weight gradients that the LDS-DMA wgrad2 kernel can take are collected and issued as grouped launches. Each launch carries up to 24 jobs in its kernel arguments and each block finds its job by binary search over block offsets. Splits are planned per job from each job's share of the total work, so many small per-layer launches become a few larger ones. Separately, the BN-fold backward kernel is split into a row-chunked pass that writes partial dot products to scratch and a column pass that reduces them, which adds parallelism over the reduction dimension at the cost of an extra launch and scratch memory.

```diff
diff --git a/confignet_amd/_lib.py b/confignet_amd/_lib.py
--- a/confignet_amd/_lib.py
+++ b/confignet_amd/_lib.py
@@ -62,7 +62,8 @@
     "cn_conv_dgrad": [_G, _p, _p, _p, _p],
     "cn_conv_dgrad_w": [_G, _p, _p, _p, _p],
     "cn_conv_dgrad_w_res": [_G, _p, _p, _p, _p, _p],
-    "cn_bn_fold_bwd": [_p, _i, _i, _p, _p, _p, _p, _p, _p, _p, _p],
+    "cn_bn_fold_bwd_chunks": [],
+    "cn_bn_fold_bwd": [_p, _i, _i, _p, _p, _p, _p, _p, _p, _p, _p, _i, _p],
     "cn_conv_wgrad_thin_partials": [],
     "cn_conv_wgrad_thin": [_G, _p, _p, _p, _p, _i, _p],
     "cn_conv_wgrad": [_G, _p, _p, _p, _i, _p],
@@ -72,6 +73,8 @@
     "cn_conv_wgrad_dt_workspace_bytes": [_G, _i, _i, ctypes.POINTER(_z)],
     "cn_conv_wgrad_dt": [_G, _p, _i, _p, _i, _p, _i, _p, _z, ctypes.POINTER(_i), _p],
     "cn_conv_wgrad_plan": [_G, _i, _i, _i, ctypes.c_uint, _i, ctypes.POINTER(ctypes.c_longlong)],
+    "cn_conv_wgrad_grouped": [_i, _p, _p, _p, _p, _p, _p, _p, _i, _p, _p],
+    "cn_conv_wgrad_grouped_plan": [_i, _p, _i, _p, _p],
     "cn_sum_parts_grouped": [_p, _i, _p],
     "cn_gemm_depth_grouped": [_p, _i, _p],
     "cn_gan_loss_grouped": [_p, _i, _i, _p],
diff --git a/confignet_amd/csrc/common.h b/confignet_amd/csrc/common.h
--- a/confignet_amd/csrc/common.h
+++ b/confignet_amd/csrc/common.h
@@ -64,9 +64,25 @@
     long tiles_x, tiles_y, splits, rows;
 };
 bool cn_wgrad2_ok(const CnConvGeom& g);
-Wg2Plan cn_wgrad2_plan(const CnConvGeom& g, int forced_cfg, long wg_target);
+Wg2Plan cn_wgrad2_plan(const CnConvGeom& g, int forced_cfg, long wg_target, bool group = false);
 void cn_wgrad2(int cfg, int ns, const CnConvGeom& g, const float* x, const float* gy, float* out, long slab_stride, int rows, int tiles_x,
                int tiles_y, int splits, int accumulate, unsigned grid, hipStream_t s);
+constexpr int CN_WG2_GROUP = 24, CN_KERNARG_BYTES = 4096;
+struct Wg2Job {
+    CnConvGeom g;
+    int rows, tiles_x, tiles_y, nsplits, accumulate;
+    const float* x;
+    const float* gy;
+    float* out;
+    long slab_stride;
+};
+struct Wg2Jobs {
+    Wg2Job job[CN_WG2_GROUP];
+    int blk0[CN_WG2_GROUP + 1];
+    int n;
+};
+static_assert(sizeof(Wg2Jobs) <= CN_KERNARG_BYTES, "the jobs of a grouped launch travel in its kernel arguments");
+void cn_wgrad2_grouped(int cfg, const Wg2Jobs& J, unsigned grid, hipStream_t s);
 void cn_igemm_wgrad(int cfg, const CnConvGeom& g, const float* x, const float* gy, float* gw, int rows, float* parts, int tx, int ty,
                     int splits, dim3 grid, hipStream_t s);
 int cn_tiny_wgrad(const CnConvGeom& g, const float* x, const float* gy, float* gw, int blocks, float* parts, hipStream_t s);
diff --git a/confignet_amd/csrc/conv_dispatch.hip b/confignet_amd/csrc/conv_dispatch.hip
--- a/confignet_amd/csrc/conv_dispatch.hip
+++ b/confignet_amd/csrc/conv_dispatch.hip
@@ -1,6 +1,7 @@
 #include "common.h"
 
 #include <algorithm>
+#include <vector>
 
 #include "mma_tile.h"
 #include "conv_geom.h"
@@ -647,6 +648,148 @@
     return p.ret;
 }
 
+namespace {
+
+struct WgGroupJob {
+    int cfg = -1, stages = 0, tx = 0, ty = 0, launch = 0;
+    long splits = 1, rows = 0, blk0 = 0, wgs = 0;
+    size_t ws_floats = 0;
+};
+
+bool wgrad_groupable(const CnConvGeom& g) { return cn_wgrad2_ok(g) && (long)g.k_d * g.k_h * g.k_w * g.cin >= 64; }
+
+bool plan_conv_wgrad_group(int njobs, const CnConvGeom* g, bool solo, std::vector<WgGroupJob>& jobs, std::vector<long>& grids) {
+    jobs.assign(njobs, WgGroupJob{});
+    grids.clear();
+    std::vector<double> work(njobs);
+    double work_all = 0.0;
+    for (int j = 0; j < njobs; ++j) {
+        if (!wgrad_groupable(g[j])) return false;
+        work[j] = (double)g[j].n * g[j].out_d * g[j].out_h * g[j].out_w * g[j].k_d * g[j].k_h * g[j].k_w * g[j].cin * g[j].cout;
+        work_all += work[j];
+    }
+    const double chip = 2.0 * cn_cu_count();
+    auto share = [&](double w, double of, double launches) { return std::max(1L, (long)(chip * launches * w / of + 0.5)); };
+    const int tuned = g_tune_cfg == 0 || (g_tune_cfg >= 2 && g_tune_cfg <= 5) ? g_tune_cfg : -1;
+    for (int j = 0; j < njobs; ++j) {
+        WgGroupJob& q = jobs[j];
+        if (solo) {
+            const WgradPlan p = plan_conv_wgrad(g[j], WgradReq{CN_F32, CN_F32, true, WG_FP32_GEMM});
+            q.cfg = p.cfg; q.splits = p.splits; q.rows = p.rows; q.tx = p.tx; q.ty = p.ty;
+        } else {
+            q.cfg = cn_wgrad2_plan(g[j], tuned, share(work[j], work_all, cn_cdiv(njobs, CN_WG2_GROUP)), true).cfg;
+        }
+        q.stages = q.cfg == 3 ? 3 : 4;
+    }
+    std::vector<int> open(8, -1), count;
+    std::vector<double> work_of;
+    for (int j = 0; j < njobs; ++j) {
+        int& l = open[jobs[j].cfg];
+        if (l < 0 || count[l] == CN_WG2_GROUP) {
+            l = (int)count.size();
+            count.push_back(0);
+            work_of.push_back(0.0);
+        }
+        jobs[j].launch = l;
+        ++count[l];
+        work_of[l] += work[j];
+    }
+    grids.assign(count.size(), 0);
+    std::vector<int> order(njobs);
+    for (int j = 0; j < njobs; ++j) {
+        WgGroupJob& q = jobs[j];
+        order[j] = j;
+        if (!solo) {
+            const Wg2Plan w = cn_wgrad2_plan(g[j], q.cfg, share(work[j], work_of[q.launch], 1.0), true);
+            q.splits = w.splits; q.rows = w.rows; q.tx = (int)w.tiles_x; q.ty = (int)w.tiles_y;
+        }
+        q.wgs = (q.splits >= 8 ? cn_cdiv(q.splits, 8) * 8 : q.splits) * q.tx * q.ty;
+        if (q.splits > 1) q.ws_floats = (size_t)q.splits * g[j].k_d * g[j].k_h * g[j].k_w * g[j].cin * g[j].cout;
+    }
+    std::stable_sort(order.begin(), order.end(), [&](int a, int b) { return jobs[a].rows > jobs[b].rows; });
+    for (int j : order) {
+        WgGroupJob& q = jobs[j];
+        q.blk0 = grids[q.launch];
+        grids[q.launch] += q.wgs;
+    }
+    for (long gr : grids)
+        if (gr >= 0x7fffffffL) return false;
+    return true;
+}
+
+}
+
+extern "C" int cn_conv_wgrad_grouped(int njobs, const CnConvGeom* geoms, const float* const* x, const float* const* gy, float* const* out,
+                                     float* const* ws, const size_t* ws_bytes, const int* accumulate, int solo, int* parts, void* stream) {
+    CN_CHECK_ARG(njobs >= 0 && (njobs == 0 || (geoms && x && gy && out && accumulate && parts)), "cn_conv_wgrad_grouped: bad arguments");
+    for (int j = 0; j < njobs; ++j) {
+        if (int e = check_geom(geoms + j)) return e;
+        CN_CHECK_ARG(x[j] && gy[j] && out[j], "cn_conv_wgrad_grouped: job %d has a NULL tensor", j);
+    }
+    std::vector<WgGroupJob> jobs;
+    std::vector<long> grids;
+    if (!plan_conv_wgrad_group(njobs, geoms, solo != 0, jobs, grids)) {
+        cn_set_error("cn_conv_wgrad_grouped: a job the LDS-DMA filter-gradient kernel does not take");
+        return CN_EUNSUPPORTED;
+    }
+    for (int j = 0; j < njobs; ++j)
+        CN_CHECK_ARG(jobs[j].ws_floats == 0 || (ws && ws_bytes && ws[j] && ws_bytes[j] >= sizeof(float) * jobs[j].ws_floats),
+                     "cn_conv_wgrad_grouped: job %d needs a workspace of %zu bytes", j, sizeof(float) * jobs[j].ws_floats);
+    const hipStream_t s = (hipStream_t)stream;
+    std::vector<int> order(njobs);
+    for (int j = 0; j < njobs; ++j) order[j] = j;
+    std::sort(order.begin(), order.end(), [&](int a, int b) { return jobs[a].blk0 < jobs[b].blk0; });
+    for (int l = 0; l < (int)grids.size(); ++l) {
+        Wg2Jobs J{};
+        int n = 0, cfg = -1;
+        double flops = 0.0, bytes = 0.0;
+        for (int j : order) {
+            const WgGroupJob& q = jobs[j];
+            if (q.launch != l) continue;
+            const CnConvGeom& g = geoms[j];
+            const long count = (long)g.k_d * g.k_h * g.k_w * g.cin * g.cout;
+            Wg2Job& o = J.job[n];
+            o.g = g;
+            o.rows = (int)q.rows; o.tiles_x = q.tx; o.tiles_y = q.ty; o.nsplits = (int)q.splits; o.accumulate = accumulate[j] ? 1 : 0;
+            o.x = x[j]; o.gy = gy[j];
+            o.out = q.splits > 1 ? ws[j] : out[j];
+            o.slab_stride = q.splits > 1 ? count : 0;
+            J.blk0[n++] = (int)q.blk0;
+            cfg = q.cfg;
+            flops += conv_flops(g);
+            bytes += conv_bytes(g, 4.0, 4.0, 4.0);
+            parts[j] = q.splits > 1 ? (int)q.splits : 0;
+        }
+        J.blk0[n] = (int)grids[l];
+        J.n = n;
+        cn_prof_begin(s, flops, bytes, wgrad_family(cfg));
+        cn_wgrad2_grouped(cfg, J, (unsigned)grids[l], s);
+        cn_prof_end(s);
+        CN_LAUNCH_CHECK();
+    }
+    return CN_OK;
+}
+
+extern "C" int cn_conv_wgrad_grouped_plan(int njobs, const CnConvGeom* geoms, int solo, long long* out, long long info[4]) {
+    CN_CHECK_ARG(njobs >= 0 && (njobs == 0 || (geoms && out)) && info, "cn_conv_wgrad_grouped_plan: bad arguments");
+    for (int j = 0; j < njobs; ++j)
+        if (int e = check_geom(geoms + j)) return e;
+    std::vector<WgGroupJob> jobs;
+    std::vector<long> grids;
+    info[0] = 0; info[1] = CN_WG2_GROUP; info[2] = (long long)sizeof(Wg2Jobs); info[3] = CN_KERNARG_BYTES;
+    if (!plan_conv_wgrad_group(njobs, geoms, solo != 0, jobs, grids)) {
+        cn_set_error("cn_conv_wgrad_grouped: a job the LDS-DMA filter-gradient kernel does not take");
+        return CN_EUNSUPPORTED;
+    }
+    info[0] = (long long)grids.size();
+    for (int j = 0; j < njobs; ++j) {
+        const WgGroupJob& q = jobs[j];
+        const long long v[10] = {q.cfg, q.stages, q.splits, q.rows, q.tx, q.ty, q.blk0, q.wgs, q.launch, (long long)q.ws_floats};
+        for (int i = 0; i < 10; ++i) out[10 * j + i] = v[i];
+    }
+    return CN_OK;
+}
+
 extern "C" int cn_conv_loop_select(int loop, int kb, int ns, int np) {
     CN_CHECK_ARG(loop >= -1 && loop <= 1 && (kb == 0 || kb == 16 || kb == 32) && (ns == 0 || ns == 3 || ns == 4) && np >= -1 && np <= 2,
                  "cn_conv_loop_select: bad argument");
diff --git a/confignet_amd/csrc/elementwise.hip b/confignet_amd/csrc/elementwise.hip
--- a/confignet_amd/csrc/elementwise.hip
+++ b/confignet_amd/csrc/elementwise.hip
@@ -1638,13 +1638,82 @@
         *gbias = o;
     }
 }
-}
+
+constexpr int BN_FOLD_CHUNKS = 16;
+__global__ __launch_bounds__(256) void bn_fold_bwd_rows_kernel(const int* __restrict__ seg, int nseg, const float* __restrict__ gwf,
+                                                               const float* __restrict__ arena, const float* __restrict__ a,
+                                                               float* __restrict__ gout, float* __restrict__ scratch, int ncols) {
+    const int b = blockIdx.x, chunk = blockIdx.y;
+    int lo = 0, hi = nseg - 1;
+    while (lo < hi) {
+        const int mid = (lo + hi + 1) >> 1;
+        if (seg[9 * mid + 8] <= b) lo = mid; else hi = mid - 1;
+    }
+    const int* sg = seg + 9 * lo;
+    const int cout = sg[3], K = sg[2] / cout;
+    const int c4 = threadIdx.x & 15, rl = threadIdx.x >> 4;
+    const int col = (b - sg[8]) * 64 + c4 * 4;
+    const int per = (K + BN_FOLD_CHUNKS - 1) / BN_FOLD_CHUNKS, r0 = chunk * per, r1 = min(K, r0 + per);
+    const float4 av = *reinterpret_cast<const float4*>(a + sg[4] + col);
+    float4 dot = make_float4(0.f, 0.f, 0.f, 0.f);
+    for (int r = r0 + rl; r < r1; r += 16) {
+        const long off = (long)r * cout + col;
+        const float4 g = *reinterpret_cast<const float4*>(gwf + sg[1] + off);
+        const float4 w = *reinterpret_cast<const float4*>(arena + sg[0] + off);
+        float4* d = reinterpret_cast<float4*>(gout + sg[0] + off);
+        float4 o = *d;
+        o.x += g.x * av.x; o.y += g.y * av.y; o.z += g.z * av.z; o.w += g.w * av.w;
+        *d = o;
+        dot.x += g.x * w.x; dot.y += g.y * w.y; dot.z += g.z * w.z; dot.w += g.w * w.w;
+    }
+    __shared__ float4 red[16][16];
+    red[rl][c4] = dot;
+    __syncthreads();
+    if (rl == 0) {
+        float4 t = red[0][c4];
+        for (int q = 1; q < 16; ++q) { const float4 u = red[q][c4]; t.x += u.x; t.y += u.y; t.z += u.z; t.w += u.w; }
+        *reinterpret_cast<float4*>(scratch + (long)chunk * ncols + sg[4] + col) = t;
+    }
+}
+
+__global__ __launch_bounds__(64) void bn_fold_bwd_cols_kernel(const int* __restrict__ seg, int nseg, const float* __restrict__ gshift,
+                                                              const float* __restrict__ a, const float* __restrict__ rs,
+                                                              const float* __restrict__ bm, float* __restrict__ gout,
+                                                              const float* __restrict__ scratch, int ncols) {
+    const int b = blockIdx.x;
+    int lo = 0, hi = nseg - 1;
+    while (lo < hi) {
+        const int mid = (lo + hi + 1) >> 1;
+        if (seg[9 * mid + 8] <= b) lo = mid; else hi = mid - 1;
+    }
+    const int* sg = seg + 9 * lo;
+    const int col = (b - sg[8]) * 64 + threadIdx.x, c = sg[4] + col;
+    float t = scratch[c];
+    for (int q = 1; q < BN_FOLD_CHUNKS; ++q) t += scratch[(long)q * ncols + c];
+    const float gs = gshift[c];
+    gout[sg[6] + col] += rs[c] * (t + gs * bm[c]);
+    gout[sg[7] + col] += gs;
+    gout[sg[5] + col] += a[c] * gs;
+}
+}
+
+extern "C" int cn_bn_fold_bwd_chunks(void) { return BN_FOLD_CHUNKS; }
 
 extern "C" int cn_bn_fold_bwd(const int* seg, int nseg, int blocks, const float* gwf, const float* gshift, const float* arena,
-                              const float* a, const float* rs, const float* bm, float* gout, void* stream) {
-    CN_CHECK_ARG(seg && gwf && gshift && arena && a && rs && bm && gout && nseg > 0 && blocks > 0, "bn_fold_bwd: bad args");
-    hipLaunchKernelGGL(bn_fold_bwd_kernel, dim3((unsigned)blocks), dim3(256), 0, (hipStream_t)stream, seg, nseg, gwf, gshift, arena, a, rs,
-                       bm, gout);
+                              const float* a, const float* rs, const float* bm, float* gout, float* scratch, int ncols, void* stream) {
+    CN_CHECK_ARG(seg && gwf && gshift && arena && a && rs && bm && gout && nseg > 0 && blocks > 0 && (!scratch || ncols > 0),
+                 "bn_fold_bwd: bad args");
+    if (!scratch || cn_det()) {
+        hipLaunchKernelGGL(bn_fold_bwd_kernel, dim3((unsigned)blocks), dim3(256), 0, (hipStream_t)stream, seg, nseg, gwf, gshift, arena, a,
+                           rs, bm, gout);
+        CN_LAUNCH_CHECK();
+        return CN_OK;
+    }
+    hipLaunchKernelGGL(bn_fold_bwd_rows_kernel, dim3((unsigned)blocks, BN_FOLD_CHUNKS), dim3(256), 0, (hipStream_t)stream, seg, nseg, gwf,
+                       arena, a, gout, scratch, ncols);
+    CN_LAUNCH_CHECK();
+    hipLaunchKernelGGL(bn_fold_bwd_cols_kernel, dim3((unsigned)blocks), dim3(64), 0, (hipStream_t)stream, seg, nseg, gshift, a, rs, bm, gout,
+                       scratch, ncols);
     CN_LAUNCH_CHECK();
     return CN_OK;
 }
diff --git a/confignet_amd/csrc/wgrad2.hip b/confignet_amd/csrc/wgrad2.hip
--- a/confignet_amd/csrc/wgrad2.hip
+++ b/confignet_amd/csrc/wgrad2.hip
@@ -17,10 +17,10 @@
     return n;
 }
 
-template <int WM, int WN, int TM, int TN, int KB, int NS>
+template <int WM, int WN, int TM, int TN, int KB, int NS, bool GROUPED>
 __device__ __forceinline__ void wgrad2_body(const CnConvGeom& g, const float* __restrict__ X, const float* __restrict__ GY,
                                             float* __restrict__ out, long slab_stride, int rows_per_split, int tiles_x, int tiles_y,
-                                            int nsplits, int accumulate) {
+                                            int nsplits, int accumulate, int id) {
     static_assert(WM * WN == 4, "4 waves per workgroup");
     constexpr int BI = 32 * WM * TM, BN = 32 * WN * TN;
     constexpr int QA = KB * BI / 256, QB = KB * BN / 256;
@@ -40,7 +40,7 @@
     static_assert(NS >= 3, "stages");
     __shared__ __attribute__((aligned(1024))) float SM[NS * (SA + SB)];
 
-    const int ntile = tiles_x * tiles_y, id = blockIdx.x;
+    const int ntile = tiles_x * tiles_y;
     int bz, tt;
     if (nsplits >= 8) {
         const int grp = id / (8 * ntile), rr = id - grp * 8 * ntile;
@@ -267,7 +267,27 @@
 __global__ __launch_bounds__(256) void wgrad2_kernel(CnConvGeom g, const float* __restrict__ X, const float* __restrict__ GY,
                                                      float* __restrict__ out, long slab_stride, int rows_per_split, int tiles_x,
                                                      int tiles_y, int nsplits, int accumulate) {
-    wgrad2_body<WM, WN, TM, TN, KB, NS>(g, X, GY, out, slab_stride, rows_per_split, tiles_x, tiles_y, nsplits, accumulate);
+    wgrad2_body<WM, WN, TM, TN, KB, NS, false>(g, X, GY, out, slab_stride, rows_per_split, tiles_x, tiles_y, nsplits, accumulate, blockIdx.x);
+}
+
+template <int WM, int WN, int TM, int TN, int KB, int NS>
+__device__ __forceinline__ void wgrad2_grouped_body(const Wg2Jobs& J) {
+    const int b = blockIdx.x;
+    int lo = 0, hi = J.n;
+    while (hi - lo > 1) {
+        const int mid = (lo + hi) >> 1;
+        if (J.blk0[mid] <= b) lo = mid;
+        else hi = mid;
+    }
+    const int j = __builtin_amdgcn_readfirstlane(lo);
+    const Wg2Job& q = J.job[j];
+    const int id = b - J.blk0[j];
+    wgrad2_body<WM, WN, TM, TN, KB, NS, true>(q.g, q.x, q.gy, q.out, q.slab_stride, q.rows, q.tiles_x, q.tiles_y, q.nsplits, q.accumulate, id);
+}
+
+template <int WM, int WN, int TM, int TN, int KB, int NS>
+__global__ __launch_bounds__(256) void wgrad2_grouped_kernel(Wg2Jobs J) {
+    wgrad2_grouped_body<WM, WN, TM, TN, KB, NS>(J);
 }
 
 struct Wg2Tile {
@@ -296,7 +316,7 @@
 
 }
 
-Wg2Plan cn_wgrad2_plan(const CnConvGeom& g, int forced, long target) {
+Wg2Plan cn_wgrad2_plan(const CnConvGeom& g, int forced, long target, bool group) {
     const long M = (long)g.n * g.out_d * g.out_h * g.out_w;
     const long Ktot = (long)g.k_d * g.k_h * g.k_w * g.cin;
     Wg2Plan p{};
@@ -308,19 +328,39 @@
             continue;
         const long tiles = (long)cn_cdiv(Ktot, t.bi) * cn_cdiv(g.cout, t.bn);
         const long max_splits = cn_cdiv(M, 4 * t.kb);
+        auto take = [&](double score, long rows, long splits) {
+            if (best < 0.0 || score < best) {
+                best = score;
+                p.cfg = t.cfg;
+                p.tiles_x = cn_cdiv(Ktot, t.bi); p.tiles_y = cn_cdiv(g.cout, t.bn);
+                p.rows = rows; p.splits = splits;
+            }
+        };
         auto consider = [&](long s_) {
             if (s_ < 1) s_ = 1;
             if (s_ > max_splits) s_ = max_splits;
             long rows, splits;
             const double us = wg2_cost(t, M, Ktot, g.cout, s_, rows, splits);
-            if (best < 0.0 || us < best) {
-                best = us;
-                p.cfg = t.cfg;
-                p.tiles_x = cn_cdiv(Ktot, t.bi); p.tiles_y = cn_cdiv(g.cout, t.bn);
-                p.rows = rows; p.splits = splits;
-            }
+            take(us, rows, splits);
         };
-        if (target > 0) {
+        if (group) {
+            long cap = target <= 0 || tiles >= target ? 1 : (target + tiles / 2) / tiles;
+            if (cap >= 8) cap = (cap + 4) / 8 * 8;
+            if (cap > max_splits) cap = max_splits;
+            double us_s = -1.0;
+            long rows = 0, splits = 1;
+            auto slices = [&](long s_) {
+                long r_, n_;
+                const double us = wg2_cost(t, M, Ktot, g.cout, s_, r_, n_);
+                if (us_s < 0.0 || us < us_s) { us_s = us; rows = r_; splits = n_; }
+            };
+            for (long s_ = 1; s_ < 8 && s_ <= cap; ++s_) slices(s_);
+            for (long s_ = 8; s_ <= cap && s_ <= 1024; s_ += 8) slices(s_);
+            const double life = ((double)rows * (32.0 * (t.bi / 32) * (t.bn / 32) / 4.0) + 9000.0) / 2400.0;
+            double chip_us = (double)(tiles * splits) * life / (t.e2 * cn_cu_count());
+            if (splits > 1) chip_us += 2.0 * (double)splits * (double)Ktot * g.cout * 4.0 / 2.5e6;
+            take(chip_us, rows, splits);
+        } else if (target > 0) {
             consider(tiles >= target ? 1 : (target + tiles / 2) / tiles);
         } else {
             for (long s_ = 1; s_ < 8 && s_ <= max_splits; ++s_) consider(s_);
@@ -353,3 +393,15 @@
 #undef WG2N
 #undef WG2
 }
+
+void cn_wgrad2_grouped(int cfg, const Wg2Jobs& J, unsigned grid, hipStream_t s) {
+#define WG2G(WM, WN, TM, TN, KB_, NS_) hipLaunchKernelGGL((wgrad2_grouped_kernel<WM, WN, TM, TN, KB_, NS_>), dim3(grid), dim3(256), 0, s, J)
+    switch (cfg) {
+        case 0: WG2G(2, 2, 2, 2, 16, 4); break;
+        case 4: WG2G(4, 1, 1, 3, 16, 4); break;
+        case 2: WG2G(2, 2, 1, 1, 32, 4); break;
+        case 5: WG2G(4, 1, 2, 2, 16, 4); break;
+        default: WG2G(4, 1, 1, 1, 32, 3); break;
+    }
+#undef WG2G
+}
diff --git a/confignet_amd/dnn_models/real_encoder.py b/confignet_amd/dnn_models/real_encoder.py
--- a/confignet_amd/dnn_models/real_encoder.py
+++ b/confignet_amd/dnn_models/real_encoder.py
@@ -312,10 +312,17 @@
         def geom(ci, t):
             return enc._convs[ci][2].geom(tuple(t.shape), wf[ci].shape[-1])
 
+        later = []
+
         def wgrad(ci, t_in, gu):
             o, shp = views[ci]
-            if want_w:
-                ops.sink_conv_wgrad_to(t_in, gu, geom(ci, t_in), shp, gwf[o:o + int(np.prod(shp))].view(shp), defer=sunk)
+            if not want_w:
+                return
+            g_, dst = geom(ci, t_in), gwf[o:o + int(np.prod(shp))].view(shp)
+            if ops.wgrad_groupable(t_in, gu, g_):
+                later.append((t_in, gu, g_, dst, 0))
+            else:
+                ops.sink_conv_wgrad_to(t_in, gu, g_, shp, dst, defer=sunk)
 
         def relu_bwd(ci, g, y, also=None):
             if not want_w:
@@ -359,9 +366,11 @@
         if not want_w:
             return (None, gx) + (None,) * len(params)
         if sunk:
+            ops.sink_conv_wgrad_group(later)
             gout = enc.grad_arena
             ops.sink_post(lambda: ops.bn_fold_bwd(seg9, blocks, gwf, gsh, enc.arena, a, rs, bm, gout), keep=(gwf, gsh, a, rs, bm))
             return (None, gx) + (None,) * len(params)
+        ops._sum_slabs_grouped(ops.conv_wgrad_grouped(later))
         gout = torch.zeros_like(enc.arena)
         ops.bn_fold_bwd(seg9, blocks, gwf, gsh, enc.arena, a, rs, bm, gout)
         base = enc.arena.data_ptr()
diff --git a/confignet_amd/ops.py b/confignet_amd/ops.py
--- a/confignet_amd/ops.py
+++ b/confignet_amd/ops.py
@@ -525,6 +525,46 @@
     return gw
 
 
+WGRAD_GROUPED = True
+
+
+def wgrad_groupable(x, gy, g):
+    if not WGRAD_GROUPED or DETERMINISTIC or ACT_DTYPE != torch.float32 or x.dtype != torch.float32 or gy.dtype != torch.float32:
+        return False
+    out = (ctypes.c_longlong * 12)()
+    return lib.cn_conv_wgrad_plan(ctypes.byref(g), CN_F32, CN_F32, 1, 0xffffffff, -1, out) == 0 and out[0] == 3
+
+
+def conv_wgrad_grouped_plan(geoms, solo=False):
+    n = len(geoms)
+    arr = (CnConvGeom * n)(*geoms)
+    out, info = (ctypes.c_longlong * (10 * n))(), (ctypes.c_longlong * 4)()
+    check(lib.cn_conv_wgrad_grouped_plan(n, arr, int(solo), out, info), "cn_conv_wgrad_grouped_plan")
+    return [tuple(out[10 * j:10 * j + 10]) for j in range(n)], tuple(info)
+
+
+def conv_wgrad_grouped(jobs, solo=False):
+    if not jobs:
+        return []
+    n = len(jobs)
+    xs, gys = [_c(j[0]) for j in jobs], [_c(j[1]) for j in jobs]
+    plan, _ = conv_wgrad_grouped_plan([j[2] for j in jobs], solo)
+    total = sum(p[9] for p in plan)
+    ws_all = torch.empty(total, device=xs[0].device, dtype=torch.float32) if total else None
+    ws, o = [], 0
+    for p in plan:
+        ws.append(ws_all[o:o + p[9]] if p[9] else None)
+        o += p[9]
+    vp = ctypes.c_void_p * n
+    parts = (ctypes.c_int * n)()
+    check(lib.cn_conv_wgrad_grouped(n, (CnConvGeom * n)(*[j[2] for j in jobs]), vp(*[_fptr(t).value for t in xs]),
+                                    vp(*[_fptr(t).value for t in gys]), vp(*[_fptr(j[3]).value for j in jobs]),
+                                    vp(*[None if w is None else w.data_ptr() for w in ws]),
+                                    (ctypes.c_size_t * n)(*[4 * p[9] for p in plan]), (ctypes.c_int * n)(*[int(bool(j[4])) for j in jobs]),
+                                    int(solo), parts, _stream()), "cn_conv_wgrad_grouped")
+    return [(ws[k], jobs[k][3], parts[k], jobs[k][3].numel(), int(bool(jobs[k][4]))) for k in range(n) if parts[k]]
+
+
 GRAD_SINK = True
 _SINK = None
 
@@ -546,6 +586,7 @@
     def __init__(self, params):
         self.slots = {p.data_ptr(): p.grad for p in params if p.grad is not None}
         self.touched = []
+        self.wgrads = []
         self.slabs = []
         self.depth = []
         self.upfold = {}
@@ -602,19 +643,20 @@
         others = [s_ for s_ in st.touched if s_ != cur]
         for s_ in others:
             cur.wait_stream(s_)
-        slabs, depth, upfold, post, post_keep = st.slabs, st.depth, st.upfold, st.post, st.post_keep
-        st.touched, st.slabs, st.depth, st.upfold, st.post, st.post_keep = [], [], [], {}, [], []
+        wgrads, slabs, depth, upfold, post, post_keep = st.wgrads, st.slabs, st.depth, st.upfold, st.post, st.post_keep
+        st.touched, st.wgrads, st.slabs, st.depth, st.upfold, st.post, st.post_keep = [], [], [], [], {}, [], []
+        slabs = slabs + conv_wgrad_grouped(wgrads)
         _sum_slabs_grouped(slabs)
         _gemm_depth_grouped(depth)
-        if slabs or depth:
-            _release_operands(cur, others, [j[0] for j in slabs] + [t for j in depth for t in j[:2]])
+        if wgrads or slabs or depth:
+            _release_operands(cur, others, [t for j in wgrads for t in j[:2]] + [j[0] for j in slabs] + [t for j in depth for t in j[:2]])
         for gw2, g, w_shape, slot in upfold.values():
             upfold_wgrad(gw2, g, w_shape, out=slot, single_writer=True)
         for fn in post:
             fn()
         if post:
             _release_operands(cur, others, post_keep)
-        if st.slabs or st.depth or st.upfold or st.post:
+        if st.wgrads or st.slabs or st.depth or st.upfold or st.post:
             raise RuntimeError("a sink_post function queued work on the gradient sink after its join")
 
     def __exit__(self, exc_type, exc, tb):
@@ -642,6 +684,15 @@
     if _SINK is not None:
         _SINK.note_stream()
     conv_wgrad(x, gy, g, w_shape, out=dst, accumulate=False, defer=defer)
+
+
+def sink_conv_wgrad_group(jobs):
+    st = _SINK
+    if st is None:
+        _sum_slabs_grouped(conv_wgrad_grouped(jobs))
+        return
+    st.note_stream()
+    st.wgrads.extend(jobs)
 
 
 def sink_post(fn, keep=()):
@@ -654,9 +705,12 @@
     st.post.append(fn)
 
 
-def bn_fold_bwd(seg9, blocks, gwf, gshift, arena, a, rs, bm, gout):
+def bn_fold_bwd(seg9, blocks, gwf, gshift, arena, a, rs, bm, gout, chunked=True):
+    scratch = None
+    if chunked and not DETERMINISTIC:
+        scratch = torch.empty(lib.cn_bn_fold_bwd_chunks() * a.numel(), device=a.device, dtype=torch.float32)
     check(lib.cn_bn_fold_bwd(_ptr(seg9), seg9.shape[0], blocks, _fptr(gwf), _fptr(gshift), _fptr(arena), _fptr(a), _fptr(rs), _fptr(bm),
-                             _fptr(gout), _stream()), "cn_bn_fold_bwd")
+                             _fptr(gout), _fptr(scratch), a.numel(), _stream()), "cn_bn_fold_bwd")
 
 
 def sink_upfold_wgrad(gy, x, g2, wd_shape, g, w_shape, slot):
diff --git a/include/confignet_hip.h b/include/confignet_hip.h
--- a/include/confignet_hip.h
+++ b/include/confignet_hip.h
@@ -60,6 +60,9 @@
 int cn_conv_wgrad_dt(const CnConvGeom* g, const void* x, int x_dt, const void* gy, int gy_dt, float* gw, int mode, void* workspace,
                      size_t workspace_bytes, int* parts, void* stream);
 int cn_conv_wgrad_plan(const CnConvGeom* g, int x_dt, int gy_dt, int caller_slabs, unsigned routes, int det, long long out[12]);
+int cn_conv_wgrad_grouped(int njobs, const CnConvGeom* geoms, const float* const* x, const float* const* gy, float* const* out,
+                          float* const* ws, const size_t* ws_bytes, const int* accumulate, int solo, int* parts, void* stream);
+int cn_conv_wgrad_grouped_plan(int njobs, const CnConvGeom* geoms, int solo, long long* out, long long info[4]);
 typedef struct CnSumJob {
     const float* src;
     float* dst;
@@ -247,8 +250,9 @@
                         int n, int h, int w, int c, void* stream);
 int cn_to_uint8(const float* x, uint8_t* out, size_t numel, void* stream);
 int cn_scale_columns_segments(const float* src, float* dst, const int* seg, const float* a, int nseg, size_t total, void* stream);
+int cn_bn_fold_bwd_chunks(void);
 int cn_bn_fold_bwd(const int* seg, int nseg, int blocks, const float* gwf, const float* gshift, const float* arena,
-                   const float* a, const float* rs, const float* bm, float* gout, void* stream);
+                   const float* a, const float* rs, const float* bm, float* gout, float* scratch, int ncols, void* stream);
 
 int cn_hdri_rows_v(const float* x, float* v, const int* y0, const float* wy, int pool, int h, int w, int oh, int t_len,
                    void* stream);
```

New measurement: 442.5 images/sec (median of 6 runs). 1.03x the previous value.
